# TimmyOVO/deepseek-ocr.rs

Measured on AMD Instinct MI355X. Metric: pages/sec + decode tok/s, DeepSeek-OCR fp16 1024px/512tok, higher is better.
Workload: dtype f32 (fp16-rounded decoder weights, bf16 vision/lm_head weights); 1 GPU; configs[1]: deepseek-ocr, 1024x1024 page, crop (2,2), 706-token prefill, 512 greedy tokens; pages_per_gpu=1, global_batch=1, parallelism=dp1

## Files before the change

deepseek-ocr.rs_amd/csrc/engine/capi.cpp:

```cpp
#include "../../../include/dsocr.h"

#include <fcntl.h>
#include <signal.h>
#include <unistd.h>

#include <cmath>
#include <cstdio>
#include <cstdlib>
#include <cstring>
#include <fstream>
#include <memory>
#include <sstream>
#include <string>
#include <utility>

#include "../common/host_util.hpp"
#include "dots.hpp"
#include "engine.hpp"
#include "host_ops.hpp"

struct dsocr_engine {
    std::unique_ptr<dsocr::Engine> impl;
    dsocr::Controls staged;
};
// ... 998 lines not shown
        out->o_proj = cp(p.o_proj);
        out->router = cp(p.router);
        out->layers_step = cp(p.layers_step);
        out->lm_head_screened = cp(p.lm_head_screened);
        out->moe_gateup_kernel = p.gateup_kernel;
        out->moe_down_kernel = p.down_kernel;
    });
}

dsocr_status dsocr_engine_set_spans(dsocr_engine* e, int enable) {
    return guarded([&] {
        if (!e) throw std::runtime_error("EINVAL: NULL engine");
        e->impl->set_spans(enable);
    });
}

dsocr_status dsocr_engine_spans(const dsocr_engine* e, uint64_t* out, size_t cap, size_t* kinds, size_t* layers,
                                size_t* steps) {
    return guarded([&] {
        if (!e) throw std::runtime_error("EINVAL: NULL engine");
        const auto& v = e->impl->spans();
        const size_t nl = e->impl->cfg().lang.layers;
        const size_t ns = v.empty() ? 0 : (size_t)e->impl->span_steps();
        if (kinds) *kinds = (size_t)e->impl->span_kinds();
        if (layers) *layers = nl;
        if (steps) *steps = ns;
        if (!out) return;
        if (v.size() > cap)
            throw std::runtime_error("EINVAL: span buffer holds " + std::to_string(cap) + " values, " +
                                     std::to_string(v.size()) + " needed");
        if (!v.empty()) std::memcpy(out, v.data(), v.size() * 8);
    });
}
static_assert(dsocr::Engine::SPAN_FIELDS == 5, "dsocr.h documents 5 fields per span record");

dsocr_status dsocr_engine_set_persist_stamps(dsocr_engine* e, int mode) {
    return guarded([&] {
        if (!e) throw std::runtime_error("EINVAL: NULL engine");
        e->impl->set_persist_stamps(mode);
    });
}

dsocr_status dsocr_engine_persist_info(const dsocr_engine* e, int* used, double* durations, size_t cap_d,
                                       size_t* n_launches, uint64_t* stamps, size_t cap_s, size_t* n_stamps) {
    return guarded([&] {
        if (!e) throw std::runtime_error("EINVAL: NULL engine");
        const auto& d = e->impl->persist_launch_us();
        const auto& st = e->impl->persist_stamps();
        if (used) *used = e->impl->persist_used() ? 1 : 0;
        if (n_launches) *n_launches = d.size();
        if (n_stamps) *n_stamps = st.size();
        if (durations) {
            if (d.size() > cap_d) throw std::runtime_error("EINVAL: duration buffer too small");
            if (!d.empty()) std::memcpy(durations, d.data(), d.size() * sizeof(double));
        }
        if (stamps) {
            if (st.size() > cap_s) throw std::runtime_error("EINVAL: stamp buffer too small");
            if (!st.empty()) std::memcpy(stamps, st.data(), st.size() * 8);
        }
    });
}

dsocr_status dsocr_device_count(int* n) {
    return guarded([&] { check_hip(hipGetDeviceCount(n), "hipGetDeviceCount"); });
}
dsocr_status dsocr_dev_alloc(size_t bytes, void** ptr) {
    return guarded([&] {
        if (hipMalloc(ptr, bytes ? bytes : 16) != hipSuccess) throw std::runtime_error("ENOMEM: hipMalloc failed");
    });
}
dsocr_status dsocr_dev_free(void* ptr) {
    return guarded([&] { check_hip(hipFree(ptr), "hipFree"); });
}
dsocr_status dsocr_memcpy_h2d(void* dst, const void* src, size_t bytes) {
    return guarded([&] { check_hip(hipMemcpy(dst, src, bytes, hipMemcpyHostToDevice), "hipMemcpy H2D"); });
}
dsocr_status dsocr_memcpy_d2h(void* dst, const void* src, size_t bytes) {
    return guarded([&] { check_hip(hipMemcpy(dst, src, bytes, hipMemcpyDeviceToHost), "hipMemcpy D2H"); });
}
dsocr_status dsocr_dev_sync(void) {
    return guarded([&] { check_hip(hipDeviceSynchronize(), "hipDeviceSynchronize"); });
}
dsocr_status dsocr_synth_bf16(const char* name, uint64_t seed, uint64_t n, uint16_t* out) {
    return guarded([&] {
        if (!name || (!out && n)) throw std::runtime_error("EINVAL: NULL argument");
        dsocr::synth_bf16(name, seed, n, out);
    });
}
dsocr_status dsocr_resize_bicubic(const uint8_t* src, uint32_t sw, uint32_t sh, uint8_t* dst, uint32_t dw, uint32_t dh) {
    return guarded([&] {
        if (!src || !dst) throw std::runtime_error("EINVAL: NULL argument");
        dsocr::resize_bicubic(src, (int)sw, (int)sh, dst, (int)dw, (int)dh);
    });
}

dsocr_status dsocr_resize_catmull_rom(const uint8_t* src, uint32_t sw, uint32_t sh, uint8_t* dst, uint32_t dw,
                                      uint32_t dh) {
    return guarded([&] {
        if (!src || !dst || !sw || !sh || !dw || !dh) throw std::runtime_error("EINVAL: NULL argument or empty image");
        dsocr::resize_catmull_rom_fir(src, (int)sw, (int)sh, dst, (int)dw, (int)dh);
    });
}

dsocr_status dsocr_k_gemm(int M, int N, int K, const float* A, const void* W, int wdtype, const float* bias, float* C,
                          int act, int accumulate) {
    return guarded([&] {
        if (K % 8) throw std::runtime_error("EINVAL: K must be a multiple of 8");
        dsocr::GemmArgs g;
        g.M = M; g.N = N; g.K = K; g.A = A; g.lda = K; g.W = W; g.ldw = K; g.wdtype = wdtype; g.bias = bias;
        g.C = C; g.ldc = N; g.act = act; g.accumulate = accumulate;
        dsocr::launch_gemm(g, nullptr);
        check_hip(hipGetLastError(), "gemm launch");
        check_hip(hipDeviceSynchronize(), "gemm");
    });
}
dsocr_status dsocr_k_gemm_grouped(int M, int N, int K, const float* A, int lda, const int* a_rows, const void* W,
                                  int wdtype, long long w_group_stride, const float* bias, long long bias_group_stride,
                                  float* C, int ldc, const int* c_rows, int act, int accumulate, const int* group_off,
                                  int groups, int max_group_rows, int kernel) {
    return guarded([&] {
        if (!A || !W || !C || !group_off || groups < 1 || M < 0 || N < 1 || K < 1)
            throw std::runtime_error("EINVAL: grouped gemm arguments");
        dsocr::GemmArgs g;
        g.M = M; g.N = N; g.K = K; g.A = A; g.lda = lda; g.a_rows = a_rows; g.W = W; g.ldw = K; g.wdtype = wdtype;
        g.w_group_stride = (long)w_group_stride; g.bias = bias; g.bias_group_stride = (long)bias_group_stride;
        g.C = C; g.ldc = ldc; g.c_rows = c_rows; g.act = act; g.accumulate = accumulate;
        g.group_off = group_off; g.groups = groups; g.max_group_rows = max_group_rows;
        if (kernel == 1 || kernel == 2) dsocr::launch_gemm_f32a_grouped(g, nullptr, kernel == 2 ? 128 : 32);
        else dsocr::launch_gemm(g, nullptr);
        check_hip(hipGetLastError(), "grouped gemm launch");
        check_hip(hipDeviceSynchronize(), "grouped gemm");
    });
}
dsocr_status dsocr_k_gemm_f32a(int M, int N, int K, const float* A, const void* W, int wdtype, const float* bias,
                               float* C, int act, int accumulate, int splits) {
    return guarded([&] {
        if (wdtype != dsocr::WDT_BF16 && wdtype != dsocr::WDT_F16) throw std::runtime_error("EINVAL: weights must be bf16 or f16");
        dsocr::GemmBf16Args g;
        g.M = M; g.N = N; g.K = K; g.A = A; g.lda = K; g.W = W; g.ldw = K; g.bias = bias;
        g.w_f16 = wdtype == dsocr::WDT_F16;
        g.C = C; g.ldc = N; g.act = act; g.accumulate = accumulate;
        if (!dsocr::gemm_f32a_ok(g)) throw std::runtime_error("EINVAL: gemm_f32a needs K % 32 == 0 and 16-byte aligned rows");
        g.splits = splits > 0 ? splits : dsocr::gemm_f32a_splits(M, N, K);
        float* part = nullptr;
        if (g.splits > 1) {
            check_hip(hipMalloc(&part, sizeof(float) * (size_t)g.splits * M * N), "hipMalloc");
            g.part = part;
        }
        dsocr::launch_gemm_f32a(g, nullptr);
        hipError_t e = hipGetLastError();
        if (e == hipSuccess) e = hipDeviceSynchronize();
        if (part) (void)hipFree(part);
        check_hip(e, "gemm_f32a");
    });
}
dsocr_status dsocr_k_gemv(int M, int N, int K, const float* x, const float* norm_w, float eps, const void* W,
                          int wdtype, const float* bias, float* y, int act, int accumulate) {
    return dsocr_k_gemv_ex(M, N, K, x, K, norm_w, eps, W, K, wdtype, bias, y, N, act, accumulate, 0, nullptr);
}
static bool gemv_kind_is_mm(const char* kind) { return std::strncmp(kind, "dec_mm_", 7) == 0; }
dsocr_status dsocr_k_gemv_ex(int M, int N, int K, const float* x, int ldx, const float* norm_w, float eps,
                             const void* W, int ldw, int wdtype, const float* bias, float* y, int ldy, int act,
                             int accumulate, int swizzle, const char** kind) {
    return guarded([&] {
        if (K < 8 || K % 8) throw std::runtime_error("EINVAL: K must be a positive multiple of 8");
        if (M < 0 || N < 0 || ldx < K || ldw < K || ldy < N || ldx % 4 || ldw % 8)
            throw std::runtime_error("EINVAL: gemv strides (ldx >= K, ldx % 4 == 0, ldw >= K, ldw % 8 == 0, ldy >= N)");
        if (wdtype != dsocr::WDT_BF16 && wdtype != dsocr::WDT_F16) throw std::runtime_error("EINVAL: weights must be bf16 or f16");
        dsocr::DecGemvArgs a;
        a.M = M; a.N = N; a.K = K; a.x = x; a.ldx = ldx; a.W = W; a.ldw = ldw; a.wdtype = wdtype; a.bias = bias;
        a.y = y; a.ldy = ldy; a.act = act; a.accumulate = accumulate; a.norm_w = norm_w; a.eps = eps;
        void* swz = nullptr;
        if (swizzle) {
            if (ldw != K) throw std::runtime_error("EINVAL: swizzle needs row-major W with ldw == K");
            if (!dsocr::dec_mm_ok(a) || !gemv_kind_is_mm(dsocr::dec_gemv_kernel_kind(a)))
                throw std::runtime_error("EINVAL: swizzle outside dec_mm's range (M 3..8, K 1280, N >= 16)");
            check_hip(hipMalloc(&swz, sizeof(uint16_t) * dsocr::mm_swizzle_elems(N, K)), "hipMalloc");
            a.w_swz = swz;
        }
        if (kind) *kind = dsocr::dec_gemv_kernel_kind(a);
        hipError_t e = hipSuccess;
        try {
            if (swz) dsocr::launch_mm_swizzle(W, N, K, swz, nullptr);
            dsocr::launch_dec_gemv(a, nullptr);
            e = hipGetLastError();
        } catch (...) {
            (void)hipDeviceSynchronize();
            if (swz) (void)hipFree(swz);
            throw;
        }
        if (e == hipSuccess) e = hipDeviceSynchronize();
        if (swz) (void)hipFree(swz);
        check_hip(e, "gemv");
    });
}
dsocr_status dsocr_k_gemv_kind(int M, int N, int K, int ldw, int wdtype, int has_norm, int has_xn_out, int swizzle,
                               const char** kind, int* rows_per_launch) {
    return guarded([&] {
        if (!kind) throw std::runtime_error("EINVAL: NULL argument");
        static float fd = 0.f;
        static uint16_t wd = 0;
        dsocr::DecGemvArgs a;
        a.M = M; a.N = N; a.K = K; a.x = &fd; a.ldx = K; a.W = &wd; a.ldw = ldw; a.wdtype = wdtype;
        a.y = &fd; a.ldy = N; a.norm_w = has_norm ? &fd : nullptr; a.xn_out = has_xn_out ? &fd : nullptr;
        a.w_swz = swizzle ? &wd : nullptr;
        *kind = dsocr::dec_gemv_kernel_kind(a, rows_per_launch);
    });
}
dsocr_status dsocr_k_mm_swizzle(int N, int K, const void* w, void* out) {
    return guarded([&] {
        if (N < 1 || K < 32 || K % 32 || !w || !out) throw std::runtime_error("EINVAL: mm_swizzle needs N >= 1, K % 32 == 0, w, out");
        dsocr::launch_mm_swizzle(w, N, K, out, nullptr);
        check_hip(hipGetLastError(), "mm_swizzle launch");
        check_hip(hipDeviceSynchronize(), "mm_swizzle");
    });
}
dsocr_status dsocr_k_silu_mul(int rows, int I, const float* g, int ldg, float* h, int ldh) {
    return guarded([&] {
        if (rows < 0 || I < 1 || ldg < 2 * I || ldh < I || !g || !h) throw std::runtime_error("EINVAL: silu_mul needs ldg >= 2 I, ldh >= I");
        dsocr::launch_silu_mul(g, ldg, I, rows, h, ldh, nullptr);
        check_hip(hipGetLastError(), "silu_mul launch");
        check_hip(hipDeviceSynchronize(), "silu_mul");
    });
}
dsocr_status dsocr_k_gemv_splitk(int M, int N, int K, const float* x, const void* W, int wdtype, const float* bias,
                                 float* y, int accumulate) {
    return guarded([&] {
        dsocr::DecGemvArgs a;
        a.M = M; a.N = N; a.K = K; a.x = x; a.ldx = K; a.W = W; a.ldw = K; a.wdtype = wdtype; a.bias = bias;
        a.y = y; a.ldy = N; a.accumulate = accumulate;
        if (!dsocr::dec_mm_splitk_ok(a)) throw std::runtime_error("EINVAL: gemv_splitk needs M <= 8, K % 64 == 0");
        float* part = nullptr;
        int* tick = nullptr;
        check_hip(hipMalloc(&part, sizeof(float) * dsocr::dec_mm_splitk_part_floats(N, K)), "hipMalloc");
        check_hip(hipMalloc(&tick, sizeof(int) * dsocr::dec_mm_splitk_ticks(N)), "hipMalloc");
        check_hip(hipMemset(tick, 0, sizeof(int) * dsocr::dec_mm_splitk_ticks(N)), "hipMemset");
        dsocr::launch_dec_mm_splitk(a, part, tick, nullptr);
        hipError_t e = hipDeviceSynchronize();
        (void)hipFree(part);
        (void)hipFree(tick);
        check_hip(e, "gemv_splitk");
    });
}
dsocr_status dsocr_k_layernorm(int rows, int cols, const float* x, const float* w, const float* b, float eps, float* y) {
    return guarded([&] {
        if (cols % 4) throw std::runtime_error("EINVAL: cols must be a multiple of 4");
        dsocr::launch_layernorm(x, cols, y, cols, nullptr, rows, cols, w, b, eps, nullptr);
        check_hip(hipDeviceSynchronize(), "layernorm");
    });
}
dsocr_status dsocr_k_dsq_dequant(int qtype, const void* src, size_t src_bytes, size_t out_dim, size_t in_dim,
                                 void* out_f16) {
    return guarded([&] {
        const size_t need = dsocr::dsq_payload_bytes(qtype, (long)out_dim, (long)in_dim);
        if (need == 0) throw std::runtime_error("EINVAL: unsupported snapshot tensor dtype code " + std::to_string(qtype));
        if (src_bytes != need)
            throw std::runtime_error("EINVAL: payload is " + std::to_string(src_bytes) + " bytes, expected " + std::to_string(need));
        dsocr::launch_dsq_dequant(qtype, src, (long)out_dim, (long)in_dim, out_f16, nullptr);
        check_hip(hipGetLastError(), "dsq_dequant launch");
        check_hip(hipDeviceSynchronize(), "dsq_dequant");
    });
}
dsocr_status dsocr_k_rmsnorm(int rows, int cols, const float* x, const float* w, float eps, float* y) {
    return guarded([&] {
        if (cols % 4) throw std::runtime_error("EINVAL: cols must be a multiple of 4");
        dsocr::launch_rmsnorm(x, cols, y, cols, rows, cols, w, eps, nullptr);
        check_hip(hipDeviceSynchronize(), "rmsnorm");
    });
}
dsocr_status dsocr_k_attention(int n_seq, int L, int heads, int hd, float scale, int causal, const float* q,
                               const float* k, const float* v, float* o, const float* relh, const float* relw, int gh,
                               int gw) {
    return guarded([&] {
        if (hd != 32 && hd != 64 && hd != 128) throw std::runtime_error("EINVAL: head_dim must be 32, 64 or 128");
        const long C = (long)heads * hd;
        dsocr::AttnArgs a;
        a.q = {q, C, hd, nullptr};
        a.k = {k, C, hd, nullptr};
        a.v = {v, C, hd, nullptr};
        a.o = o; a.o_row_stride = C; a.o_head_stride = hd; a.n_seq = n_seq; a.L = L; a.heads = heads;
        a.kv_heads = heads; a.hd = hd; a.scale = scale; a.causal = causal;
        float* rb = nullptr;
        float* part = nullptr;
        if (causal) {
            a.part_floats = dsocr::attention_causal_part_floats(n_seq, heads, L, hd);
            check_hip(hipMalloc(&part, sizeof(float) * a.part_floats), "hipMalloc attention pieces");
            a.part = part;
        }
        if (relh && relw) {
            if (gh * gw != L) throw std::runtime_error("EINVAL: rel-pos grid does not match L");
            check_hip(hipMalloc(&rb, sizeof(float) * (size_t)n_seq * heads * L * (gh + gw)), "hipMalloc relbias");
            dsocr::launch_sam_relbias(q, C, n_seq, gh, gw, heads, hd, relh, relw, rb, nullptr);
            a.relbias = rb; a.rel_h = gh; a.rel_w = gw;
        }
        dsocr::launch_attention(a, nullptr);
        hipError_t e = hipDeviceSynchronize();
        if (rb) (void)hipFree(rb);
        if (part) (void)hipFree(part);
        check_hip(e, "attention");
    });
}
dsocr_status dsocr_k_attention_prefix(int n_seq, int L, int prefix, int heads, int kv_heads, int hd, float scale,
                                      const float* q, const float* k, const float* v, float* o) {
    return guarded([&] {
        dsocr::AttnPrefixArgs a;
        a.q = q; a.k = k; a.v = v; a.o = o;
// ... 1436 lines not shown
```

deepseek-ocr.rs_amd/csrc/engine/engine.cpp:

```cpp
#include "engine.hpp"

#include <algorithm>
#include <chrono>
#include <random>
#include <cstdlib>
#include <cmath>
#include <cstring>
#include <fstream>
#include <functional>
#include <sstream>

#include "../common/host_util.hpp"
#include "dsq.hpp"
#include "host_ops.hpp"

namespace dsocr {

namespace {

struct HostMat {
    std::vector<uint16_t> data;
    int dt = WDT_BF16;
};

// ... 566 lines not shown
            g.data.insert(g.data.end(), u.data.begin(), u.data.end());
            e.gu.W = up16(g);
            e.gu.wdt = g.dt;
            e.gu.N = 2 * Q.inter;
            e.gu.K = D;
            e.down = lin_nobias(lp + "mlp.down_proj", D, Q.inter);
            enc_.layers.push_back(e);
        }
        enc_.norm = vecf(qp + "model.model.norm.weight", D);
        enc_.query_768 = vecf(qp + "query_768.weight", (size_t)Q.query_768 * D);
        enc_.query_1024 = vecf(qp + "query_1024.weight", (size_t)Q.query_1024 * D);
        {
            const int Lmax = 2 * Q.query_1024, half = hd / 2;
            std::vector<float> inv(half), c((size_t)Lmax * hd), s((size_t)Lmax * hd);
            for (int i = 0; i < half; ++i) inv[i] = 1.0f / powf(Q.rope_theta, (float)i / (float)half);
            for (int p = 0; p < Lmax; ++p)
                for (int i = 0; i < half; ++i) {
                    const float a = (float)p * inv[i];
                    c[(size_t)p * hd + i] = c[(size_t)p * hd + half + i] = cosf(a);
                    s[(size_t)p * hd + i] = s[(size_t)p * hd + half + i] = sinf(a);
                }
            enc_.cos = upf(c);
            enc_.sin = upf(s);
        }
        if (S.out_ch[1] != D) throw std::runtime_error("EINVAL: SAM output channels must equal the qwen2-0-5b encoder width");
    } else {
    const ClipConfig& C = cfg_.clip;
    const std::string cp = "model.vision_model.";
    clip_.cls = vecf(cp + "embeddings.class_embedding", C.hidden);
    clip_.pos_host = src.f32(cp + "embeddings.position_embedding.weight", (size_t)(C.seq + 1) * C.hidden);
    clip_.pre = {vecf(cp + "pre_layrnorm.weight", C.hidden), vecf(cp + "pre_layrnorm.bias", C.hidden)};
    for (int l = 0; l < C.layers; ++l) {
        ClipLayer cl;
        const std::string lp = cp + "transformer.layers." + std::to_string(l) + ".";
        cl.ln1 = {vecf(lp + "layer_norm1.weight", C.hidden), vecf(lp + "layer_norm1.bias", C.hidden)};
        cl.ln2 = {vecf(lp + "layer_norm2.weight", C.hidden), vecf(lp + "layer_norm2.bias", C.hidden)};
        cl.qkv = lin(lp + "self_attn.qkv_proj", 3 * C.hidden, C.hidden, true);
        cl.out = lin(lp + "self_attn.out_proj", C.hidden, C.hidden, true);
        cl.fc1 = lin(lp + "mlp.fc1", C.ffn, C.hidden, true);
        cl.fc2 = lin(lp + "mlp.fc2", C.hidden, C.ffn, true);
        clip_.layers.push_back(cl);
    }
    if (C.hidden != S.out_ch[1]) throw std::runtime_error("EINVAL: CLIP width must equal SAM output channels");
    if (C.hidden + S.out_ch[1] != cfg_.proj_in) throw std::runtime_error("EINVAL: combined hidden dims do not match projector input");
    }

    proj_ = lin("model.projector.layers", cfg_.proj_out, cfg_.proj_in, true);
    newline_ = cfg_.variant != VARIANT_OCR2 && src.has("model.image_newline")
                   ? vecf("model.image_newline", cfg_.proj_out)
                   : upf(std::vector<float>(cfg_.proj_out, 0.f));
    separator_ = vecf("model.view_seperator", cfg_.proj_out);

    const LangConfig& L = cfg_.lang;
    {
        HostMat m = src.h16("model.embed_tokens.weight", (size_t)L.vocab * L.hidden);
        embed_ = up16(m);
        embed_dt_ = m.dt;
    }
    const int H = L.hidden, KVH = L.kv_heads * L.head_dim;
    for (int l = 0; l < L.layers; ++l) {
        DecLayer d;
        const std::string lp = "model.layers." + std::to_string(l) + ".";
        d.in_norm = {vecf(lp + "input_layernorm.weight", H), nullptr};
        d.post_norm = {vecf(lp + "post_attention_layernorm.weight", H), nullptr};
        d.qkv = lin_cat({lp + "self_attn.q_proj", lp + "self_attn.k_proj", lp + "self_attn.v_proj"},
                        {L.heads * L.head_dim, KVH, L.kv_heads * L.v_head_dim}, H);
        d.o = lin(lp + "self_attn.o_proj", H, L.heads * L.v_head_dim, true);
        d.moe = L.moe_layer(l);
        if (!d.moe) {
            d.gu = lin_cat({lp + "mlp.gate_proj", lp + "mlp.up_proj"}, {L.inter, L.inter}, H);
            d.down = lin(lp + "mlp.down_proj", H, L.inter, true);
            if (d.gu.b || d.down.b) throw std::runtime_error("EINVAL: biased dense MLP not supported");
        } else {
            const int E = L.n_routed, I = L.moe_inter;
            HostMat r = src.h16(lp + "mlp.gate.weight", (size_t)E * H);
            d.router.W = up16(r);
            d.router.wdt = r.dt;
            d.router.N = E;
            d.router.K = H;
            d.router.b = optvec(lp + "mlp.gate.e_score_correction_bias", E);
            HostMat gu, dn;
            gu.data.resize((size_t)E * 2 * I * H);
            dn.data.resize((size_t)E * H * I);
            for (int e = 0; e < E; ++e) {
                const std::string ep = lp + "mlp.experts." + std::to_string(e) + ".";
                HostMat g = src.h16(ep + "gate_proj.weight", (size_t)I * H, I, H);
                HostMat u = src.h16(ep + "up_proj.weight", (size_t)I * H, I, H);
                HostMat w = src.h16(ep + "down_proj.weight", (size_t)H * I, H, I);
                if (src.has(ep + "gate_proj.bias") || src.has(ep + "down_proj.bias"))
                    throw std::runtime_error("EINVAL: biased experts not supported");
                std::copy(g.data.begin(), g.data.end(), gu.data.begin() + (size_t)e * 2 * I * H);
                std::copy(u.data.begin(), u.data.end(), gu.data.begin() + (size_t)e * 2 * I * H + (size_t)I * H);
                std::copy(w.data.begin(), w.data.end(), dn.data.begin() + (size_t)e * H * I);
                gu.dt = dn.dt = g.dt;
            }
            d.e_gu = up16(gu);
            d.e_d = up16(dn);
            d.e_wdt = gu.dt;
            if (L.n_shared > 0) {
                const int Is = I * L.n_shared;
                d.has_shared = true;
                d.s_gu = lin_cat({lp + "mlp.shared_experts.gate_proj", lp + "mlp.shared_experts.up_proj"}, {Is, Is}, H);
                d.s_d = lin(lp + "mlp.shared_experts.down_proj", H, Is, true);
            }
            if (packed_experts && d.e_wdt == WDT_F16 && dec_route_grp_ok(8, E, H, L.topk)) {
                std::vector<std::string> gu_n, dn_n;
                for (int e = 0; e < E; ++e) {
                    const std::string ep = lp + "mlp.experts." + std::to_string(e) + ".";
                    gu_n.push_back(ep + "gate_proj.weight");
                    gu_n.push_back(ep + "up_proj.weight");
                    dn_n.push_back(ep + "down_proj.weight");
                }
                const long Is = (long)I * L.n_shared;
                const std::vector<std::string> sgu_n = {lp + "mlp.shared_experts.gate_proj.weight",
                                                        lp + "mlp.shared_experts.up_proj.weight"};
                const std::vector<std::string> sdn_n = {lp + "mlp.shared_experts.down_proj.weight"};
                bool ok = records_qtype(gu_n, I, H) >= 0 && records_qtype(dn_n, H, I) >= 0;
                if (ok && d.has_shared)
                    ok = !d.s_gu.b && !d.s_d.b && records_qtype(sgu_n, Is, H) >= 0 && records_qtype(sdn_n, H, Is) >= 0;
                if (ok) {
                    pack_records(gu_n, I, H, d.q_gu, d.packed_bytes);
                    pack_records(dn_n, H, I, d.q_d, d.packed_bytes);
                    if (d.has_shared) {
                        pack_records(sgu_n, Is, H, d.q_sgu, d.packed_bytes);
                        pack_records(sdn_n, H, Is, d.q_sd, d.packed_bytes);
                    }
                    d.packed = true;
                }
            }
        }
        layers_.push_back(d);
    }
    HIP_CHECK(hipDeviceSynchronize());
    final_norm_ = vecf("model.norm.weight", H);
    lm_head_ = lin("lm_head", L.vocab, H, false);
    if ((lm_head_.wdt == WDT_BF16 || lm_head_.wdt == WDT_F16) && H % 16 == 0 && H <= 1536) {
        const size_t vp = (size_t)(L.vocab + 15) / 16 * 16;
        lmq_ = dev_alloc((size_t)L.vocab * H);
        lmq_scale_ = (float*)dev_alloc(vp * 4);
        lmq_bound_ = (float*)dev_alloc(vp * 4);
        HIP_CHECK(hipMemset(lmq_scale_, 0, vp * 4));
        HIP_CHECK(hipMemset(lmq_bound_, 0, vp * 4));
        if (lmhead_q8mm_ok(8, L.vocab, H)) {
            lmq_qnorm_ = (float*)dev_alloc(vp * 4);
            HIP_CHECK(hipMemset(lmq_qnorm_, 0, vp * 4));
            lmq_frag_ = dev_alloc(lmhead_qfrag_bytes(L.vocab, H));
        }
        launch_lmhead_quantize(lm_head_.W, L.vocab, H, lmq_, lmq_scale_, lmq_bound_, nullptr, lmq_qnorm_, lmq_frag_,
                               lm_head_.wdt);
        HIP_CHECK(hipDeviceSynchronize());
    }
}

void Engine::linear(const float* x, int M, int ldx, const Lin& l, float* y, int ldy, int act, int accumulate,
                    const int* c_rows) {
    flops_acc_ += 2.0 * M * (double)l.N * l.K;
    if (M <= 16 && !c_rows) {
        DecGemvArgs a;
        a.M = M; a.N = l.N; a.K = l.K; a.x = x; a.ldx = ldx; a.W = l.W; a.ldw = l.K; a.wdtype = l.wdt;
        a.bias = l.b; a.y = y; a.ldy = ldy; a.act = act; a.accumulate = accumulate;
        launch_dec_gemv(a, stream_);
    } else if ((l.wdt == WDT_F16 || l.wdt == WDT_BF16) && l.K % 32 == 0 && ldx % 4 == 0 &&
               (reinterpret_cast<uintptr_t>(x) & 15) == 0) {
        GemmBf16Args g;
        g.M = M; g.N = l.N; g.K = l.K; g.A = x; g.lda = ldx; g.W = l.W; g.ldw = l.K; g.w_f16 = l.wdt == WDT_F16;
        g.bias = l.b; g.C = y; g.ldc = ldy; g.c_rows = c_rows; g.act = act; g.accumulate = accumulate;
        g.splits = gemm_f32a_splits(M, l.N, l.K);
        if (g.splits > 1) g.part = wsf("g_splitk", (size_t)g.splits * M * l.N);
        launch_gemm_f32a(g, stream_);
    } else {
        GemmArgs g;
        g.M = M; g.N = l.N; g.K = l.K; g.A = x; g.lda = ldx; g.W = l.W; g.ldw = l.K; g.wdtype = l.wdt;
        g.bias = l.b; g.C = y; g.ldc = ldy; g.c_rows = c_rows; g.act = act; g.accumulate = accumulate;
        launch_gemm(g, stream_);
    }
}

float* Engine::sam_pos(int g) {
    auto it = sam_.pos_dev.find(g);
    if (it != sam_.pos_dev.end()) return it->second;
    const int C = cfg_.sam.dim, src = sam_.pos_grid;
    std::vector<float> r = bicubic_resize_aa(sam_.pos_host, C, src, src, g, g);
    std::vector<float> nhwc((size_t)g * g * C);
    for (int c = 0; c < C; ++c)
        for (int p = 0; p < g * g; ++p) nhwc[(size_t)p * C + c] = r[(size_t)c * g * g + p];
    float* d = (float*)dev_alloc(nhwc.size() * 4);
    HIP_CHECK(hipMemcpy(d, nhwc.data(), nhwc.size() * 4, hipMemcpyHostToDevice));
    sam_.pos_dev[g] = d;
    return d;
}

std::pair<float*, float*> Engine::sam_rel(SamBlock& b, int g) {
    auto it = b.rel_dev.find(g);
    if (it != b.rel_dev.end()) return it->second;
    const int hd = cfg_.sam.dim / cfg_.sam.heads;
    std::vector<float> rh = rel_pos_resize(b.relh, b.rel_len, hd, g);
    std::vector<float> rw = rel_pos_resize(b.relw, b.rel_len, hd, g);
    float* dh = (float*)dev_alloc(rh.size() * 4);
    float* dw = (float*)dev_alloc(rw.size() * 4);
    HIP_CHECK(hipMemcpy(dh, rh.data(), rh.size() * 4, hipMemcpyHostToDevice));
    HIP_CHECK(hipMemcpy(dw, rw.data(), rw.size() * 4, hipMemcpyHostToDevice));
    b.rel_dev[g] = {dh, dw};
    return {dh, dw};
}

float* Engine::clip_pos(int tokens) {
    auto it = clip_.pos_dev.find(tokens);
    if (it != clip_.pos_dev.end()) return it->second;
    const ClipConfig& C = cfg_.clip;
    std::vector<float> out;
    if (tokens == C.seq + 1) {
        out = clip_.pos_host;
    } else {
        const int s = (int)std::lround(std::sqrt((double)C.seq)), t = (int)std::lround(std::sqrt((double)(tokens - 1)));
        if (t * t != tokens - 1) throw std::runtime_error("EINVAL: clip positional table tgt tokens not square");
        std::vector<float> grid((size_t)C.hidden * s * s);
        for (int p = 0; p < s * s; ++p)
            for (int c = 0; c < C.hidden; ++c) grid[(size_t)c * s * s + p] = clip_.pos_host[(size_t)(1 + p) * C.hidden + c];
        std::vector<float> r = bicubic_resize_aa(grid, C.hidden, s, s, t, t);
        out.resize((size_t)tokens * C.hidden);
        std::copy(clip_.pos_host.begin(), clip_.pos_host.begin() + C.hidden, out.begin());
        for (int p = 0; p < t * t; ++p)
            for (int c = 0; c < C.hidden; ++c) out[(size_t)(1 + p) * C.hidden + c] = r[(size_t)c * t * t + p];
    }
    float* d = (float*)dev_alloc(out.size() * 4);
    HIP_CHECK(hipMemcpy(d, out.data(), out.size() * 4, hipMemcpyHostToDevice));
    clip_.pos_dev[tokens] = d;
    return d;
}

static bool vis_streams_on() {
    static const bool v = !(getenv("DSOCR_VIS_STREAMS") && atoi(getenv("DSOCR_VIS_STREAMS")) == 0);
    return v;
}

float* Engine::vision_pass(const float* imgs, int n, int Spx, const std::string& out) {
    const SamConfig& S = cfg_.sam;
    const ClipConfig& CC = cfg_.clip;
    const int C = S.dim, heads = S.heads, hd = C / heads;
    if (Spx % S.patch) throw std::runtime_error("EINVAL: image dimensions must be divisible by patch size");
    const int g = Spx / S.patch;
    if (g % 2 || (g / 2) % 2) throw std::runtime_error("EINVAL: spatial dims cannot be evenly downsampled by stride 2");
    const long rows = (long)n * g * g;
    hipStream_t st = stream_;
    const bool s1 = vis_stage_ == 0 || vis_stage_ == 1, s2 = vis_stage_ == 0 || vis_stage_ == 2;
    const bool s3 = vis_stage_ == 0 || vis_stage_ == 3;
    const int g2 = g / 2, g4 = g / 4, c0 = S.out_ch[0], c1 = S.out_ch[1];
    const int Sq = g4 * g4;
    float* sam_out = wsf("v_samout", (size_t)n * Sq * c1);
    if (s1) {
    float* cols = wsf("v_cols", (size_t)rows * 3 * S.patch * S.patch);
    launch_patch_im2col(imgs, n, Spx, Spx, S.patch, cols, st);
    float* x = wsf("v_x", (size_t)rows * C);
    linear(cols, (int)rows, 3 * S.patch * S.patch, sam_.patch, x, C);
    if (sam_.has_pos) launch_add_broadcast(x, sam_pos(g), (long)g * g, C, n, st);

    const int W = S.window;
    const int gp = g + (W - g % W) % W, nw = gp / W;
    const long wrows = (long)n * nw * nw * W * W;
    auto wm = winmaps_.find({n, g});
    if (wm == winmaps_.end()) {
        std::vector<int> tok2win(rows), win2tok(wrows, -1);
        for (int b = 0; b < n; ++b)
            for (int y = 0; y < g; ++y)
                for (int xx = 0; xx < g; ++xx) {
                    long t = ((long)b * g + y) * g + xx;
                    long w = (((long)b * nw + y / W) * nw + xx / W) * W * W + (y % W) * W + (xx % W);
                    tok2win[t] = (int)w;
                    win2tok[w] = (int)t;
                }
        int *a = nullptr, *b2 = nullptr;
        HIP_CHECK(hipMalloc(&a, tok2win.size() * 4));
        HIP_CHECK(hipMalloc(&b2, win2tok.size() * 4));
        HIP_CHECK(hipMemcpy(a, tok2win.data(), tok2win.size() * 4, hipMemcpyHostToDevice));
        HIP_CHECK(hipMemcpy(b2, win2tok.data(), win2tok.size() * 4, hipMemcpyHostToDevice));
        wm = winmaps_.emplace(std::make_pair(n, g), std::make_pair(a, b2)).first;
    }
    int* d_tok2win = wm->second.first;
    int* d_win2tok = wm->second.second;
    const long maxrows = std::max(rows, wrows);
    float* xn = wsf("v_xn", (size_t)maxrows * C);
    float* qkv = wsf("v_qkv", (size_t)maxrows * 3 * C);
    float* ctx = wsf("v_ctx", (size_t)maxrows * C);
    const int hid = (int)(C * S.mlp_ratio);
    float* hbuf = wsf("v_h", (size_t)rows * hid);

    for (int bi = 0; bi < S.depth; ++bi) {
        SamBlock& blk = sam_.blocks[bi];
        const bool win = !blk.global;
        const int L = win ? W * W : g * g;
        const int nseq = win ? n * nw * nw : n;
        const long arows = (long)nseq * L;
        if (win) {
            HIP_CHECK(hipMemsetAsync(xn, 0, (size_t)wrows * C * 4, st));
            launch_layernorm(x, C, xn, C, d_tok2win, (int)rows, C, blk.n1.w, blk.n1.b, 1e-6f, st);
        } else {
            launch_layernorm(x, C, xn, C, nullptr, (int)rows, C, blk.n1.w, blk.n1.b, 1e-6f, st);
        }
        linear(xn, (int)arows, C, blk.qkv, qkv, 3 * C);
        AttnArgs a;
        a.q = {qkv, 3L * C, hd, nullptr};
        a.k = {qkv + C, 3L * C, hd, nullptr};
        a.v = {qkv + 2 * C, 3L * C, hd, nullptr};
        a.o = ctx;
        a.o_row_stride = C;
        a.o_head_stride = hd;
        a.n_seq = nseq;
        a.L = L;
        a.heads = heads;
        a.kv_heads = heads;
        a.hd = hd;
        a.scale = (float)(1.0 / std::sqrt((double)hd));
        if (blk.use_rel) {
            const int gg = win ? W : g;
            auto rel = win ? std::make_pair<float*, float*>(nullptr, nullptr) : sam_rel(blk, g);
            if (win) rel = sam_rel(blk, W);
            float* rb = wsf("v_relbias", (size_t)nseq * heads * L * (2 * gg));
            launch_sam_relbias(qkv, 3L * C, nseq, gg, gg, heads, hd, rel.first, rel.second, rb, st);
            a.relbias = rb;
            a.rel_h = gg;
            a.rel_w = gg;
        }
        flops_acc_ += 4.0 * nseq * (double)L * L * hd * heads;
        launch_attention(a, st);
        linear(ctx, (int)arows, C, blk.proj, x, C, 0, 1, win ? d_win2tok : nullptr);
        launch_layernorm(x, C, xn, C, nullptr, (int)rows, C, blk.n2.w, blk.n2.b, 1e-6f, st);
        linear(xn, (int)rows, C, blk.fc1, hbuf, hid, ACT_GELU_ERF);
        linear(hbuf, (int)rows, hid, blk.fc2, x, C, 0, 1);
    }
    const int NC = S.neck;
    float* y = wsf("v_neck", (size_t)rows * NC);
    linear(x, (int)rows, C, sam_.neck0, y, NC);
    launch_layernorm(y, NC, y, NC, nullptr, (int)rows, NC, sam_.neck1.w, sam_.neck1.b, 1e-6f, st);
    float* ncols = wsf("v_ncols", (size_t)rows * 9 * NC);
    launch_conv_im2col_nhwc(y, n, g, g, NC, 3, 3, 1, 1, ncols, st);
    linear(ncols, (int)rows, 9 * NC, sam_.neck2, y, NC);
    launch_layernorm(y, NC, y, NC, nullptr, (int)rows, NC, sam_.neck3.w, sam_.neck3.b, 1e-6f, st);
    launch_conv_im2col_nhwc(y, n, g, g, NC, 3, 3, 2, 1, ncols, st);
    float* z = wsf("v_net2", (size_t)n * g2 * g2 * c0);
    linear(ncols, n * g2 * g2, 9 * NC, sam_.net2, z, c0);
    float* ncols2 = wsf("v_ncols2", (size_t)n * g4 * g4 * 9 * c0);
    launch_conv_im2col_nhwc(z, n, g2, g2, c0, 3, 3, 2, 1, ncols2, st);
    linear(ncols2, n * Sq, 9 * c0, sam_.net3, sam_out, c1);
    }
    if (cfg_.variant == VARIANT_OCR2) return encoder_pass(sam_out, n, Sq, out);

    const int T = Sq + 1, CH = CC.hidden, chd = CH / CC.heads;
    const long crow = (long)n * T;
    float* cx = wsf("c_x", (size_t)crow * CH);
    if (s2) {
    launch_clip_embed(sam_out, clip_.cls, clip_pos(T), n, Sq, CH, cx, st);
    launch_layernorm(cx, CH, cx, CH, nullptr, (int)crow, CH, clip_.pre.w, clip_.pre.b, 1e-5f, st);
    }
    float* cxn = wsf("c_xn", (size_t)crow * CH);
    float* cqkv = wsf("c_qkv", (size_t)crow * 3 * CH);
    float* cctx = wsf("c_ctx", (size_t)crow * CH);
    float* ch = wsf("c_h", (size_t)crow * CC.ffn);
    for (int l = 0; s2 && l < CC.layers; ++l) {
        ClipLayer& cl = clip_.layers[l];
        launch_layernorm(cx, CH, cxn, CH, nullptr, (int)crow, CH, cl.ln1.w, cl.ln1.b, 1e-5f, st);
        linear(cxn, (int)crow, CH, cl.qkv, cqkv, 3 * CH);
        AttnArgs a;
        a.q = {cqkv, 3L * CH, chd, nullptr};
        a.k = {cqkv + CH, 3L * CH, chd, nullptr};
        a.v = {cqkv + 2 * CH, 3L * CH, chd, nullptr};
        a.o = cctx;
        a.o_row_stride = CH;
        a.o_head_stride = chd;
        a.n_seq = n;
        a.L = T;
        a.heads = CC.heads;
        a.kv_heads = CC.heads;
        a.hd = chd;
        a.scale = (float)(1.0 / std::sqrt((double)chd));
        flops_acc_ += 4.0 * n * (double)T * T * chd * CC.heads;
        launch_attention(a, st);
        linear(cctx, (int)crow, CH, cl.out, cx, CH, 0, 1);
        launch_layernorm(cx, CH, cxn, CH, nullptr, (int)crow, CH, cl.ln2.w, cl.ln2.b, 1e-5f, st);
        linear(cxn, (int)crow, CH, cl.fc1, ch, CC.ffn, ACT_QUICK_GELU);
        linear(ch, (int)crow, CC.ffn, cl.fc2, cx, CH, 0, 1);
    }
    float* pre = wsf("p_pre", (size_t)n * Sq * (CH + c1));
    float* post = wsf(out, (size_t)n * Sq * cfg_.proj_out);
    if (s3) {
        launch_concat_clip_sam(cx, sam_out, n, Sq, CH, c1, pre, st);
        linear(pre, n * Sq, CH + c1, proj_, post, cfg_.proj_out);
    }
    return post;
}

float* Engine::encoder_pass(const float* sam_out, int n, int P, const std::string& out) {
    const Qwen2EncConfig& Q = cfg_.enc;
    const float* query = P == Q.query_768 ? enc_.query_768 : P == Q.query_1024 ? enc_.query_1024 : nullptr;
    if (!query)
        throw std::runtime_error("EINVAL: unsupported Qwen2 query length " + std::to_string(P) + " (expected " +
                                 std::to_string(Q.query_768) + " or " + std::to_string(Q.query_1024) + ")");
    hipStream_t st = stream_;
    const int D = Q.dim, hd = Q.head_dim, L = 2 * P, QW = Q.heads * hd, KW = Q.kv_heads * hd, W3 = QW + 2 * KW;
    const long rows = (long)n * L;
    float* x = wsf("q2_x", (size_t)rows * D);
    float* xn = wsf("q2_xn", (size_t)rows * D);
    float* qkv = wsf("q2_qkv", (size_t)rows * W3);
    float* ctx = wsf("q2_ctx", (size_t)rows * QW);
    float* gu = wsf("q2_gu", (size_t)rows * 2 * Q.inter);
    float* hbuf = wsf("q2_h", (size_t)rows * Q.inter);
    const bool s2 = vis_stage_ == 0 || vis_stage_ == 2, s3 = vis_stage_ == 0 || vis_stage_ == 3;
    if (s2) launch_ocr2_build_seq(sam_out, query, n, P, D, x, st);
    for (const EncLayer& e : enc_.layers) {
        if (!s2) break;
        launch_rmsnorm(x, D, xn, D, (int)rows, D, e.in_norm.w, Q.rms_eps, st);
        linear(xn, (int)rows, D, e.qkv, qkv, W3);
        launch_ocr2_rope(qkv, W3, rows, L, Q.heads + Q.kv_heads, hd, enc_.cos, enc_.sin, st);
        AttnPrefixArgs a;
        a.q = qkv; a.k = qkv + QW; a.v = qkv + QW + KW; a.o = ctx;
        a.ldq = a.ldk = a.ldv = W3; a.ldo = QW;
        a.n_seq = n; a.L = L; a.prefix = P; a.heads = Q.heads; a.kv_heads = Q.kv_heads; a.hd = hd;
        a.scale = (float)(1.0 / std::sqrt((double)hd));
        flops_acc_ += 4.0 * n * Q.heads * hd * (2.0 * P * P + 0.5 * P * (P + 1.0));
        launch_attention_prefix(a, st);
        linear(ctx, (int)rows, QW, e.o, x, D, 0, 1);
        launch_rmsnorm(x, D, xn, D, (int)rows, D, e.post_norm.w, Q.rms_eps, st);
        linear(xn, (int)rows, D, e.gu, gu, 2 * Q.inter);
        launch_silu_mul(gu, 2 * Q.inter, Q.inter, (int)rows, hbuf, Q.inter, st);
        linear(hbuf, (int)rows, Q.inter, e.down, x, D, 0, 1);
    }
    float* qx = wsf("q2_q", (size_t)n * P * D);
    float* post = wsf(out, (size_t)n * P * cfg_.proj_out);
    if (s3) {
        launch_ocr2_take_queries(x, n, P, D, qx, st);
        launch_rmsnorm(qx, D, qx, D, n * P, D, enc_.norm, Q.rms_eps, st);
        linear(qx, n * P, D, proj_, post, cfg_.proj_out);
    }
    return post;
}

void Engine::check_page_variant(const PagePixels& pg) const {
    if (pg.variant != cfg_.variant)
        throw std::runtime_error(std::string("EINVAL: page was prepared for ") +
                                 (pg.variant == VARIANT_OCR2 ? "DeepSeek-OCR-2" : "DeepSeek-OCR") + " but the engine runs " +
                                 (cfg_.variant == VARIANT_OCR2 ? "DeepSeek-OCR-2" : "DeepSeek-OCR") +
                                 " (image slot layout mismatch)");
}

enum RowKind : int { ROW_TOKEN = 0, ROW_HOST = 1, ROW_VISION = 2, ROW_NEWLINE = 3, ROW_SEPARATOR = 4 };

static std::vector<std::pair<int, long>> image_row_order(const PagePixels& pg) {
    std::vector<std::pair<int, long>> seq;
    const int ls = pg.tile / 64, gs = pg.gsize / 64;
    const long n_local = pg.n_tiles > 0 ? (long)pg.n_tiles * ls * ls : 0;
    if (pg.variant == VARIANT_OCR2) {
        for (long i = 0; i < n_local + (long)gs * gs; ++i) seq.push_back({ROW_VISION, i});
        seq.push_back({ROW_SEPARATOR, 0});
        return seq;
    }
    for (int R = 0; n_local && R < pg.crop_h * ls; ++R) {
        for (int Cc = 0; Cc < pg.crop_w * ls; ++Cc) {
            const int crop = (R / ls) * pg.crop_w + (Cc / ls);
            seq.push_back({ROW_VISION, ((long)crop * ls + R % ls) * ls + Cc % ls});
        }
        seq.push_back({ROW_NEWLINE, 0});
    }
    for (int R = 0; R < gs; ++R) {
        for (int Cc = 0; Cc < gs; ++Cc) seq.push_back({ROW_VISION, n_local + (long)R * gs + Cc});
        seq.push_back({ROW_NEWLINE, 0});
    }
    seq.push_back({ROW_SEPARATOR, 0});
    return seq;
}

std::vector<std::vector<float>> Engine::image_embeddings(const std::vector<const PagePixels*>& pages) {
    std::vector<std::vector<float>> result;
    const int H = cfg_.proj_out;
    for (const PagePixels* p : pages) {
        check_page_variant(*p);
        float* gimg = p->global_dev && p->dev_ordinal == device_ ? p->global_dev : upload("e_gimg", p->global_chw);
        float* gpost = vision_pass(gimg, 1, p->gsize, "e_gpost");
        const int gs = p->gsize / 64;
        std::vector<float> gh((size_t)gs * gs * H);
        HIP_CHECK(hipMemcpyAsync(gh.data(), gpost, gh.size() * 4, hipMemcpyDeviceToHost, stream_));
        std::vector<float> lh;
        int ls = 0;
        if (p->n_tiles > 0) {
            float* timg = p->tiles_dev && p->dev_ordinal == device_ ? p->tiles_dev : upload("e_timg", p->tiles_chw);
            float* lpost = vision_pass(timg, p->n_tiles, p->tile, "e_lpost");
            ls = p->tile / 64;
            lh.resize((size_t)p->n_tiles * ls * ls * H);
            HIP_CHECK(hipMemcpyAsync(lh.data(), lpost, lh.size() * 4, hipMemcpyDeviceToHost, stream_));
        }
        HIP_CHECK(hipStreamSynchronize(stream_));
        std::vector<float> nl(H), sp(H);
        HIP_CHECK(hipMemcpy(nl.data(), newline_, H * 4, hipMemcpyDeviceToHost));
        HIP_CHECK(hipMemcpy(sp.data(), separator_, H * 4, hipMemcpyDeviceToHost));
        std::vector<float> rows;
        const size_t n_local = lh.size() / H;
        for (const auto& [kind, i] : image_row_order(*p)) {
            const float* r = kind == ROW_NEWLINE ? nl.data() : kind == ROW_SEPARATOR ? sp.data()
                             : (size_t)i < n_local ? &lh[i * H] : &gh[(i - n_local) * H];
            rows.insert(rows.end(), r, r + H);
        }
        result.push_back(std::move(rows));
    }
    return result;
}

void Engine::layer_forward_prefill(int l, int T, int B, const int* row_page, const int* row_pos, const long* q_off,
                                   const long* kv_off, const long* o_off, const int* seq_len, int max_len, int Lmax,
                                   const int* past, int max_total, bool chunk_attn) {
    const LangConfig& L = cfg_.lang;
    DecLayer& d = layers_[l];
    hipStream_t st = stream_;
    const int H = L.hidden, hd = L.head_dim, KVH = L.kv_heads * hd, QKVN = d.qkv.N;
    float* X = wsf("d_x", (size_t)T * H);
    float* XN = wsf("d_xn", (size_t)T * H);
    float* QKV = wsf("d_qkv", (size_t)T * QKVN);
    float* CTX = wsf("d_ctx", (size_t)T * H);
    float* kc = kc_ + (long)l * layer_kv(B) + (long)kv_page0_ * page_stride_;
    float* vc = vc_ + (long)l * layer_kv(B) + (long)kv_page0_ * page_stride_;

    launch_rmsnorm(X, H, XN, H, T, H, d.in_norm.w, L.rms_eps, st);
    linear(XN, T, H, d.qkv, QKV, QKVN);
    RopeKvArgs r;
    r.qkv = QKV; r.ld = QKVN; r.rows = T; r.row_page = row_page; r.row_pos = row_pos;
    r.heads = L.heads; r.kv_heads = L.kv_heads; r.hd = hd; r.rope_dim = L.rope_dim; r.use_mla = L.use_mla;
    r.cos = rope_cos_; r.sin = rope_sin_; r.kc = kc; r.vc = vc; r.page_stride = page_stride_; r.head_stride = head_stride_;
    launch_rope_kv(r, st);
    if (past) {
        AttnPastArgs a;
        a.q = {QKV, QKVN, hd, q_off};
        a.k = {kc, hd, head_stride_, kv_off};
        a.v = {vc, hd, head_stride_, kv_off};
        a.o = CTX; a.o_row_stride = H; a.o_head_stride = hd; a.o_seq_off = o_off;
        a.n_seq = B; a.past = past; a.n_q = seq_len; a.max_q = max_len; a.max_total = max_total;
        a.heads = L.heads; a.kv_heads = L.kv_heads; a.hd = hd;
        a.scale = (float)(1.0 / std::sqrt((double)hd));
        flops_acc_ += 4.0 * (double)T * max_total * hd * L.heads;
        if (chunk_attn) {
            launch_attention_chunk(a, st);
            ++chunk_attn_launches_;
        } else {
            a.part_floats = attention_past_part_floats(B, L.heads, max_len, max_total, hd);
            a.part = wsf("d_attn_past", a.part_floats);
            launch_attention_past(a, st);
        }
    } else {
        AttnArgs a;
        a.q = {QKV, QKVN, hd, q_off};
        a.k = {kc, hd, head_stride_, kv_off};
        a.v = {vc, hd, head_stride_, kv_off};
        a.o = CTX; a.o_row_stride = H; a.o_head_stride = hd; a.o_seq_off = o_off;
        a.n_seq = B; a.L = max_len; a.seq_len = seq_len;
        a.heads = L.heads; a.kv_heads = L.kv_heads; a.hd = hd;
        a.scale = (float)(1.0 / std::sqrt((double)hd));
        a.causal = 1;
        constexpr size_t kPartCapFloats = (size_t)128 << 20;
        const size_t part_floats = attention_causal_part_floats(B, L.heads, max_len, hd);
        if (part_floats <= kPartCapFloats) {
            a.part_floats = part_floats;
            a.part = wsf("d_attn_part", a.part_floats);
        }
        for (int q = 0; q < B && q < (int)prefill_lens_.size(); ++q)
            flops_acc_ += 2.0 * (double)prefill_lens_[q] * (prefill_lens_[q] + 1) * hd * L.heads;
        launch_attention(a, st);
    }
    (void)Lmax;
    (void)KVH;
    linear(CTX, T, H, d.o, X, H, 0, 1);
    launch_rmsnorm(X, H, XN, H, T, H, d.post_norm.w, L.rms_eps, st);
    if (!d.moe) {
        const int I = L.inter;
        float* G = wsf("d_g", (size_t)T * 2 * I);
        float* HH = wsf("d_hh", (size_t)T * I);
        linear(XN, T, H, d.gu, G, 2 * I);
        launch_silu_mul(G, 2 * I, I, T, HH, I, st);
        linear(HH, T, I, d.down, X, H, 0, 1);
        return;
    }
    const int E = L.n_routed, K = L.topk, I = L.moe_inter, TK = T * K;
    float* LOG = wsf("d_log", (size_t)T * E);
    int* IDS = wsi("d_ids", TK);
    float* WTS = wsf("d_wts", TK);
    int* EOFF = wsi("d_eoff", E + 1);
    int* AROW = wsi("d_arow", TK);
    int* APOS = wsi("d_apos", TK);
    linear(XN, T, H, d.router, LOG, E);
    launch_router_topk(LOG, T, E, K, L.scoring == "softmax", L.norm_topk, L.routed_scaling, IDS, WTS, st);
    launch_moe_group(IDS, T, K, E, EOFF, AROW, APOS, nullptr, st);
    float* G = wsf("d_eg", (size_t)TK * 2 * I);
    float* HH = wsf("d_ehh", (size_t)TK * I);
    float* Y = wsf("d_ey", (size_t)TK * H);
    GemmArgs g1;
    g1.M = TK; g1.N = 2 * I; g1.K = H; g1.A = XN; g1.lda = H; g1.a_rows = AROW; g1.W = d.e_gu; g1.ldw = H;
    g1.wdtype = d.e_wdt; g1.w_group_stride = (long)2 * I * H; g1.C = G; g1.ldc = 2 * I;
    g1.group_off = EOFF; g1.groups = E; g1.max_group_rows = T;
    launch_gemm(g1, st);
    flops_acc_ += 2.0 * TK * (2.0 * I) * H + 2.0 * TK * (double)H * I;
    launch_silu_mul(G, 2 * I, I, TK, HH, I, st);
    GemmArgs g2;
    g2.M = TK; g2.N = H; g2.K = I; g2.A = HH; g2.lda = I; g2.W = d.e_d; g2.ldw = I; g2.wdtype = d.e_wdt;
    g2.w_group_stride = (long)H * I; g2.C = Y; g2.ldc = H; g2.group_off = EOFF; g2.groups = E; g2.max_group_rows = T;
    launch_gemm(g2, st);
    float* YS = nullptr;
    if (d.has_shared) {
        const int Is = d.s_d.K;
        float* GS = wsf("d_sg", (size_t)T * 2 * Is);
        float* HS = wsf("d_shh", (size_t)T * Is);
        YS = wsf("d_sy", (size_t)T * H);
        linear(XN, T, H, d.s_gu, GS, 2 * Is);
        launch_silu_mul(GS, 2 * Is, Is, T, HS, Is, st);
        linear(HS, T, Is, d.s_d, YS, H);
    }
    launch_moe_combine(Y, APOS, WTS, YS, T, K, H, X, 1, st);
}

static bool router_swz_off() {
    const char* e = getenv("DSOCR_ROUTER_SWZ");
    return e && atoi(e) == 0;
}
static bool mm_swz_off() {
    const char* e = getenv("DSOCR_MM_SWZ");
    return e && atoi(e) == 0;
}

MoeDecodeArgs Engine::moe_args(int l, int B, float* X) {
    const LangConfig& L = cfg_.lang;
    DecLayer& d = layers_[l];
    const int H = L.hidden, E = L.n_routed, K = L.topk, I = L.moe_inter, TK = B * K;
    MoeDecodeArgs a;
    a.T = B; a.H = H; a.E = E; a.topk = K; a.I = I;
    a.x = X; a.norm_w = d.post_norm.w; a.eps = L.rms_eps; a.out = X;
    a.router = d.router.W; a.router_wdt = d.router.wdt; a.router_bias = d.router.b;
    a.Wgu = d.e_gu; a.Wd = d.e_d; a.wdtype = d.e_wdt;
    if (d.has_shared) {
        if (d.s_gu.wdt != d.e_wdt) throw std::runtime_error("EINTERNAL: shared/routed expert dtype mismatch");
        a.Is = d.s_d.K; a.sWgu = d.s_gu.W; a.sWd = d.s_d.W; a.hs = wsf("s_shh", (size_t)B * a.Is);
    }
    a.softmax_scoring = L.scoring == "softmax"; a.norm_topk = L.norm_topk; a.scaling = L.routed_scaling;
    a.xn = wsf("s_xn", (size_t)B * H);
    a.xn_router = wsf("s_xn_router", (size_t)B * H);
    a.logits = wsf("s_log", (size_t)B * E);
    a.ids = wsi("s_ids", TK); a.wts = wsf("s_wts", TK);
    a.h = wsf("s_ehh", (size_t)TK * I);
    a.grp = wsi("s_grp", moe_grp_ints(E, B, K));
    a.route_cnt = rows_.route_cnt;
    if (B >= 3 && B <= 8) {
        a.dn_part = wsf("s_dnpart", moe_down_mm_part_floats(E, B, K, I, a.Is, H));
        a.dn_tick = rows_.dn_tick;
    }
    if (B <= 8 && d.packed) {
        a.qWgu = d.q_gu; a.qWd = d.q_d; a.qsWgu = d.q_sgu; a.qsWd = d.q_sd;
    }
    if (B <= 8 && d.e_gu_swz && (!d.has_shared || d.s_gu_swz)) {
        a.Wgu_swz = d.e_gu_swz; a.Wd_swz = d.e_d_swz; a.sWgu_swz = d.s_gu_swz; a.sWd_swz = d.s_d_swz;
        if (!router_swz_off()) a.router_swz = d.router_swz;
    }
    if (B > 8) {
        a.eoff = wsi("s_eoff", E + 1); a.arow = wsi("s_arow", TK); a.apos = wsi("s_apos", TK);
        a.aw = wsf("s_aw", TK); a.active = wsi("s_active", E); a.n_active = wsi("s_nact", 1);
    }
    return a;
}

DecAttn2Args Engine::attn_args(int l, int B, int Lmax, int copy) {
    const LangConfig& L = cfg_.lang;
    const int hd = L.head_dim, QKVN = layers_[l].qkv.N;
    const long layer_kv = this->layer_kv(B);
    DecAttn2Args da;
    da.qkv = rows_.qkv[copy]; da.ld = QKVN; da.kv_pos = rows_.kv_pos; da.B = B;
    da.heads = L.heads; da.kv_heads = L.kv_heads; da.hd = hd; da.rope_dim = L.rope_dim; da.use_mla = L.use_mla;
    da.max_len = Lmax; da.cos = rope_cos_; da.sin = rope_sin_;
    da.kc = kc_ + (long)l * layer_kv; da.vc = vc_ + (long)l * layer_kv;
    da.page_stride = page_stride_; da.head_stride = head_stride_;
    da.scale = (float)(1.0 / std::sqrt((double)hd));
    da.part = rows_.part[copy];
    da.o = wsf("s_ctx", (size_t)B * L.hidden); da.o_ld = L.hidden;
    da.counters = rows_.attn_cnt;
    da.err = rows_.err;
    return da;
}

static bool graphs_on() {
    const char* e = getenv("DSOCR_NO_GRAPH");
    return !(e && atoi(e) != 0);
}

bool Engine::persist_ok(int B, int Lmax) {
    const char* e = getenv("DSOCR_PERSIST");
    if (!e || atoi(e) == 0) return false;
    const LangConfig& L = cfg_.lang;
    for (const DecLayer& d : layers_)
        if (d.packed) return false;
    if (B != 1 || L.use_mla || L.rope_dim != L.head_dim || L.v_head_dim != L.head_dim || L.n_shared <= 0 ||
        L.topk_method != "greedy" || L.hidden_act != "silu")
        return false;
    if (!dec_persist_shape_ok(L.hidden, L.heads, L.kv_heads, L.head_dim, L.n_routed, L.topk, L.moe_inter,
                              L.n_shared * L.moe_inter, L.inter, Lmax))
        return false;
    for (const DecLayer& d : layers_) {
        if (d.qkv.wdt != WDT_F16 || d.qkv.b || d.o.wdt != WDT_F16 || d.o.b) return false;
        if (d.moe) {
            if (!d.router.W || d.router.wdt != WDT_F16 || d.e_wdt != WDT_F16 || !d.has_shared || d.s_gu.wdt != WDT_F16 ||
                d.s_d.wdt != WDT_F16 || d.s_gu.b || d.s_d.b)
                return false;
        } else if (!d.gu.W || d.gu.wdt != WDT_F16 || d.down.wdt != WDT_F16) {
            return false;
        }
    }
    return dec_persist_resident() != 0;
}

void Engine::ensure_persist() {
    if (persist_lw_ || capturing_) return;
    const LangConfig& L = cfg_.lang;
    const int H = L.hidden, E = L.n_routed, I = L.moe_inter;
    std::vector<PersistLayerW> tab(layers_.size());
    for (size_t l = 0; l < layers_.size(); ++l) {
        DecLayer& d = layers_[l];
        PersistLayerW& w = tab[l];
        w.qkv = (const uint16_t*)d.qkv.W;
        w.o = (const uint16_t*)d.o.W;
        w.in_w = d.in_norm.w;
// ... 2295 lines not shown
```

deepseek-ocr.rs_amd/csrc/engine/engine.hpp:

```cpp
#pragma once
#include <hip/hip_runtime.h>

#include <cstring>
#include <functional>
#include <map>
#include <memory>
#include <set>
#include <stdexcept>
#include <string>
#include <vector>

#include "../kernels/kernels.hpp"
#include "config.hpp"
#include "hip_raii.hpp"

namespace dsocr {

struct Lin {
    void* W = nullptr;
    int wdt = WDT_BF16;
    int N = 0, K = 0;
    float* b = nullptr;
};
struct Ln {
// ... 199 lines not shown
        *g_status = nullptr, *g_on = nullptr, *g_stage = nullptr;
    size_t g_stage_cap = 0;
    GuidedTables guided_tables() const {
        GuidedTables t;
        t.mask = g_mask; t.mask_ld = g_mask_ld; t.cap_states = g_states; t.cap_edges = g_edges;
        t.rowptr = g_rowptr; t.tok = g_tok; t.next = g_next;
        t.state = g_state; t.seen = g_seen; t.status = g_status; t.on = g_on;
        return t;
    }
};
struct DecodeRowsSpec {
    int rows = 0, Lcap = 0;
    long ctx_cap = 0, out_cap = 0;
    bool sampler = false, ban = false, rowpar = false;
    bool handoff_max = false;
    bool zero_fill = false;
    int lp_k = -1;
    bool lp_side = false;
    bool bias = false;
    size_t bias_stage = 0;
    bool stops = false;
    int stop_stage_rows = 1;
    bool penalties = false;
    bool ngram_window = false;
    bool guided = false;
    int guided_states = GUIDED_MAX_STATES;
    long guided_edges = GUIDED_MAX_EDGES;
    size_t guided_stage = 0;
};
typedef void (*TokenCb)(size_t, const int64_t*, void*);
std::vector<uint32_t> rng_state_from_u64(uint64_t seed);

class Engine {
  public:
    Engine(const std::string& config_path, const std::string& weights_path, int device, int dtype, uint64_t seed,
           const std::string& snapshot_path = "", uint32_t load_flags = 0);
    ~Engine();
    void packed_info(size_t* packed_layers, size_t* moe_layers, size_t* packed_bytes) const;

    const ModelConfig& cfg() const { return cfg_; }
    int variant() const { return cfg_.variant; }
    std::vector<std::vector<float>> image_embeddings(const std::vector<const PagePixels*>& pages);
    std::vector<std::vector<int64_t>> generate(const std::vector<GenRequest>& reqs, const GenParams& p, TokenCb cb,
                                               void* user);
    Timings last_timings() const { return timings_; }
    struct LogprobRows {
        int K = 0;
        size_t cap = 0;
        std::vector<int> n;
        std::vector<float> lp, top_lp;
        std::vector<int> top_id;
    };
    const LogprobRows& last_logprobs() const { return last_lp_; }
    const std::vector<int>& last_stop_hits() const { return last_stop_hits_; }
    const std::vector<int>& last_guided() const { return last_guided_; }
    size_t stop_launches() const { return stop_launches_; }
    struct KernelProfile {
        double avg_us = 0, bytes = 0, flops = 0;
        int launches = 0;
        double replay_us = 0;
        double ctx_us = 0;
    };
    struct DecodeProfile {
        KernelProfile moe_gateup, moe_down, attention, lm_head, qkv, o_proj, router, layers_step, lm_head_screened;
        int experts_touched = 0, tokens = 0, kv_len = 0;
        const char* gateup_kernel = "";
        const char* down_kernel = "";
    };
    DecodeProfile profile_decode(int iters);
    enum SpanKind : int { SPAN_GATEUP = 0, SPAN_DOWN = 1, SPAN_ATTN = 2, SPAN_KINDS = 3, SPAN_OPROJ = 3, SPAN_ROUTER = 4,
                          SPAN_KINDS_CHAIN = 5 };
    static constexpr int SPAN_FIELDS = 5;
    enum SpanMode : int { SPAN_WAVES = 1, SPAN_EVENTS = 2, SPAN_CHAIN = 4 };
    void set_spans(int mode) { span_mode_ = (mode & SPAN_CHAIN) ? SPAN_CHAIN : mode & (SPAN_WAVES | SPAN_EVENTS); }
    int span_kinds() const { return spans_kinds_; }
    const std::vector<unsigned long long>& spans() const { return spans_host_; }
    int span_steps() const { return spans_steps_; }
    hipStream_t stream() const { return stream_; }
    void set_persist_stamps(int mode) { persist_stamp_mode_ = mode; }
    bool persist_used() const { return persist_active_; }
    const std::vector<unsigned long long>& persist_stamps() const { return persist_stamps_host_; }
    const std::vector<double>& persist_launch_us() const { return persist_ev_us_; }
    void upload_page(PagePixels& pg);
    void prepare_page_device(const uint8_t* rgb, int w, int h, PagePixels& px);

    struct SessionFeatures {
        bool per_request = false;
        bool logprobs = false;
        bool logit_bias = false;
        bool stops = false;
        bool penalties = false;
        bool ngram_window = false;
        bool guided = false;
    };
    struct SessionInfo {
        int slots = 0, active = 0, max_context = 0, out_cap = 0, kv_cap = 0, burst_cap = 0;
        size_t steps = 0;
        size_t steps_screened = 0, steps_exact = 0;
        SessionFeatures feat;
        bool pending = false;
        int pending_rows_done = 0, pending_rows_total = 0, pending_slices = 0;
        int pending_stage = 0;
        size_t chunk_attn_launches = 0;
    };
    struct SlotStatus {
        int slot = 0, done = 0, out_len = 0;
        std::vector<int64_t> fresh;
    };
    void session_open(int slots, int max_context, const GenParams& p, const SessionFeatures& feat);
    void session_stop_hit(int slot, int* seq, int* match_len);
    void session_guided_state(int slot, int* state, int* status);
    void session_logprobs(int slot, size_t first, size_t count, int top_k, float* token_lp, int64_t* top_id, float* top_lp);
    int session_admit(const GenRequest& rq, size_t max_new, bool seed_set, uint64_t seed);
    int session_admit(const GenRequest& rq, const GenParams& p);
    std::vector<SlotStatus> session_step(int k);
    std::vector<SlotStatus> session_poll();
    std::vector<int64_t> session_retire(int slot, int* moved_from);
    void session_close();
    bool session_info(SessionInfo* out) const;
    static constexpr int kMaxPrefixEntries = 64;
    struct PrefixStats {
        size_t entries = 0, bytes = 0, admissions = 0, rows_reused = 0;
    };
    int session_prefix_keep(int slot, int rows);
    int session_admit_prefix(int handle, const GenRequest& rq, const GenParams& p);
    void session_prefix_drop(int handle);
    PrefixStats session_prefix_stats() const;
    int session_admit_begin(const GenRequest& rq, const GenParams& p, int chunk_rows);
    bool session_admit_advance(int* slot);
    void session_admit_cancel();

  private:
    void load_weights(const std::string& path, uint64_t seed, const std::string& snapshot_path, bool packed_experts);
    void* ws(const std::string& name, size_t bytes);
    float* wsf(const std::string& name, size_t n) { return (float*)ws(name, n * sizeof(float)); }
    int* wsi(const std::string& name, size_t n) { return (int*)ws(name, n * sizeof(int)); }
    long* wsl(const std::string& name, size_t n) { return (long*)ws(name, n * sizeof(long)); }
    template <typename T>
    T* upload(const std::string& name, const std::vector<T>& v) {
        T* p = (T*)ws(name, v.size() * sizeof(T) + 16);
        upload_to(p, name, v);
        return p;
    }
    template <typename T>
    void upload_to(T* dst, const std::string& name, const std::vector<T>& v) {
        const size_t bytes = v.size() * sizeof(T);
        if (v.empty()) return;
        void* h = pinned(name, bytes);
        std::memcpy(h, v.data(), bytes);
        HIP_CHECK(hipMemcpyAsync(dst, h, bytes, hipMemcpyHostToDevice, stream_));
    }
    void* pinned(const std::string& name, size_t bytes);
    void linear(const float* x, int M, int ldx, const Lin& l, float* y, int ldy, int act = 0, int accumulate = 0,
                const int* c_rows = nullptr);
    float* sam_pos(int g);
    std::pair<float*, float*> sam_rel(SamBlock& b, int g);
    float* clip_pos(int tokens);
    float* vision_pass(const float* imgs, int n, int S, const std::string& out);
    float* encoder_pass(const float* sam_out, int n, int P, const std::string& out);
    void check_page_variant(const PagePixels& pg) const;
    void decode_step(int B, int Lmax);
    bool persist_ok(int B, int Lmax);
    void ensure_persist();
    MoeDecodeArgs moe_args(int l, int B, float* X);
    DecAttn2Args attn_args(int l, int B, int Lmax, int copy = 0);
    DecodeRows rows_;
    void reserve_decode_rows(const DecodeRowsSpec& spec);
    void refill_handoffs();
    void sample_args(int B, int slot0, const GenParams& p, bool per_request, DecSampleArgs& sa, SampleArgs& pen);
    DecLpArgs lp_args(const DecSampleArgs& sa, int row0);
    DecBiasArgs bias_args(const DecSampleArgs& sa, int row0);
    void build_logit_bias(const LogitBias& lb, int row, size_t stage_off);
    DecPenaltyArgs penalty_args(const DecSampleArgs& sa, int row0);
    void write_penalties(const GenRequest* reqs, int row0, int n);
    DecNgramWindowArgs ngram_window_args(const DecSampleArgs& sa, int row0, int plain);
    void write_ngram_windows(const GenRequest* reqs, int row0, int n);
    void build_guided(const Guided& g, int row, size_t stage_off, long eos);
    DecGuidedMaskArgs guided_mask_args(const DecSampleArgs& sa, int row0);
    DecGuidedAdvanceArgs guided_advance_args(const DecSampleArgs& sa, int row0);
    DecStopArgs stop_args(const DecSampleArgs& sa, int row0);
    void stop_match(const DecSampleArgs& sa, int row0);
    void build_stop_table(const StopSet& st, int row, int stage_row);
    void decode_head(int B, DecSampleArgs& sa, const SampleArgs& pen, bool screened, const DecLpArgs* lp = nullptr,
                     bool stops = false, int window = -1);
    struct TailPlan {
        bool bias = false, guided = false, penalties = false, stops = false;
        int window = -1;
        const DecLpArgs* lp = nullptr;
    };
    void selection_tail(const DecSampleArgs& sa, const SampleArgs& pen, int row0, const TailPlan& t);
    void write_controls(const GenRequest* reqs, int row0, int n, long eos);
    void reserve_head_ws(int B);
    LmHeadQ8Args head_q8_args(int B);
    bool screen_applies(int B, float rep_penalty) const;
    struct GenState;
    void embed_pages(GenState& g);
    void plan_image_rows(GenState& g);
    void reset_decode_state(GenState& g);
    void forward_rows(GenState& g, const std::vector<int>& lens, const std::vector<int>& past = {}, int row0 = 0,
                      bool head = true, bool chunk_attn = false);
    void init_sampling(GenState& g);
    bool poll(GenState& g);
    void stream_tokens(GenState& g, int n);
    void decode_uncached(GenState& g);
    void decode_cached(GenState& g);
    void step_body(GenState& g);
    void begin_spans(GenState& g);
    void read_span_events(size_t step);
    void collect_spans();
    std::vector<std::vector<int64_t>> collect_outputs(GenState& g);
    struct Session;
    std::unique_ptr<Session> sess_;
    Session& open_session();
    void session_step_body(Session& s, bool screened, bool stops, bool windowed);
    bool session_head_screened(const Session& s, unsigned carried) const;
    double replay_us(int n, const std::function<void()>& body);
    void time_launches(KernelProfile& kp, int n, const std::function<void(int)>& body);
    void profile_gemvs(DecodeProfile& prof, int iters, const std::vector<int>& moe_layers);
    void profile_step_context(DecodeProfile& prof, int iters, int n_moe);
    void layer_forward_prefill(int l, int T, int B, const int* row_page, const int* row_pos, const long* q_off,
                               const long* kv_off, const long* o_off, const int* seq_len, int max_len, int Lmax,
                               const int* past = nullptr, int max_total = 0, bool chunk_attn = false);
    void session_admit_checks(const Session& s, const GenRequest& rq, const GenParams& rp, bool behind_prefix) const;
    int session_admit_tail(Session& s, const GenRequest& rq, const GenParams& rp, const RowParams& row, int slot = -1,
                           bool finish = true);
    struct PendingAdmit;
    void session_slot_move(Session& s, int src, int dst, int rows_bound);

    ModelConfig cfg_;
    int device_ = 0;
    int dtype_ = 1;
    hipStream_t stream_ = nullptr;
    hipStream_t vstream_ = nullptr;
    hipEvent_t vis_ev_[2] = {nullptr, nullptr};
    std::string ws_prefix_;
    std::vector<void*> allocations_;
    std::map<std::string, std::pair<void*, size_t>> ws_;
    bool capturing_ = false;

    SamW sam_;
    ClipW clip_;
    Qwen2EncW enc_;
    Lin proj_;
    float* newline_ = nullptr;
    float* separator_ = nullptr;
    void* embed_ = nullptr;
    int embed_dt_ = WDT_F16;
    std::vector<DecLayer> layers_;
    float* final_norm_ = nullptr;
    Lin lm_head_;
    void* lm_swz_ = nullptr;
    void ensure_mm_weights(int B);
    bool dense_mm_ok(const DecLayer& d, int B) const;
    void* lmq_ = nullptr;
    float* lmq_scale_ = nullptr;
    float* lmq_bound_ = nullptr;
    float* lmq_qnorm_ = nullptr;
    void* lmq_frag_ = nullptr;
    float* rope_cos_ = nullptr;
    float* rope_sin_ = nullptr;
    int rope_cap_ = 0;
    float* ones_ = nullptr;
    int* iota_ = nullptr;
    int small_cap_ = 0;
    float* kc_ = nullptr;
    float* vc_ = nullptr;
    long page_stride_ = 0, head_stride_ = 0;
    int kv_pages_ = 0, kv_page0_ = 0;
    long layer_kv(int B) const { return (long)(kv_pages_ ? kv_pages_ : B) * page_stride_; }
    std::set<std::string> ws_frozen_;
    Timings timings_;
    int vis_stage_ = 0;
    size_t chunk_attn_launches_ = 0;
    size_t stop_launches_ = 0;
    std::vector<int> last_stop_hits_;
    std::vector<int> last_guided_;
    double flops_acc_ = 0;
    std::vector<int> prefill_lens_;
    int last_B_ = 0;
    std::map<std::string, std::pair<void*, size_t>> pinned_;
    std::map<std::pair<int, int>, std::pair<int*, int*>> winmaps_;
    int last_Lmax_ = 0;
    float* trace_ = nullptr;
    LogprobRows last_lp_;
    int span_mode_ = 0;
    enum StepSkip : int { SKIP_GATEUP = 1, SKIP_DOWN = 2, SKIP_ATTN = 4 };
    int step_skip_ = 0;
    static bool qkv_attn_fused();
    static bool att_refill_defer();
    static int att_kv_delay();
    unsigned long long* span_slots_ = nullptr;
    unsigned long long* span_rec_ = nullptr;
    const int* span_step_ = nullptr;
    int span_cap_ = 0;
    std::vector<unsigned long long> spans_host_;
    int spans_steps_ = 0;
    std::vector<HipEvent> span_ev_;
    std::vector<double> span_ev_ns_;
    int spans_kinds_ = SPAN_KINDS;
    bool chain_active_ = false;
    unsigned long long* span_chain_ = nullptr;
    unsigned long long* span_chain_rec_ = nullptr;
    unsigned long long* span_tmark_ = nullptr;
    unsigned long long* chain_slots(int layer, int kind) const {
        return chain_active_ ? span_chain_ + ((size_t)layer * SPAN_KINDS_CHAIN + kind) * SPAN_SLOTS * 2 : nullptr;
    }
    unsigned long long* span_rec(int kind, int layer) const {
// ... 20 lines not shown
```

deepseek-ocr.rs_amd/csrc/kernels/gemm_bf16.hip:

```cpp
#include <algorithm>
#include <cstdint>
#include <cstdlib>
#include <stdexcept>

#include "dev_common.hpp"
#include "kernels.hpp"

namespace dsocr {

typedef __bf16 bf16x8_v __attribute__((ext_vector_type(8)));
typedef __attribute__((address_space(3))) void lds_void;

constexpr int TB_M = 128, TB_N = 128, TB_K = 64;
constexpr int TB_STAGE = (TB_M + TB_N) * TB_K;

__device__ __forceinline__ void stage_tile(const uint16_t* g, long ld, int r0, int rmax, int k0, uint16_t* lds,
                                           int wave, int lane) {
#pragma unroll
    for (int i = 0; i < 4; ++i) {
        const int R = (wave * 4 + i) * 8;
        const int r = R + (lane >> 3);
        const int j = (lane & 7) ^ ((r >> 1) & 7);
        const long row = min(r0 + r, rmax);
        __builtin_amdgcn_global_load_lds(reinterpret_cast<const void*>(g + row * ld + k0 + j * 8),
                                         (lds_void*)(lds + R * TB_K), 16, 0, 0);
    }
}

__device__ __forceinline__ bf16x8_v frag(const uint16_t* lds, int r, int kc) {
    const int c = kc ^ ((r >> 1) & 7);
    return *reinterpret_cast<const bf16x8_v*>(lds + r * TB_K + c * 8);
}

__device__ __forceinline__ float rnd_bf16(float v) { return (float)(__bf16)v; }

__device__ __forceinline__ void tile_coords(int tile, int ntm, int ntn, int gm, int& bm, int& bn) {
    if (gm <= 1) {
        bm = tile / ntn;
        bn = tile % ntn;
        return;
    }
    const int per_group = gm * ntn;
    const int first = (tile / per_group) * gm;
    const int gsz = min(ntm - first, gm);
    const int t = tile % per_group;
    bm = first + t % gsz;
    bn = t / gsz;
}

static int gemm_group_m(int requested) {
    if (requested >= 0) return requested;
    static const int v = getenv("DSOCR_GEMM_GROUP_M") ? atoi(getenv("DSOCR_GEMM_GROUP_M")) : 8;
    return v;
}

__device__ __forceinline__ void bf16_store_epilogue(const GemmBf16Args& g, long orow, int col, float acc, float bv) {
    float v = rnd_bf16(acc);
    if (g.bias) v = rnd_bf16(v + bv);
    if (g.act) v = rnd_bf16(apply_act(v, g.act));
    __bf16* cp = reinterpret_cast<__bf16*>(g.C) + orow * (long)g.ldc + col;
    if (g.accumulate) v = rnd_bf16((float)*cp + v);
    *cp = (__bf16)v;
}

template <int NST>
__global__ __launch_bounds__(256, 2) void gemm_bf16_nt_kernel(GemmBf16Args g) {
    __shared__ __attribute__((aligned(16))) uint16_t smem[NST * TB_STAGE];
    const int tid = threadIdx.x, lane = tid & 63, wave = tid >> 6;
    const int wm = wave >> 1, wn = wave & 1;
    const int ntn = (g.N + TB_N - 1) / TB_N;
    const int nwg = gridDim.x;
    const int orig = blockIdx.x, xcd = orig & 7, q = nwg >> 3, rr = nwg & 7;
    const int wgid = (xcd < rr ? xcd * (q + 1) : rr * (q + 1) + (xcd - rr) * q) + (orig >> 3);
    const int split = wgid % g.splits, tile = wgid / g.splits;
    int bm, bn;
    tile_coords(tile, (g.M + TB_M - 1) / TB_M, ntn, g.group_m, bm, bn);
    const int m0 = bm * TB_M, n0 = bn * TB_N;
    const uint16_t* A = reinterpret_cast<const uint16_t*>(g.A);
    const uint16_t* W = reinterpret_cast<const uint16_t*>(g.W);
    f32x16 acc[2][2];
#pragma unroll
    for (int i = 0; i < 2; ++i)
#pragma unroll
        for (int j = 0; j < 2; ++j)
#pragma unroll
            for (int r = 0; r < 16; ++r) acc[i][j][r] = 0.f;
    const int nk_all = g.K / TB_K;
    const int kbeg = (int)((long)nk_all * split / g.splits), kend = (int)((long)nk_all * (split + 1) / g.splits);
    const int nk = kend - kbeg;
    auto issue = [&](int kt) {
        uint16_t* st = smem + (NST == 1 ? 0 : (kt & 1) * TB_STAGE);
        stage_tile(A, g.lda, m0, g.M - 1, (kbeg + kt) * TB_K, st, wave, lane);
        stage_tile(W, g.ldw, n0, g.N - 1, (kbeg + kt) * TB_K, st + TB_M * TB_K, wave, lane);
    };
    if (NST == 2 && nk > 0) issue(0);
    for (int kt = 0; kt < nk; ++kt) {
        if (NST == 1) {
            issue(kt);
            asm volatile("s_waitcnt vmcnt(0)" ::: "memory");
        } else if (kt + 1 < nk) {
            issue(kt + 1);
            asm volatile("s_waitcnt vmcnt(8)" ::: "memory");
        } else {
            asm volatile("s_waitcnt vmcnt(0)" ::: "memory");
        }
        __builtin_amdgcn_s_barrier();
        asm volatile("" ::: "memory");
        const uint16_t* As = smem + (NST == 1 ? 0 : (kt & 1) * TB_STAGE);
        const uint16_t* Bs = As + TB_M * TB_K;
#pragma unroll
        for (int ks = 0; ks < TB_K / 16; ++ks) {
            const int kc = ks * 2 + (lane >> 5);
            bf16x8_v af[2], bfv[2];
#pragma unroll
            for (int i = 0; i < 2; ++i) af[i] = frag(As, wm * 64 + i * 32 + (lane & 31), kc);
#pragma unroll
            for (int j = 0; j < 2; ++j) bfv[j] = frag(Bs, wn * 64 + j * 32 + (lane & 31), kc);
#pragma unroll
            for (int i = 0; i < 2; ++i)
#pragma unroll
                for (int j = 0; j < 2; ++j) acc[i][j] = __builtin_amdgcn_mfma_f32_32x32x16_bf16(af[i], bfv[j], acc[i][j], 0, 0, 0);
        }
        asm volatile("s_waitcnt lgkmcnt(0)" ::: "memory");
        __builtin_amdgcn_s_barrier();
        asm volatile("" ::: "memory");
    }
    const int half = lane >> 5, l32 = lane & 31;
    if (g.splits > 1) {
        float* P = g.part + (long)split * g.M * g.N;
#pragma unroll
        for (int i = 0; i < 2; ++i)
#pragma unroll
            for (int j = 0; j < 2; ++j) {
                const int col = n0 + wn * 64 + j * 32 + l32;
#pragma unroll
                for (int r = 0; r < 16; ++r) {
                    const int row = m0 + wm * 64 + i * 32 + (r & 3) + 8 * (r >> 2) + 4 * half;
                    if (row < g.M && col < g.N) P[(long)row * g.N + col] = acc[i][j][r];
                }
            }
        return;
    }
#pragma unroll
    for (int i = 0; i < 2; ++i) {
#pragma unroll
        for (int j = 0; j < 2; ++j) {
            const int col = n0 + wn * 64 + j * 32 + l32;
            if (col >= g.N) continue;
            const float bv = g.bias ? g.bias[col] : 0.f;
#pragma unroll
            for (int r = 0; r < 16; ++r) {
                const int row = m0 + wm * 64 + i * 32 + (r & 3) + 8 * (r >> 2) + 4 * half;
                if (row >= g.M) continue;
                const long orow = g.c_rows ? (long)g.c_rows[row] : (long)row;
                if (orow < 0) continue;
                if (g.out_bf16) {
                    bf16_store_epilogue(g, orow, col, acc[i][j][r], bv);
                    continue;
                }
                float v = apply_act(acc[i][j][r] + bv, g.act);
                float* cp = g.C + orow * (long)g.ldc + col;
                if (g.accumulate) v += *cp;
                *cp = v;
            }
        }
    }
}

__global__ __launch_bounds__(256) void splitk_reduce_kernel(GemmBf16Args g) {
    const long i = (long)blockIdx.x * 256 + threadIdx.x;
    if (i >= (long)g.M * g.N) return;
    const int row = (int)(i / g.N), col = (int)(i % g.N);
    float v = 0.f;
    for (int sp = 0; sp < g.splits; ++sp) v += g.part[(long)sp * g.M * g.N + i];
    const long orow = g.c_rows ? (long)g.c_rows[row] : (long)row;
    if (orow < 0) return;
    if (g.out_bf16) {
        bf16_store_epilogue(g, orow, col, v, g.bias ? g.bias[col] : 0.f);
        return;
    }
    v = apply_act(v + (g.bias ? g.bias[col] : 0.f), g.act);
    float* cp = g.C + orow * g.ldc + col;
    if (g.accumulate) v += *cp;
    *cp = v;
}

__global__ __launch_bounds__(256) void splitk_reduce4_kernel(GemmBf16Args g) {
    const int col = (blockIdx.x * 256 + threadIdx.x) * 4;
    const int row = blockIdx.y;
    if (col >= g.N) return;
    const long i = (long)row * g.N + col;
    const long mn = (long)g.M * g.N;
    const long orow = g.c_rows ? (long)g.c_rows[row] : (long)row;
    float bv[4] = {0.f, 0.f, 0.f, 0.f};
    if (g.bias)
#pragma unroll
        for (int e = 0; e < 4; ++e) bv[e] = g.bias[col + e];
    float4 v = make_float4(0.f, 0.f, 0.f, 0.f);
    for (int sp0 = 0; sp0 < g.splits; sp0 += 8) {
        float4 p[8];
#pragma unroll
        for (int j = 0; j < 8; ++j)
            if (sp0 + j < g.splits) p[j] = *reinterpret_cast<const float4*>(g.part + (sp0 + j) * mn + i);
#pragma unroll
        for (int j = 0; j < 8; ++j)
            if (sp0 + j < g.splits) { v.x += p[j].x; v.y += p[j].y; v.z += p[j].z; v.w += p[j].w; }
    }
    if (orow < 0) return;
    const float r[4] = {v.x, v.y, v.z, v.w};
#pragma unroll
    for (int e = 0; e < 4; ++e) {
        if (g.out_bf16) {
            bf16_store_epilogue(g, orow, col + e, r[e], bv[e]);
            continue;
        }
        float x = apply_act(r[e] + bv[e], g.act);
        float* cp = g.C + orow * g.ldc + col + e;
        if (g.accumulate) x += *cp;
        *cp = x;
    }
}

static void launch_splitk_reduce(const GemmBf16Args& g, hipStream_t s) {
    if (g.N % 4 == 0 && g.M <= 65535 && (reinterpret_cast<uintptr_t>(g.part) & 15) == 0) {
        hipLaunchKernelGGL(splitk_reduce4_kernel, dim3((unsigned)((g.N / 4 + 255) / 256), (unsigned)g.M), dim3(256), 0, s, g);
        return;
    }
    const long n = (long)g.M * g.N;
    hipLaunchKernelGGL(splitk_reduce_kernel, dim3((unsigned)((n + 255) / 256)), dim3(256), 0, s, g);
}

constexpr int PP_M = 256, PP_N = 256, PP_K = 32, PP_NST = 4;
constexpr int PP_STAGE = (PP_M + PP_N) * PP_K;
constexpr int PP_LDS = PP_NST * PP_STAGE * 2;

__device__ __forceinline__ bf16x8_v pp_frag(const uint16_t* lds, int r, int kc) {
    return *reinterpret_cast<const bf16x8_v*>(lds + r * PP_K + ((kc ^ ((r >> 2) & 3)) * 8));
}

__device__ __forceinline__ void pp_issue(int p, const uint16_t* A, long lda, int m0, int mmax, const uint16_t* W,
                                         long ldw, int n0, int nmax, int k0, uint16_t* st, int grp, int wg, int lane) {
    const int R = grp * 128 + (wg * 2 + (p >> 1)) * 16;
    const int r = R + (lane >> 2);
    const int j = (lane & 3) ^ ((r >> 2) & 3);
    if ((p & 1) == 0) {
        const long ra = min(m0 + r, mmax);
        __builtin_amdgcn_global_load_lds(reinterpret_cast<const void*>(A + ra * lda + k0 + j * 8),
                                         (lds_void*)(st + R * PP_K), 16, 0, 0);
    } else {
        const long rw = min(n0 + r, nmax);
        __builtin_amdgcn_global_load_lds(reinterpret_cast<const void*>(W + rw * ldw + k0 + j * 8),
                                         (lds_void*)(st + PP_M * PP_K + R * PP_K), 16, 0, 0);
    }
}

__device__ __forceinline__ void pp_wait_n(int n) {
    if (n >= 8) asm volatile("s_waitcnt vmcnt(8)" ::: "memory");
    else if (n >= 6) asm volatile("s_waitcnt vmcnt(6)" ::: "memory");
    else if (n >= 4) asm volatile("s_waitcnt vmcnt(4)" ::: "memory");
    else if (n >= 2) asm volatile("s_waitcnt vmcnt(2)" ::: "memory");
    else asm volatile("s_waitcnt vmcnt(0)" ::: "memory");
}

__device__ __forceinline__ void pp_barrier() {
    __builtin_amdgcn_sched_barrier(0);
    __builtin_amdgcn_s_barrier();
    asm volatile("" ::: "memory");
    __builtin_amdgcn_sched_barrier(0);
}

#define PP_STAMP(var)                                                                           \
    if (STAMPS) {                                                                               \
        __builtin_amdgcn_sched_barrier(0);                                                      \
        asm volatile("s_memtime %0\n\ts_waitcnt lgkmcnt(0)" : "=s"(var)::"memory");          \
        __builtin_amdgcn_sched_barrier(0);                                                      \
    }

__device__ __forceinline__ float pp_rope(float x, float pt, float cs, float sn, bool lo) {
#pragma clang fp contract(off)
    const float rot = lo ? -pt : pt;
    const float a = x * cs;
    const float b = rot * sn;
    return a + b;
}

template <bool STAMPS>
__global__ __launch_bounds__(512, 1) void gemm_bf16_pp_kernel(GemmBf16Args g) {
    extern __shared__ __attribute__((aligned(16))) uint16_t pp_smem[];
    const int lane = threadIdx.x & 63;
    const int wave = __builtin_amdgcn_readfirstlane(threadIdx.x >> 6);
    const int wr = wave >> 2, wc = wave & 3;
    const int ntn = (g.N + PP_N - 1) / PP_N;
    const int nwg = gridDim.x;
    const int orig = blockIdx.x, xcd = orig & 7, q = nwg >> 3, rr = nwg & 7;
    const int tile = (xcd < rr ? xcd * (q + 1) : rr * (q + 1) + (xcd - rr) * q) + (orig >> 3);
    int bm, bn;
    tile_coords(tile, (g.M + PP_M - 1) / PP_M, ntn, g.group_m, bm, bn);
    const int m0 = bm * PP_M, n0 = bn * PP_N;
    const uint16_t* A = reinterpret_cast<const uint16_t*>(g.A);
    const uint16_t* W = reinterpret_cast<const uint16_t*>(g.W);
    f32x16 acc[4][2];
#pragma unroll
    for (int i = 0; i < 4; ++i)
#pragma unroll
        for (int j = 0; j < 2; ++j)
#pragma unroll
            for (int r = 0; r < 16; ++r) acc[i][j][r] = 0.f;
    const int nk = g.K / PP_K;
    auto issue = [&](int p, int kt) {
        pp_issue(p, A, g.lda, m0, g.M - 1, W, g.ldw, n0, g.N - 1, kt * PP_K, pp_smem + (kt & 3) * PP_STAGE, wr, wc, lane);
    };
    unsigned long long p0 = 0, rt0 = 0;
    if (STAMPS) {
        asm volatile("s_memtime %0\n\ts_waitcnt lgkmcnt(0)" : "=s"(p0)::"memory");
        asm volatile("s_memrealtime %0\n\ts_waitcnt lgkmcnt(0)" : "=s"(rt0)::"memory");
    }
    for (int kt = 0; kt < 3 && kt < nk; ++kt)
#pragma unroll
        for (int p = 0; p < 4; ++p) issue(p, kt);
    pp_wait_n(4 * min(2, nk - 1));
    pp_barrier();
    if (wr == 1) pp_barrier();
    unsigned long long seg[8] = {0, 0, 0, 0, 0, 0, 0, 0}, sa = 0, sb = 0, sc = 0, sd = 0, se = 0, sf = 0, sh = 0, si = 0, s0 = 0;
    PP_STAMP(s0);
    for (int t = 0; t < nk; ++t) {
        const bool more = t + 3 < nk;
        PP_STAMP(sa);
        PP_STAMP(sb);
        const uint16_t* As = pp_smem + (t & 3) * PP_STAGE;
        const uint16_t* Bs = As + PP_M * PP_K;
        bf16x8_v af[2][4], bfv[2][2];
#pragma unroll
        for (int ks = 0; ks < 2; ++ks) {
            const int kc = ks * 2 + (lane >> 5);
#pragma unroll
            for (int j = 0; j < 2; ++j) bfv[ks][j] = pp_frag(Bs, wc * 64 + j * 32 + (lane & 31), kc);
#pragma unroll
            for (int i = 0; i < 4; ++i) af[ks][i] = pp_frag(As, wr * 128 + i * 32 + (lane & 31), kc);
        }
        asm volatile("s_waitcnt lgkmcnt(0)" ::: "memory");
        PP_STAMP(sc);
        if (wr == 1 && t + 1 < nk) pp_wait_n(t + 2 < nk ? 4 : 0);
        PP_STAMP(sd);
        pp_barrier();
        PP_STAMP(se);
        __builtin_amdgcn_s_setprio(1);
#pragma unroll
        for (int ks = 0; ks < 2; ++ks)
#pragma unroll
            for (int i = 0; i < 4; ++i) {
#pragma unroll
                for (int j = 0; j < 2; ++j)
                    acc[i][j] = __builtin_amdgcn_mfma_f32_32x32x16_bf16(af[ks][i], bfv[ks][j], acc[i][j], 0, 0, 0);
                const int m = ks * 4 + i;
                if (m % 2 == 1) {
                    if (more) issue(m / 2, t + 3);
                    __builtin_amdgcn_sched_barrier(0);
                }
            }
        __builtin_amdgcn_s_setprio(0);
        PP_STAMP(sf);
        if (wr == 0 && t + 1 < nk) pp_wait_n((t + 2 < nk ? 4 : 0) + (more ? 4 : 0));
        PP_STAMP(sh);
        pp_barrier();
        PP_STAMP(si);
        if (STAMPS) {
            seg[0] += sb - sa; seg[1] += sc - sb; seg[2] += sd - sc; seg[3] += se - sd;
            seg[4] += sf - se; seg[5] += sh - sf; seg[6] += si - sh;
        }
    }
    if (wr == 0) pp_barrier();
    const int half = lane >> 5, l32 = lane & 31;
    uint16_t* ep = pp_smem + wave * (128 * 64);
    if (g.swiglu) {
        if (n0 + wc * 64 >= g.N) return;
        const int gc = n0 + wc * 64 + l32, uc = gc + 32;
        const float bg = g.bias ? g.bias[gc] : 0.f, bu = g.bias ? g.bias[uc] : 0.f;
#pragma unroll
        for (int i = 0; i < 4; ++i) {
#pragma unroll
            for (int r = 0; r < 16; ++r) {
                const int row = i * 32 + (r & 3) + 8 * (r >> 2) + 4 * half;
                float gv = rnd_bf16(acc[i][0][r]), uv = rnd_bf16(acc[i][1][r]);
                if (g.bias) {
                    gv = rnd_bf16(gv + bg);
                    uv = rnd_bf16(uv + bu);
                }
                const float ex = rnd_bf16(expf(-gv));
                const float sv = rnd_bf16(gv / rnd_bf16(1.0f + ex));
                const __bf16 hv = (__bf16)(sv * uv);
                ep[row * 32 + l32] = *reinterpret_cast<const uint16_t*>(&hv);
            }
        }
        asm volatile("s_waitcnt lgkmcnt(0)" ::: "memory");
        __builtin_amdgcn_wave_barrier();
        __bf16* H = reinterpret_cast<__bf16*>(g.C);
        const int hc = (n0 + wc * 64) / 2;
#pragma unroll 4
        for (int it = 0; it < 8; ++it) {
            const int row = it * 16 + (lane >> 2), ch = lane & 3;
            const int grow = m0 + wr * 128 + row;
            const u32x4 q = *reinterpret_cast<const u32x4*>(ep + row * 32 + ch * 8);
            if (grow < g.M) *reinterpret_cast<u32x4*>(H + (long)grow * g.ldc + hc + ch * 8) = q;
        }
        return;
    }
#pragma unroll
    for (int j = 0; j < 2; ++j) {
        const int col = n0 + wc * 64 + j * 32 + l32;
        const float bv = (g.bias && col < g.N) ? g.bias[col] : 0.f;
#pragma unroll
        for (int i = 0; i < 4; ++i) {
#pragma unroll
            for (int r = 0; r < 16; ++r) {
                const int row = i * 32 + (r & 3) + 8 * (r >> 2) + 4 * half;
                float v = rnd_bf16(acc[i][j][r]);
                if (g.bias) v = rnd_bf16(v + bv);
                const int c = j * 32 + l32;
                const int cs = (((c >> 3) ^ (((row >> 2) & 1) << 2)) << 3) | (c & 7);
                const __bf16 hv = (__bf16)v;
                ep[row * 64 + cs] = *reinterpret_cast<const uint16_t*>(&hv);
            }
        }
    }
    asm volatile("s_waitcnt lgkmcnt(0)" ::: "memory");
    __builtin_amdgcn_wave_barrier();
    __bf16* C = reinterpret_cast<__bf16*>(g.C);
    if (g.rope_cos && n0 < g.rope_cols) {
        __builtin_amdgcn_s_barrier();
        asm volatile("" ::: "memory");
        const uint16_t* pe = pp_smem + (wr * 4 + (wc ^ 1)) * (128 * 64);
        const int d0 = (wc & 1) * 64;
#pragma unroll 2
        for (int it = 0; it < 16; ++it) {
            const int row = it * 8 + (lane >> 3), ch = lane & 7;
            const int off = row * 64 + ((ch ^ (((row >> 2) & 1) << 2)) << 3);
            const u32x4 q = *reinterpret_cast<const u32x4*>(ep + off);
            const u32x4 pq = *reinterpret_cast<const u32x4*>(pe + off);
            const int grow = m0 + wr * 128 + row;
            if (grow >= g.M) continue;
            const float* ct = g.rope_cos + (long)grow * 128 + d0 + ch * 8;
            const float* st = g.rope_sin + (long)grow * 128 + d0 + ch * 8;
            const float4 c0 = *reinterpret_cast<const float4*>(ct), c1 = *reinterpret_cast<const float4*>(ct + 4);
            const float4 s0 = *reinterpret_cast<const float4*>(st), s1 = *reinterpret_cast<const float4*>(st + 4);
            const float cs[8] = {c0.x, c0.y, c0.z, c0.w, c1.x, c1.y, c1.z, c1.w};
            const float sn[8] = {s0.x, s0.y, s0.z, s0.w, s1.x, s1.y, s1.z, s1.w};
            const uint16_t* xv = reinterpret_cast<const uint16_t*>(&q);
            const uint16_t* pv = reinterpret_cast<const uint16_t*>(&pq);
            u32x4 o;
#pragma unroll
            for (int e = 0; e < 4; ++e) {
                const float a0 = pp_rope(__uint_as_float((uint32_t)xv[2 * e] << 16), __uint_as_float((uint32_t)pv[2 * e] << 16),
                                         cs[2 * e], sn[2 * e], d0 == 0);
                const float a1 = pp_rope(__uint_as_float((uint32_t)xv[2 * e + 1] << 16),
                                         __uint_as_float((uint32_t)pv[2 * e + 1] << 16), cs[2 * e + 1], sn[2 * e + 1], d0 == 0);
                const __bf16 h0 = (__bf16)a0, h1 = (__bf16)a1;
                o[e] = (uint32_t)*reinterpret_cast<const uint16_t*>(&h0) | ((uint32_t)*reinterpret_cast<const uint16_t*>(&h1) << 16);
            }
            *reinterpret_cast<u32x4*>(C + (long)grow * g.ldc + n0 + wc * 64 + ch * 8) = o;
        }
        return;
    }
#pragma unroll 4
    for (int it = 0; it < 16; ++it) {
        const int row = it * 8 + (lane >> 3), ch = lane & 7;
        const u32x4 q = *reinterpret_cast<const u32x4*>(ep + row * 64 + ((ch ^ (((row >> 2) & 1) << 2)) << 3));
        const int grow = m0 + wr * 128 + row, gcol = n0 + wc * 64 + ch * 8;
        if (grow >= g.M || gcol >= g.N) continue;
        __bf16* cp = C + (long)grow * g.ldc + gcol;
        const uint16_t* qv = reinterpret_cast<const uint16_t*>(&q);
        if (gcol + 8 <= g.N && !g.accumulate) {
            *reinterpret_cast<u32x4*>(cp) = q;
            continue;
        }
        u32x4 cv = gcol + 8 <= g.N ? *reinterpret_cast<const u32x4*>(cp) : u32x4{0, 0, 0, 0};
        uint16_t* cw = reinterpret_cast<uint16_t*>(&cv);
#pragma unroll
        for (int e = 0; e < 8; ++e) {
            if (gcol + e >= g.N) break;
            float v = __uint_as_float((uint32_t)qv[e] << 16);
            if (g.accumulate) {
                const float cold = gcol + 8 <= g.N ? __uint_as_float((uint32_t)cw[e] << 16) : (float)cp[e];
                v = rnd_bf16(cold + v);
            }
            const __bf16 hv = (__bf16)v;
            cw[e] = *reinterpret_cast<const uint16_t*>(&hv);
        }
        if (gcol + 8 <= g.N) *reinterpret_cast<u32x4*>(cp) = cv;
        else
            for (int e = 0; e < 8 && gcol + e < g.N; ++e) reinterpret_cast<uint16_t*>(cp)[e] = cw[e];
    }
    if (STAMPS) {
        unsigned long long e1 = 0, rt1 = 0;
        asm volatile("s_waitcnt vmcnt(0)" ::: "memory");
        asm volatile("s_memtime %0\n\ts_waitcnt lgkmcnt(0)" : "=s"(e1)::"memory");
        asm volatile("s_memrealtime %0\n\ts_waitcnt lgkmcnt(0)" : "=s"(rt1)::"memory");
        if (lane == 0 && blockIdx.x < 64) {
            seg[7] = si - s0;
            unsigned long long* o = g.stamps + ((long)blockIdx.x * 8 + wave) * 12;
            for (int k = 0; k < 8; ++k) o[k] = seg[k];
            o[8] = s0 - p0; o[9] = e1 - si; o[10] = e1 - p0; o[11] = rt1 - rt0;
        }
    }
}

static bool gemm_pp_on() {
    static const int v = getenv("DSOCR_GEMM_PP") ? atoi(getenv("DSOCR_GEMM_PP")) : 1;
    return v != 0;
}

int gemm_bf16_splits(int M, int N, int K) {
    const int tiles = ((M + TB_M - 1) / TB_M) * ((N + TB_N - 1) / TB_N);
    const int nk = K / TB_K;
    int sp = 1;
    while (tiles * sp < 256 && nk / (sp * 2) >= 8) sp *= 2;
    return sp;
}

void launch_gemm_bf16(const GemmBf16Args& g0, hipStream_t s) {
    GemmBf16Args g = g0;
    if (g.M <= 0 || g.N <= 0) return;
    if (g.K % TB_K || g.lda % 8 || g.ldw % 8 || (reinterpret_cast<uintptr_t>(g.A) & 15) ||
        (reinterpret_cast<uintptr_t>(g.W) & 15))
        throw std::runtime_error("EINVAL: gemm_bf16 needs K % 64 == 0 and 16-byte aligned rows");
    if (g.splits < 1 || !g.part) g.splits = 1;
    g.group_m = gemm_group_m(g.group_m);
    const long pp_tiles = (long)((g.M + PP_M - 1) / PP_M) * ((g.N + PP_N - 1) / PP_N);
    if (g.swiglu && (g.splits != 1 || g.K % PP_K || !g.out_bf16 || g.act || g.c_rows || g.accumulate || g.N % 64 ||
                     g.ldc % 8 || (reinterpret_cast<uintptr_t>(g.C) & 15)))
        throw std::runtime_error("EINVAL: the SwiGLU-pair GEMM needs one K slice, K % 32, N % 64, bf16 out, 16-byte rows");
    if (g.rope_cos && (g.swiglu || g.splits != 1 || g.K % PP_K || !g.out_bf16 || g.act || g.c_rows || g.accumulate ||
                       g.rope_cols % PP_N || g.rope_cols > g.N || g.ldc % 8 || (reinterpret_cast<uintptr_t>(g.C) & 15) ||
                       !g.rope_sin))
        throw std::runtime_error("EINVAL: the rotary GEMM epilogue needs one K slice, K % 32, bf16 out, q|k columns "
                                 "in whole 256-column tiles, 16-byte rows");
    if (g.swiglu || g.rope_cos || (g.splits == 1 && g.K % PP_K == 0 && g.out_bf16 && !g.act && !g.c_rows && g.ldc % 8 == 0 &&
                     (reinterpret_cast<uintptr_t>(g.C) & 15) == 0 &&
                     (g.variant == 3 || (g.variant == 0 && gemm_pp_on() && pp_tiles >= 256)))) {
        static bool attr = false;
        if (!attr) {
            const void* fns[2] = {reinterpret_cast<const void*>(gemm_bf16_pp_kernel<false>),
                                  reinterpret_cast<const void*>(gemm_bf16_pp_kernel<true>)};
            for (const void* f : fns)
                if (hipFuncSetAttribute(f, hipFuncAttributeMaxDynamicSharedMemorySize, PP_LDS) != hipSuccess)
                    throw std::runtime_error("gemm_bf16_pp: cannot reserve 128 KiB of LDS");
            attr = true;
        }
        const dim3 grid((unsigned)pp_tiles), blk(512);
        if (g.stamps) hipLaunchKernelGGL((gemm_bf16_pp_kernel<true>), grid, blk, PP_LDS, s, g);
        else hipLaunchKernelGGL((gemm_bf16_pp_kernel<false>), grid, blk, PP_LDS, s, g);
        return;
    }
    const int tiles = ((g.M + TB_M - 1) / TB_M) * ((g.N + TB_N - 1) / TB_N);
    if (g.variant == 2) hipLaunchKernelGGL(gemm_bf16_nt_kernel<2>, dim3(tiles * g.splits), dim3(256), 0, s, g);
    else hipLaunchKernelGGL(gemm_bf16_nt_kernel<1>, dim3(tiles * g.splits), dim3(256), 0, s, g);
    if (g.splits > 1) launch_splitk_reduce(g, s);
}

constexpr int FX_M = 128, FX_N = 128, FX_K = 32;
constexpr int FX_AS = FX_M * FX_K;
constexpr int FX_WS = FX_N * FX_K;

__device__ __forceinline__ bf16x8_v fx_pack(const float* v) {
    bf16x8_v r;
#pragma unroll
    for (int j = 0; j < 8; ++j) r[j] = (__bf16)v[j];
    return r;
}

template <bool F16W, bool W22 = F16W, int NST = 2, int BN = FX_N>
__global__ __launch_bounds__(256, 2) void gemm_f32a_nt_kernel(GemmBf16Args g) {
    constexpr int WN = W22 ? 2 : 1, WM = 4 / WN;
    constexpr int TI = FX_M / WM / 32, TJ = BN / WN / 32;
    constexpr int WS = BN * FX_K;
    __shared__ __attribute__((aligned(16))) float a_lds[NST * FX_AS];
    __shared__ __attribute__((aligned(16))) uint16_t w_lds[NST * WS];
    const int tid = threadIdx.x, lane = tid & 63, wave = tid >> 6;
    const int wm = wave / WN, wn = wave % WN;
    const int ntn = (g.N + BN - 1) / BN;
    const int nwg = gridDim.x;
    const int orig = blockIdx.x, xcd = orig & 7, q = nwg >> 3, rr = nwg & 7;
    const int wgid = (xcd < rr ? xcd * (q + 1) : rr * (q + 1) + (xcd - rr) * q) + (orig >> 3);
    const int split = wgid % g.splits, tile = wgid / g.splits;
    int bm, bn;
    tile_coords(tile, (g.M + FX_M - 1) / FX_M, ntn, g.group_m, bm, bn);
    const int m0 = bm * FX_M, n0 = bn * BN;
    const float* A = reinterpret_cast<const float*>(g.A);
    const uint16_t* W = reinterpret_cast<const uint16_t*>(g.W);
    f32x16 acc[TI][TJ];
#pragma unroll
    for (int i = 0; i < TI; ++i)
#pragma unroll
        for (int j = 0; j < TJ; ++j)
#pragma unroll
            for (int r = 0; r < 16; ++r) acc[i][j][r] = 0.f;
    const int nk_all = g.K / FX_K;
    const int kbeg = (int)((long)nk_all * split / g.splits), kend = (int)((long)nk_all * (split + 1) / g.splits);
    const int nk = kend - kbeg;
    auto issue = [&](int kt) {
        const int k0 = (kbeg + kt) * FX_K;
        float* as = a_lds + (NST == 1 ? 0 : (kt & 1) * FX_AS);
        uint16_t* ws_ = w_lds + (NST == 1 ? 0 : (kt & 1) * WS);
#pragma unroll
        for (int i = 0; i < 4; ++i) {
            const int R = (wave * 4 + i) * 8;
            const int r = R + (lane >> 3);
            const int j = (lane & 7) ^ ((r >> 1) & 7);
            const long row = min(m0 + r, g.M - 1);
            __builtin_amdgcn_global_load_lds(reinterpret_cast<const void*>(A + row * g.lda + k0 + j * 4),
                                             (lds_void*)(as + R * FX_K), 16, 0, 0);
        }
#pragma unroll
        for (int i = 0; i < BN / 64; ++i) {
            const int R = (wave * (BN / 64) + i) * 16;
            const int r = R + (lane >> 2);
            const int j = (lane & 3) ^ ((r >> 2) & 3);
            const long row = min(n0 + r, g.N - 1);
            __builtin_amdgcn_global_load_lds(reinterpret_cast<const void*>(W + row * g.ldw + k0 + j * 8),
                                             (lds_void*)(ws_ + R * FX_K), 16, 0, 0);
        }
    };
    if (NST == 2 && nk > 0) issue(0);
    for (int kt = 0; kt < nk; ++kt) {
        if (NST == 1) issue(kt);
        asm volatile("s_waitcnt vmcnt(0)" ::: "memory");
        __builtin_amdgcn_s_barrier();
        asm volatile("" ::: "memory");
        if (NST == 2 && kt + 1 < nk) issue(kt + 1);
        const float* As = a_lds + (NST == 1 ? 0 : (kt & 1) * FX_AS);
        const uint16_t* Ws = w_lds + (NST == 1 ? 0 : (kt & 1) * WS);
#pragma unroll
        for (int ks = 0; ks < FX_K / 16; ++ks) {
            const int kc = ks * 2 + (lane >> 5);
            bf16x8_v bfv[TJ], blo[TJ];
#pragma unroll
            for (int j = 0; j < TJ; ++j) {
                const int r = wn * (BN / WN) + j * 32 + (lane & 31);
                if constexpr (F16W) {
                    const uint4 raw = *reinterpret_cast<const uint4*>(Ws + r * FX_K + ((kc ^ ((r >> 2) & 3)) * 8));
                    float wv[8], wh[8], wl[8];
                    unpack8<f16_t>(raw, wv);
#pragma unroll
                    for (int e = 0; e < 8; ++e) {
                        wh[e] = (float)(__bf16)wv[e];
                        wl[e] = wv[e] - wh[e];
                    }
                    bfv[j] = fx_pack(wh);
                    blo[j] = fx_pack(wl);
                } else {
                    bfv[j] = *reinterpret_cast<const bf16x8_v*>(Ws + r * FX_K + ((kc ^ ((r >> 2) & 3)) * 8));
                }
            }
#pragma unroll
            for (int i = 0; i < TI; ++i) {
                const int r = wm * (FX_M / WM) + i * 32 + (lane & 31);
                const int sw = (r >> 1) & 7;
                const float4 lo4 = *reinterpret_cast<const float4*>(As + r * FX_K + (((2 * kc) ^ sw) * 4));
                const float4 hi4 = *reinterpret_cast<const float4*>(As + r * FX_K + (((2 * kc + 1) ^ sw) * 4));
                const float av[8] = {lo4.x, lo4.y, lo4.z, lo4.w, hi4.x, hi4.y, hi4.z, hi4.w};
                float h[8], m[8], l[8];
#pragma unroll
                for (int e = 0; e < 8; ++e) {
                    h[e] = (float)(__bf16)av[e];
                    const float r1 = av[e] - h[e];
                    m[e] = (float)(__bf16)r1;
                    l[e] = r1 - m[e];
                }
                const bf16x8_v ph = fx_pack(h), pm = fx_pack(m), pl = fx_pack(l);
#pragma unroll
                for (int j = 0; j < TJ; ++j) {
                    if constexpr (F16W) {
                        acc[i][j] = __builtin_amdgcn_mfma_f32_32x32x16_bf16(pl, bfv[j], acc[i][j], 0, 0, 0);
                        acc[i][j] = __builtin_amdgcn_mfma_f32_32x32x16_bf16(pm, blo[j], acc[i][j], 0, 0, 0);
                        acc[i][j] = __builtin_amdgcn_mfma_f32_32x32x16_bf16(pm, bfv[j], acc[i][j], 0, 0, 0);
                        acc[i][j] = __builtin_amdgcn_mfma_f32_32x32x16_bf16(ph, blo[j], acc[i][j], 0, 0, 0);
                        acc[i][j] = __builtin_amdgcn_mfma_f32_32x32x16_bf16(ph, bfv[j], acc[i][j], 0, 0, 0);
                    } else {
                        acc[i][j] = __builtin_amdgcn_mfma_f32_32x32x16_bf16(pl, bfv[j], acc[i][j], 0, 0, 0);
                        acc[i][j] = __builtin_amdgcn_mfma_f32_32x32x16_bf16(pm, bfv[j], acc[i][j], 0, 0, 0);
                        acc[i][j] = __builtin_amdgcn_mfma_f32_32x32x16_bf16(ph, bfv[j], acc[i][j], 0, 0, 0);
                    }
                }
            }
        }
        asm volatile("s_waitcnt lgkmcnt(0)" ::: "memory");
        if (NST == 1) {
            __builtin_amdgcn_s_barrier();
            asm volatile("" ::: "memory");
        }
    }
    const int half = lane >> 5, l32 = lane & 31;
    if (g.splits > 1) {
        float* P = g.part + (long)split * g.M * g.N;
#pragma unroll
        for (int i = 0; i < TI; ++i)
#pragma unroll
            for (int j = 0; j < TJ; ++j) {
                const int col = n0 + wn * (BN / WN) + j * 32 + l32;
#pragma unroll
                for (int r = 0; r < 16; ++r) {
                    const int row = m0 + wm * (FX_M / WM) + i * 32 + (r & 3) + 8 * (r >> 2) + 4 * half;
                    if (row < g.M && col < g.N) P[(long)row * g.N + col] = acc[i][j][r];
                }
            }
        return;
    }
#pragma unroll
    for (int i = 0; i < TI; ++i) {
#pragma unroll
        for (int j = 0; j < TJ; ++j) {
            const int col = n0 + wn * (BN / WN) + j * 32 + l32;
            if (col >= g.N) continue;
            const float bv = g.bias ? g.bias[col] : 0.f;
#pragma unroll
            for (int r = 0; r < 16; ++r) {
                const int row = m0 + wm * (FX_M / WM) + i * 32 + (r & 3) + 8 * (r >> 2) + 4 * half;
                if (row >= g.M) continue;
                const long orow = g.c_rows ? (long)g.c_rows[row] : (long)row;
                if (orow < 0) continue;
                float v = apply_act(acc[i][j][r] + bv, g.act);
                float* cp = g.C + orow * (long)g.ldc + col;
                if (g.accumulate) v += *cp;
                *cp = v;
            }
        }
    }
}

int gemm_f32a_splits(int M, int N, int K) {
    const int tiles = ((M + FX_M - 1) / FX_M) * ((N + FX_N - 1) / FX_N);
    const int nk = K / FX_K;
    int sp = 1;
    while (tiles * sp < 512 && nk / (sp * 2) >= 2) sp *= 2;
    return sp;
}

bool gemm_f32a_ok(const GemmBf16Args& g) {
    return g.K % FX_K == 0 && g.lda % 4 == 0 && g.ldw % 8 == 0 && (reinterpret_cast<uintptr_t>(g.A) & 15) == 0 &&
           (reinterpret_cast<uintptr_t>(g.W) & 15) == 0 && !g.out_bf16;
}

static int gemm_nst_env() {
    static const int v = getenv("DSOCR_GEMM_NST") ? atoi(getenv("DSOCR_GEMM_NST")) : 1;
    return v;
}

void launch_gemm_f32a(const GemmBf16Args& g0, hipStream_t s) {
    GemmBf16Args g = g0;
    if (!g.variant) g.variant = gemm_nst_env();
    if (g.M <= 0 || g.N <= 0) return;
    if (!gemm_f32a_ok(g)) throw std::runtime_error("EINVAL: gemm_f32a needs K % 32 == 0 and 16-byte aligned rows");
    if (g.splits < 1 || !g.part) g.splits = 1;
    g.group_m = gemm_group_m(g.group_m);
    const int tiles = ((g.M + FX_M - 1) / FX_M) * ((g.N + FX_N - 1) / FX_N);
    if (g.w_f16) hipLaunchKernelGGL((gemm_f32a_nt_kernel<true>), dim3(tiles * g.splits), dim3(256), 0, s, g);
    else if (g.variant == 2) hipLaunchKernelGGL((gemm_f32a_nt_kernel<false, false, 2>), dim3(tiles * g.splits), dim3(256), 0, s, g);
    else hipLaunchKernelGGL((gemm_f32a_nt_kernel<false, false, 1>), dim3(tiles * g.splits), dim3(256), 0, s, g);
    if (g.splits > 1) launch_splitk_reduce(g, s);
}

constexpr int GX_N = 128, GX_K = 32;

template <bool F16W, int GM>
__global__ __launch_bounds__(256) void gemm_f32a_grp_kernel(GemmArgs g) {
    constexpr int GX_M = GM, WM = GM == 32 ? 1 : 2, WN = 4 / WM, TI = GM / WM / 32, TJ = GX_N / WN / 32;
    constexpr int AI = GM / 32;
    __shared__ __attribute__((aligned(16))) float a_lds[2 * GX_M * GX_K];
    __shared__ __attribute__((aligned(16))) uint16_t w_lds[2 * GX_N * GX_K];
    const int tid = threadIdx.x, lane = tid & 63, wave = tid >> 6;
    const int t = blockIdx.y;
    int cnt = 0;
    if (lane < g.groups) cnt = g.group_off[lane + 1] - g.group_off[lane];
    const int nt = (cnt + GX_M - 1) / GX_M;
    int pre = nt;
#pragma unroll
    for (int d = 1; d < 64; d <<= 1) {
        const int o = __shfl_up(pre, d);
        if (lane >= d) pre += o;
    }
    const unsigned long long hit = __ballot(lane < g.groups && pre > t);
    if (!hit) return;
    const int grp = __builtin_ctzll(hit);
    const int m_begin = __shfl(g.group_off[min(lane, g.groups - 1)], grp);
    const int rows = __shfl(cnt, grp);
    const int mt = t - (__shfl(pre, grp) - __shfl(nt, grp));
    const int m0 = mt * GX_M, n0 = blockIdx.x * GX_N;
    const uint16_t* W = reinterpret_cast<const uint16_t*>(g.W) + (long)grp * g.w_group_stride;
    const float* bias = g.bias ? g.bias + (long)grp * g.bias_group_stride : nullptr;
    const float* a_src[AI];
#pragma unroll
    for (int i = 0; i < AI; ++i) {
        const int ar = (wave * AI + i) * 8 + (lane >> 3);
        const int aj = (lane & 7) ^ ((ar >> 1) & 7);
        const int arr = m_begin + min(m0 + ar, rows - 1);
        a_src[i] = g.A + (long)(g.a_rows ? g.a_rows[arr] : arr) * g.lda + aj * 4;
    }
    const uint16_t* w_src[2];
#pragma unroll
    for (int i = 0; i < 2; ++i) {
        const int r = (wave * 2 + i) * 16 + (lane >> 2);
        const int j = (lane & 3) ^ ((r >> 2) & 3);
        w_src[i] = W + (long)min(n0 + r, g.N - 1) * g.ldw + j * 8;
    }
    auto issue = [&](int kt) {
        const int k0 = kt * GX_K;
        float* as = a_lds + (kt & 1) * GX_M * GX_K;
        uint16_t* ws_ = w_lds + (kt & 1) * GX_N * GX_K;
#pragma unroll
        for (int i = 0; i < AI; ++i)
            __builtin_amdgcn_global_load_lds(reinterpret_cast<const void*>(a_src[i] + k0),
                                             (lds_void*)(as + (wave * AI + i) * 8 * GX_K), 16, 0, 0);
#pragma unroll
        for (int i = 0; i < 2; ++i)
            __builtin_amdgcn_global_load_lds(reinterpret_cast<const void*>(w_src[i] + k0),
                                             (lds_void*)(ws_ + (wave * 2 + i) * 16 * GX_K), 16, 0, 0);
    };
    const int wm = wave / WN, wn = wave % WN;
    f32x16 acc[TI][TJ];
#pragma unroll
    for (int i = 0; i < TI; ++i)
#pragma unroll
        for (int j = 0; j < TJ; ++j)
#pragma unroll
            for (int r = 0; r < 16; ++r) acc[i][j][r] = 0.f;
    const int nk = g.K / GX_K;
    issue(0);
    for (int kt = 0; kt < nk; ++kt) {
        asm volatile("s_waitcnt vmcnt(0)" ::: "memory");
        __builtin_amdgcn_s_barrier();
        asm volatile("" ::: "memory");
        if (kt + 1 < nk) issue(kt + 1);
        const float* As = a_lds + (kt & 1) * GX_M * GX_K;
        const uint16_t* Ws = w_lds + (kt & 1) * GX_N * GX_K;
#pragma unroll
        for (int ks = 0; ks < GX_K / 16; ++ks) {
            const int kc = ks * 2 + (lane >> 5);
            bf16x8_v bfv[TJ], blo[TJ];
#pragma unroll
            for (int j = 0; j < TJ; ++j) {
                const int r = wn * (GX_N / WN) + j * 32 + (lane & 31);
                if constexpr (F16W) {
                    const uint4 raw = *reinterpret_cast<const uint4*>(Ws + r * GX_K + ((kc ^ ((r >> 2) & 3)) * 8));
                    float wv[8], wh[8], wl[8];
                    unpack8<f16_t>(raw, wv);
#pragma unroll
                    for (int e = 0; e < 8; ++e) {
                        wh[e] = (float)(__bf16)wv[e];
                        wl[e] = wv[e] - wh[e];
                    }
                    bfv[j] = fx_pack(wh);
                    blo[j] = fx_pack(wl);
                } else {
                    bfv[j] = *reinterpret_cast<const bf16x8_v*>(Ws + r * GX_K + ((kc ^ ((r >> 2) & 3)) * 8));
                }
            }
#pragma unroll
            for (int i = 0; i < TI; ++i) {
            const int r = wm * (GX_M / WM) + i * 32 + (lane & 31);
            const int sw = (r >> 1) & 7;
            const float4 lo4 = *reinterpret_cast<const float4*>(As + r * GX_K + (((2 * kc) ^ sw) * 4));
            const float4 hi4 = *reinterpret_cast<const float4*>(As + r * GX_K + (((2 * kc + 1) ^ sw) * 4));
            const float av[8] = {lo4.x, lo4.y, lo4.z, lo4.w, hi4.x, hi4.y, hi4.z, hi4.w};
            float h[8], m[8], l[8];
#pragma unroll
            for (int e = 0; e < 8; ++e) {
                h[e] = (float)(__bf16)av[e];
                const float r1 = av[e] - h[e];
                m[e] = (float)(__bf16)r1;
                l[e] = r1 - m[e];
            }
            const bf16x8_v ph = fx_pack(h), pm = fx_pack(m), pl = fx_pack(l);
#pragma unroll
            for (int j = 0; j < TJ; ++j) {
                if constexpr (F16W) {
                    acc[i][j] = __builtin_amdgcn_mfma_f32_32x32x16_bf16(pl, bfv[j], acc[i][j], 0, 0, 0);
                    acc[i][j] = __builtin_amdgcn_mfma_f32_32x32x16_bf16(pm, blo[j], acc[i][j], 0, 0, 0);
                    acc[i][j] = __builtin_amdgcn_mfma_f32_32x32x16_bf16(pm, bfv[j], acc[i][j], 0, 0, 0);
                    acc[i][j] = __builtin_amdgcn_mfma_f32_32x32x16_bf16(ph, blo[j], acc[i][j], 0, 0, 0);
                    acc[i][j] = __builtin_amdgcn_mfma_f32_32x32x16_bf16(ph, bfv[j], acc[i][j], 0, 0, 0);
                } else {
                    acc[i][j] = __builtin_amdgcn_mfma_f32_32x32x16_bf16(pl, bfv[j], acc[i][j], 0, 0, 0);
                    acc[i][j] = __builtin_amdgcn_mfma_f32_32x32x16_bf16(pm, bfv[j], acc[i][j], 0, 0, 0);
                    acc[i][j] = __builtin_amdgcn_mfma_f32_32x32x16_bf16(ph, bfv[j], acc[i][j], 0, 0, 0);
                }
            }
            }
        }
        asm volatile("s_waitcnt lgkmcnt(0)" ::: "memory");
    }
    const int half = lane >> 5, l32 = lane & 31;
#pragma unroll
    for (int j = 0; j < TJ; ++j) {
        const int col = n0 + wn * (GX_N / WN) + j * 32 + l32;
        if (col >= g.N) continue;
        const float bv = bias ? bias[col] : 0.f;
#pragma unroll
        for (int i = 0; i < TI; ++i) {
#pragma unroll
            for (int r = 0; r < 16; ++r) {
                const int row = m0 + wm * (GX_M / WM) + i * 32 + (r & 3) + 8 * (r >> 2) + 4 * half;
                if (row >= rows) continue;
                const long orow = g.c_rows ? (long)g.c_rows[m_begin + row] : (long)(m_begin + row);
                if (orow < 0) continue;
                float v = apply_act(acc[i][j][r] + bv, g.act);
                float* cp = g.C + orow * (long)g.ldc + col;
// ... 31 lines not shown
```

deepseek-ocr.rs_amd/csrc/kernels/kernels.hpp:

```cpp
#pragma once
#include <hip/hip_runtime.h>
#include <math.h>
#include <stdint.h>

namespace dsocr {

enum WDType : int { WDT_BF16 = 0, WDT_F16 = 1 };

struct QMat {
    const void* q = nullptr;
    const void* d = nullptr;
    int qtype = 0;
};

constexpr long SPAN_SLOTS = 16384;
void launch_span_chain_fold(const unsigned long long* slots, int nreg, unsigned long long* rec, const int* step, int cap,
                            unsigned long long* tmark, hipStream_t s);
void launch_span_reduce(unsigned long long* slots, unsigned long long* rec, const int* step, int cap, const int* ids,
                        int n_ids, hipStream_t s);
struct ProfEvents {
    hipEvent_t start = nullptr, stop = nullptr;
};
ProfEvents& prof_events();
enum Act : int { ACT_NONE = 0, ACT_GELU_ERF = 1, ACT_QUICK_GELU = 2, ACT_SILU = 3 };

struct GemmBf16Args {
    int M = 0, N = 0, K = 0;
    const void* A = nullptr; long lda = 0;
    const void* W = nullptr; long ldw = 0;
    const float* bias = nullptr;
    float* C = nullptr; long ldc = 0;
    const int* c_rows = nullptr;
    int act = 0, accumulate = 0;
    int splits = 1; float* part = nullptr;
    int out_bf16 = 0;
    int w_f16 = 0;
    int variant = 0;
    int group_m = -1;
    int swiglu = 0;
    const float* rope_cos = nullptr;
    const float* rope_sin = nullptr;
    int rope_cols = 0;
    unsigned long long* stamps = nullptr;
};
void launch_gemm_bf16(const GemmBf16Args& g, hipStream_t s);
int gemm_bf16_splits(int M, int N, int K);
bool gemm_f32a_ok(const GemmBf16Args& g);
int gemm_f32a_splits(int M, int N, int K);
void launch_gemm_f32a(const GemmBf16Args& g, hipStream_t s);

struct GemmArgs {
    int M = 0, N = 0, K = 0;
    const float* A = nullptr;
    int lda = 0;
    const int* a_rows = nullptr;
    const void* W = nullptr;
    int ldw = 0;
    int wdtype = WDT_BF16;
    long w_group_stride = 0;
    const float* bias = nullptr;
    long bias_group_stride = 0;
    float* C = nullptr;
    int ldc = 0;
    const int* c_rows = nullptr;
    int act = 0;
    int accumulate = 0;
    const int* group_off = nullptr;
    int groups = 1;
    int max_group_rows = 0;
};
void launch_gemm(const GemmArgs& g, hipStream_t s);
bool gemm_f32a_grouped_ok(const GemmArgs& g);
void launch_gemm_f32a_grouped(const GemmArgs& g, hipStream_t s, int tile_rows = 0);

void launch_router_topk(const float* logits, int T, int E, int topk, int softmax_scoring, int norm_topk,
                        float scaling, int* topk_ids, float* topk_w, hipStream_t s);
void launch_moe_group(const int* topk_ids, int T, int topk, int E, int* eoff, int* arow, int* apos, int* scratch,
                      hipStream_t s);
void launch_moe_combine(const float* y, const int* apos, const float* topk_w, const float* shared, int T, int topk,
                        int H, float* out, int accumulate, hipStream_t s);
void launch_silu_mul(const float* g, int ldg, int I, int rows, float* h, int ldh, hipStream_t s);

void launch_layernorm(const float* x, int ldx, float* y, int ldy, const int* out_rows, int rows, int cols,
                      const float* w, const float* b, float eps, hipStream_t s);
void launch_rmsnorm(const float* x, int ldx, float* y, int ldy, int rows, int cols, const float* w, float eps,
                    hipStream_t s);

struct AttnView {
    const float* ptr = nullptr;
    long row_stride = 0, head_stride = 0;
    const long* seq_off = nullptr;
};
struct AttnArgs {
    AttnView q, k, v;
    float* o = nullptr;
    long o_row_stride = 0, o_head_stride = 0;
    const long* o_seq_off = nullptr;
    int n_seq = 0, L = 0;
    const int* seq_len = nullptr;
    int heads = 0, kv_heads = 0, hd = 0;
    float scale = 1.f;
    int causal = 0;
    const float* relbias = nullptr;
    int rel_h = 0, rel_w = 0;
    float* part = nullptr;
    size_t part_floats = 0;
};
void launch_attention(const AttnArgs& a, hipStream_t s);
size_t attention_causal_part_floats(int n_seq, int heads, int L, int hd);
struct AttnBf16Args {
    const uint16_t* q = nullptr; const uint16_t* k = nullptr; const uint16_t* v = nullptr;
    long q_rs = 0, q_hs = 0, k_rs = 0, k_hs = 0, v_rs = 0, v_hs = 0;
    void* o = nullptr; long o_rs = 0, o_hs = 0; int o_bf16 = 0;
    int n_seq = 0, L = 0, heads = 0, kv_heads = 0, hd = 0;
    float scale = 1.f;
    int pv_planes = 3;
};
void launch_attention_bf16(const AttnBf16Args& a, hipStream_t s);
void launch_sam_relbias(const float* q, long q_row_stride, int n_seq, int gh, int gw, int heads, int hd,
                        const float* Rh, const float* Rw, float* out, hipStream_t s);
struct RopeKvArgs {
    float* qkv = nullptr; long ld = 0; int rows = 0;
    const int* row_page = nullptr; const int* row_pos = nullptr;
    int heads = 0, kv_heads = 0, hd = 0, rope_dim = 0, use_mla = 0;
    const float* cos = nullptr; const float* sin = nullptr;
    float* kc = nullptr; float* vc = nullptr; long page_stride = 0, head_stride = 0;
};
void launch_rope_kv(const RopeKvArgs& a, hipStream_t s);

struct AttnPrefixArgs {
    const float* q = nullptr; const float* k = nullptr; const float* v = nullptr;
    float* o = nullptr;
    long ldq = 0, ldk = 0, ldv = 0, ldo = 0;
    int n_seq = 0, L = 0, prefix = 0, heads = 0, kv_heads = 0, hd = 0;
    float scale = 1.f;
};
bool attention_prefix_ok(const AttnPrefixArgs& a);
void launch_attention_prefix(const AttnPrefixArgs& a, hipStream_t s);

struct AttnPastArgs {
    AttnView q, k, v;
    float* o = nullptr;
    long o_row_stride = 0, o_head_stride = 0;
    const long* o_seq_off = nullptr;
    int n_seq = 0;
    const int* past = nullptr;
    const int* n_q = nullptr;
    int max_q = 0, max_total = 0;
    int heads = 0, kv_heads = 0, hd = 0;
    float scale = 1.f;
    float* part = nullptr;
    size_t part_floats = 0;
};
size_t attention_past_part_floats(int n_seq, int heads, int max_q, int max_total, int hd);
bool attention_past_ok(const AttnPastArgs& a);
void launch_attention_past(const AttnPastArgs& a, hipStream_t s);
bool attention_chunk_ok(const AttnPastArgs& a);
void launch_attention_chunk(const AttnPastArgs& a, hipStream_t s);

void launch_ocr2_build_seq(const float* feat, const float* query, int n, int P, int D, float* out, hipStream_t s);
void launch_ocr2_rope(float* x, long ld, long rows, int L, int n_heads, int hd, const float* cos_t, const float* sin_t,
                      hipStream_t s);
void launch_ocr2_take_queries(const float* src, int n, int P, int D, float* dst, hipStream_t s);

void launch_dots_rmsnorm(const void* x, int in_f32, long rows, int D, const float* w, float eps, void* y, hipStream_t s);
void launch_dots_layernorm(const void* x, long rows, int D, const float* w, const float* b, float eps, void* y,
                           hipStream_t s);
void launch_dots_swiglu(const void* gu, long N, int I, void* h, hipStream_t s);
void launch_dots_rope_qk(const void* qkv, long N, int heads, int hd, const float* cos_t, const float* sin_t, void* out,
                         hipStream_t s);
void launch_dots_gelu(void* x, long n, hipStream_t s);
void launch_dots_to_bf16(const float* x, long N, int D, long ldi, void* y, int ldo, hipStream_t s);
void launch_dots_bf16_to_f32(const void* x, long n, float* y, hipStream_t s);

void launch_patch_im2col(const float* img, int n, int H, int W, int ps, float* cols, hipStream_t s);
void launch_conv_im2col_nhwc(const float* x, int n, int H, int W, int C, int kh, int kw, int stride, int pad,
                             float* cols, hipStream_t s);
void launch_add_broadcast(float* x, const float* t, long rows_per_rep, int cols, int reps, hipStream_t s);
void launch_clip_embed(const float* sam, const float* cls, const float* pos, int n, int S, int C, float* out,
                       hipStream_t s);
void launch_concat_clip_sam(const float* clip, const float* sam, int n, int S, int C1, int C2, float* out,
                            hipStream_t s);
void launch_assemble_rows(const int* kind, const int* index, int rows, int H, const void* table, int table_dt,
                          const float* srcA, const float* srcB, const float* vecA, const float* vecB, float* dst,
                          long ld_dst, hipStream_t s);
void launch_trace_logits(const float* logits, int B, int V, long ld, const int* out_len, const int* done, float* trace,
                         long steps, hipStream_t s);
void launch_embed_tokens(const void* table, int table_dt, const int* ids, int n, int H, float* out, long ld,
                         hipStream_t s);
struct RowParams {
    double temperature = 0.0, top_p = -1.0;
    long top_k = 0;
    float rep_penalty = 1.f;
    int do_sample = 0, ngram = 0, eos = -1;
};
constexpr int ROWPAR_INTS = (int)(sizeof(RowParams) / sizeof(int));
static_assert(sizeof(RowParams) == 40 && sizeof(RowParams) % sizeof(int) == 0, "RowParams is staged as ints");
inline bool rep_penalty_active(float p) { return p > 0.f && fabsf(p - 1.0f) > 1.1920929e-07f; }
struct PenaltyRec {
    float frequency = 0.f, presence = 0.f;
    double ln_min_p = -INFINITY;
// ... 451 lines not shown
```

deepseek-ocr.rs_amd/csrc/kernels/norm.hip:

```cpp
#include "dev_common.hpp"
#include "kernels.hpp"

namespace dsocr {

__global__ __launch_bounds__(256) void layernorm_kernel(const float* x, int ldx, float* y, int ldy, const int* out_rows,
                                                        int rows, int cols, const float* w, const float* b, float eps) {
    const int lane = threadIdx.x & 63;
    const int r = blockIdx.x * 4 + (threadIdx.x >> 6);
    if (r >= rows) return;
    const float* xr = x + (long)r * ldx;
    const long orow = out_rows ? (long)out_rows[r] : (long)r;
    if (orow < 0) return;
    float* yr = y + orow * ldy;
    float s = 0.f;
    for (int c = lane * 4; c < cols; c += 256) {
        float4 v = *reinterpret_cast<const float4*>(xr + c);
        s += (v.x + v.y) + (v.z + v.w);
    }
    const float mean = wave_sum(s) / (float)cols;
    float q = 0.f;
    for (int c = lane * 4; c < cols; c += 256) {
        float4 v = *reinterpret_cast<const float4*>(xr + c);
        float a0 = v.x - mean, a1 = v.y - mean, a2 = v.z - mean, a3 = v.w - mean;
        q += (a0 * a0 + a1 * a1) + (a2 * a2 + a3 * a3);
    }
    const float var = wave_sum(q) / (float)cols;
    const float denom = sqrtf(var + eps);
    for (int c = lane * 4; c < cols; c += 256) {
        float4 v = *reinterpret_cast<const float4*>(xr + c);
        float4 wv = *reinterpret_cast<const float4*>(w + c);
        float4 bv = *reinterpret_cast<const float4*>(b + c);
        float4 o;
        o.x = (v.x - mean) / denom * wv.x + bv.x;
        o.y = (v.y - mean) / denom * wv.y + bv.y;
        o.z = (v.z - mean) / denom * wv.z + bv.z;
        o.w = (v.w - mean) / denom * wv.w + bv.w;
        *reinterpret_cast<float4*>(yr + c) = o;
    }
}

void launch_layernorm(const float* x, int ldx, float* y, int ldy, const int* out_rows, int rows, int cols,
                      const float* w, const float* b, float eps, hipStream_t s) {
    if (rows == 0) return;
    hipLaunchKernelGGL(layernorm_kernel, dim3((rows + 3) / 4), dim3(256), 0, s, x, ldx, y, ldy, out_rows, rows, cols,
                       w, b, eps);
}

__global__ __launch_bounds__(256) void rmsnorm_kernel(const float* x, int ldx, float* y, int ldy, int rows, int cols,
                                                      const float* w, float eps) {
    const int lane = threadIdx.x & 63;
    const int r = blockIdx.x * 4 + (threadIdx.x >> 6);
    if (r >= rows) return;
    const float* xr = x + (long)r * ldx;
    float* yr = y + (long)r * ldy;
    float q = 0.f;
    for (int c = lane * 4; c < cols; c += 256) {
        float4 v = *reinterpret_cast<const float4*>(xr + c);
        q += (v.x * v.x + v.y * v.y) + (v.z * v.z + v.w * v.w);
    }
    const float denom = sqrtf(wave_sum(q) / (float)cols + eps);
    for (int c = lane * 4; c < cols; c += 256) {
        float4 v = *reinterpret_cast<const float4*>(xr + c);
        float4 wv = *reinterpret_cast<const float4*>(w + c);
        float4 o;
        o.x = (v.x / denom) * wv.x;
        o.y = (v.y / denom) * wv.y;
        o.z = (v.z / denom) * wv.z;
        o.w = (v.w / denom) * wv.w;
        *reinterpret_cast<float4*>(yr + c) = o;
    }
}

void launch_rmsnorm(const float* x, int ldx, float* y, int ldy, int rows, int cols, const float* w, float eps,
                    hipStream_t s) {
    if (rows == 0) return;
    hipLaunchKernelGGL(rmsnorm_kernel, dim3((rows + 3) / 4), dim3(256), 0, s, x, ldx, y, ldy, rows, cols, w, eps);
}

}
```

deepseek-ocr.rs_amd/dsocr/_lib.py:

```python
from __future__ import annotations

import ctypes as C
import os

_HERE = os.path.dirname(os.path.abspath(__file__))
LIB_PATH = os.path.join(os.path.dirname(_HERE), "lib", "libdsocr.so")

OK, EINVAL, ENOENT, EDEVICE, ENOMEM, EINTERNAL = range(6)
STATUS_NAMES = {0: "OK", 1: "EINVAL", 2: "ENOENT", 3: "EDEVICE", 4: "ENOMEM", 5: "EINTERNAL"}
DTYPES = {"f32": 0, "f16": 1, "bf16": 2}


class DsocrError(RuntimeError):
    def __init__(self, status: int, message: str):
        super().__init__(f"{STATUS_NAMES.get(status, status)}: {message}")
        self.status = status
        self.message = message


class LoadArgs(C.Structure):
    _fields_ = [("config_path", C.c_char_p), ("weights_path", C.c_char_p), ("snapshot_path", C.c_char_p),
                ("device_ordinal", C.c_int), ("dtype", C.c_int), ("synthetic_seed", C.c_uint64)]


class VisionSettingsC(C.Structure):
    _fields_ = [("base_size", C.c_uint32), ("image_size", C.c_uint32), ("crop_mode", C.c_int)]


class DecodeParamsC(C.Structure):
    _fields_ = [("max_new_tokens", C.c_size_t), ("do_sample", C.c_int), ("temperature", C.c_double),
                ("top_p", C.c_double), ("top_k", C.c_size_t), ("repetition_penalty", C.c_float),
                ("no_repeat_ngram_size", C.c_size_t), ("seed", C.c_uint64), ("use_cache", C.c_int),
                ("eos_token_id", C.c_int64), ("ignore_eos", C.c_int), ("has_seed", C.c_int)]


class RequestC(C.Structure):
    _fields_ = [("input_ids", C.POINTER(C.c_int64)), ("image_mask", C.POINTER(C.c_uint8)),
                ("prompt_len", C.c_size_t), ("page", C.c_void_p), ("image_rows", C.POINTER(C.c_float)),
                ("n_image_rows", C.c_size_t)]


class ResultC(C.Structure):
    _fields_ = [("out_ids", C.POINTER(C.c_int64)), ("cap", C.c_size_t), ("n_out", C.c_size_t),
                ("status", C.c_int)]


class TimingsC(C.Structure):
    _fields_ = [("vision_prepare_ms", C.c_double), ("vision_compute_ms", C.c_double),
                ("decode_prefill_ms", C.c_double), ("decode_iterative_ms", C.c_double),
                ("decode_generate_ms", C.c_double), ("decode_steps", C.c_size_t), ("pages", C.c_size_t),
                ("vision_flops", C.c_double), ("prefill_flops", C.c_double)]


class KernelProfileC(C.Structure):
    _fields_ = [("avg_us", C.c_double), ("bytes", C.c_double), ("flops", C.c_double), ("launches", C.c_int),
                ("replay_us", C.c_double), ("ctx_us", C.c_double)]


class DecodeProfileC(C.Structure):
    _fields_ = [("moe_gateup", KernelProfileC), ("moe_down", KernelProfileC), ("attention", KernelProfileC),
                ("lm_head", KernelProfileC), ("experts_touched", C.c_int), ("tokens", C.c_int), ("kv_len", C.c_int),
                ("qkv", KernelProfileC), ("o_proj", KernelProfileC), ("router", KernelProfileC),
                ("layers_step", KernelProfileC), ("lm_head_screened", KernelProfileC),
                ("moe_gateup_kernel", C.c_char_p), ("moe_down_kernel", C.c_char_p)]


class SlotStatusC(C.Structure):
    _fields_ = [("slot", C.c_int32), ("done", C.c_int32), ("out_len", C.c_int32), ("n_new", C.c_int32)]


class SessionDescC(C.Structure):
    _fields_ = [("slots", C.c_size_t), ("active", C.c_size_t), ("max_context", C.c_size_t), ("out_cap", C.c_size_t),
                ("kv_cap", C.c_size_t), ("burst_cap", C.c_size_t), ("steps", C.c_size_t), ("flags", C.c_size_t)]


class LogprobsC(C.Structure):
    _fields_ = [("token_lp", C.POINTER(C.c_float)), ("top_id", C.POINTER(C.c_int64)), ("top_lp", C.POINTER(C.c_float)),
                ("cap", C.c_size_t), ("n", C.c_size_t)]


class LogitBiasC(C.Structure):
    _fields_ = [("ids", C.POINTER(C.c_int64)), ("values", C.POINTER(C.c_float)), ("n", C.c_size_t),
                ("allow_only", C.c_int)]


class StopSetC(C.Structure):
    _fields_ = [("ids", C.POINTER(C.c_int64)), ("lens", C.POINTER(C.c_size_t)), ("n", C.c_size_t)]


class StopHitC(C.Structure):
    _fields_ = [("seq", C.c_int32), ("match_len", C.c_int32)]


class PenaltiesC(C.Structure):
    _fields_ = [("frequency", C.c_float), ("presence", C.c_float), ("min_p", C.c_double)]


class NgramWindowC(C.Structure):
    _fields_ = [("ngram_size", C.c_int32), ("window", C.c_int32), ("whitelist", C.POINTER(C.c_int32)),
                ("n_whitelist", C.c_size_t)]


class GuidedC(C.Structure):
    _fields_ = [("n_states", C.c_int32), ("start", C.c_int32), ("accepting", C.POINTER(C.c_uint8)),
                ("row_ptr", C.POINTER(C.c_int32)), ("edge_tok", C.POINTER(C.c_int32)),
                ("edge_next", C.POINTER(C.c_int32))]


class GuidedResultC(C.Structure):
    _fields_ = [("state", C.c_int32), ("status", C.c_int32)]


class RowParamsC(C.Structure):
    _fields_ = [("do_sample", C.c_int), ("temperature", C.c_double), ("top_p", C.c_double), ("top_k", C.c_size_t),
                ("repetition_penalty", C.c_float), ("no_repeat_ngram_size", C.c_size_t), ("eos_token_id", C.c_int64)]


class ScreenStepsC(C.Structure):
    _fields_ = ([(n, C.c_int) for n in ("B", "V", "K", "wdtype", "steps", "probe")] +
                [("W", C.c_void_p), ("x", C.c_void_p), ("ldx", C.c_longlong), ("norm_w", C.c_void_p), ("eps", C.c_float),
                 ("ctx", C.c_void_p), ("ctx_cap", C.c_int), ("ctx_len", C.c_void_p), ("ngram", C.c_int), ("eos", C.c_int),
                 ("rows", C.POINTER(RowParamsC)), ("ban", C.c_void_p), ("ban_ld", C.c_int), ("out_cap", C.c_int),
                 ("table", C.c_void_p), ("table_dt", C.c_int), ("H", C.c_int)] +
                [(n, C.c_void_p) for n in ("out_tok", "ban_out", "ctx_out", "ctx_len_out", "out_ids", "out_len", "done",
                                           "kv_pos", "kv_len", "x_next", "blk_cnt", "blk_t", "cand", "cand_hi", "xn_out", "xn_gemv",
                                           "q", "scale", "bound", "qnorm", "qfrag")])


SESSION_PER_REQUEST = 1
SESSION_LOGPROBS = 2
SESSION_LOGIT_BIAS = 4
SESSION_STOP = 8
SESSION_PENALTIES = 16
SESSION_NGRAM_WINDOW = 32
MAX_NGRAM_WHITELIST = 32
SESSION_GUIDED = 64
MAX_STOP_SEQS = 16
MAX_STOP_LEN = 32
SESSION_ADMIT_PENDING = 0x100
MAX_TOP_LOGPROBS = 20


class DotsTimingsC(C.Structure):
    _fields_ = [("total_ms", C.c_double), ("patch_ms", C.c_double), ("blocks_ms", C.c_double),
                ("attention_ms", C.c_double), ("merger_ms", C.c_double), ("tokens", C.c_size_t), ("groups", C.c_size_t)]


LOAD_PACKED_EXPERTS = 1
STREAM_CB = C.CFUNCTYPE(None, C.c_size_t, C.POINTER(C.c_int64), C.c_void_p)

EXPORTS = [
    "dsocr_engine_load", "dsocr_engine_free", "dsocr_last_error", "dsocr_engine_info", "dsocr_prepare_page",
    "dsocr_page_free", "dsocr_page_to_device", "dsocr_page_info", "dsocr_page_pixels_view", "dsocr_image_embeddings", "dsocr_generate",
    "dsocr_generate_batch", "dsocr_last_timings", "dsocr_profile_decode", "dsocr_device_count", "dsocr_dev_alloc", "dsocr_dev_free",
    "dsocr_memcpy_h2d", "dsocr_memcpy_d2h", "dsocr_dev_sync", "dsocr_synth_bf16", "dsocr_resize_bicubic",
    "dsocr_k_gemm", "dsocr_k_gemm_f32a", "dsocr_k_gemm_grouped", "dsocr_k_gemv", "dsocr_k_layernorm", "dsocr_k_rmsnorm", "dsocr_k_attention", "dsocr_k_decode_attention", "dsocr_k_moe",
    "dsocr_k_sample_greedy", "dsocr_k_sample_stoch", "dsocr_k_dsq_dequant", "dsocr_prepare_page_device", "dsocr_page_read_device",
    "dsocr_generate_trace", "dsocr_k_moe_kernels", "dsocr_k_lmhead_screened",
    "dsocr_dots_load", "dsocr_dots_free", "dsocr_dots_info", "dsocr_dots_preprocess", "dsocr_dots_embed",
    "dsocr_dots_embed_device", "dsocr_dots_last_timings", "dsocr_k_attention_bf16", "dsocr_k_gemv_splitk",
    "dsocr_engine_set_spans", "dsocr_engine_spans", "dsocr_k_qkv_attention", "dsocr_k_poll_wait_fits",
    "dsocr_engine_set_persist_stamps", "dsocr_engine_persist_info",
    "dsocr_resize_catmull_rom",
    "dsocr_engine_load_flags", "dsocr_engine_packed_info", "dsocr_k_moe_packed", "dsocr_k_dsq_rows_dot",
    "dsocr_k_moe_ex", "dsocr_k_moe_route_kind", "dsocr_k_moe_prefill_route", "dsocr_k_moe_combine",
    "dsocr_k_gemm_bf16", "dsocr_k_dots_op",
    "dsocr_k_gemv_ex", "dsocr_k_gemv_kind", "dsocr_k_mm_swizzle", "dsocr_k_silu_mul",
    "dsocr_config_variant", "dsocr_engine_variant", "dsocr_prepare_page_variant", "dsocr_prepare_page_device_variant", "dsocr_k_attention_prefix",
    "dsocr_k_prefill_attention",
    "dsocr_session_open", "dsocr_session_admit", "dsocr_session_step", "dsocr_session_poll", "dsocr_session_retire",
    "dsocr_session_close", "dsocr_session_info", "dsocr_k_session_slot_move",
    "dsocr_session_open_ex", "dsocr_session_admit_params", "dsocr_session_head_steps", "dsocr_k_select_rows",
    "dsocr_generate_logprobs", "dsocr_session_logprobs", "dsocr_k_logprobs", "dsocr_k_logprobs_penalty",
    "dsocr_session_prefix_keep", "dsocr_session_admit_prefix", "dsocr_session_prefix_drop", "dsocr_session_prefix_stats",
    "dsocr_k_prefill_attention_past", "dsocr_k_session_prefix_copy",
    "dsocr_k_qkv_attention_layers",
    "dsocr_k_lmhead_screen_steps", "dsocr_k_lmhead_screen_grid",
    "dsocr_session_admit_begin", "dsocr_session_admit_advance", "dsocr_session_admit_cancel",
    "dsocr_session_admit_progress", "dsocr_k_attention_chunk",
    "dsocr_logit_bias_check", "dsocr_generate_logit_bias", "dsocr_session_stage_logit_bias", "dsocr_k_logit_bias",
    "dsocr_stop_set_check", "dsocr_generate_stop", "dsocr_session_stage_stop", "dsocr_session_stop_hit",
    "dsocr_stop_launches", "dsocr_k_stop_match", "dsocr_generate_stop_stream",
    "dsocr_penalties_check", "dsocr_generate_penalties", "dsocr_session_stage_penalties", "dsocr_k_out_penalty",
    "dsocr_k_sample_stoch_min_p",
    "dsocr_ngram_window_check", "dsocr_generate_ngram_window", "dsocr_session_stage_ngram_window",
    "dsocr_k_ngram_window",
    "dsocr_guided_check", "dsocr_generate_guided", "dsocr_session_stage_guided", "dsocr_session_guided_state",
    "dsocr_k_guided_mask", "dsocr_k_guided_advance",
]

VARIANT_OCR1, VARIANT_OCR2 = 0, 1

DOTS_RMSNORM, DOTS_LAYERNORM, DOTS_SWIGLU, DOTS_GELU, DOTS_ROPE_QK, DOTS_TO_BF16, DOTS_BF16_TO_F32 = range(7)

_lib = None


def lib():
    global _lib
    if _lib is not None:
        return _lib
    if not os.path.exists(LIB_PATH):
        raise DsocrError(EINTERNAL, f"libdsocr.so not built at {LIB_PATH}; run `python deepseek-ocr.rs_amd/build.py`")
    L = C.CDLL(LIB_PATH)
    vp, sz, i32, u32, f32, i64 = C.c_void_p, C.c_size_t, C.c_int, C.c_uint32, C.c_float, C.c_int64
    L.dsocr_last_error.restype = C.c_char_p
    L.dsocr_engine_load.argtypes = [C.POINTER(LoadArgs), C.POINTER(vp)]
    L.dsocr_engine_load_flags.argtypes = [C.POINTER(LoadArgs), u32, C.POINTER(vp)]
    L.dsocr_engine_packed_info.argtypes = [vp, C.POINTER(sz), C.POINTER(sz), C.POINTER(sz)]
    L.dsocr_engine_free.argtypes = [vp]
    L.dsocr_engine_free.restype = None
    L.dsocr_engine_info.argtypes = [vp, C.POINTER(sz), C.POINTER(sz), C.POINTER(i64), C.POINTER(sz)]
    L.dsocr_prepare_page.argtypes = [vp, u32, u32, C.POINTER(VisionSettingsC), C.POINTER(vp)]
    L.dsocr_page_free.argtypes = [vp]
    L.dsocr_engine_variant.argtypes = [vp, C.POINTER(i32)]
    L.dsocr_config_variant.argtypes = [C.c_char_p, C.POINTER(i32), C.POINTER(u32), C.POINTER(u32)]
    L.dsocr_prepare_page_variant.argtypes = [vp, u32, u32, C.POINTER(VisionSettingsC), i32, C.POINTER(vp)]
    L.dsocr_prepare_page_device_variant.argtypes = [vp, vp, u32, u32, C.POINTER(VisionSettingsC), C.POINTER(vp)]
    L.dsocr_k_attention_prefix.argtypes = [i32, i32, i32, i32, i32, i32, f32, vp, vp, vp, vp]
    L.dsocr_prepare_page_device.argtypes = [vp, vp, u32, u32, C.POINTER(VisionSettingsC), C.POINTER(vp)]
    L.dsocr_page_read_device.argtypes = [vp, vp, vp]
    L.dsocr_page_free.restype = None
    L.dsocr_page_to_device.argtypes = [vp, vp]
    L.dsocr_page_info.argtypes = [vp, C.POINTER(u32), C.POINTER(u32), C.POINTER(u32), C.POINTER(sz)]
    L.dsocr_page_pixels_view.argtypes = [vp, C.POINTER(vp), C.POINTER(u32), C.POINTER(vp), C.POINTER(u32)]
    L.dsocr_image_embeddings.argtypes = [vp, C.POINTER(vp), sz, vp, sz, C.POINTER(sz)]
    L.dsocr_generate.argtypes = [vp, C.POINTER(RequestC), C.POINTER(DecodeParamsC), STREAM_CB, vp, vp, sz,
                                 C.POINTER(sz)]
    L.dsocr_generate_batch.argtypes = [vp, sz, C.POINTER(RequestC), C.POINTER(DecodeParamsC), C.POINTER(ResultC)]
    L.dsocr_generate_trace.argtypes = [vp, sz, C.POINTER(RequestC), C.POINTER(DecodeParamsC), C.POINTER(ResultC), vp,
                                       sz]
    L.dsocr_k_attention_bf16.argtypes = [i32, i32, i32, i32, f32, vp, C.c_long, vp, C.c_long, i32]
    L.dsocr_k_gemm_bf16.argtypes = [i32, i32, i32, vp, C.c_long, vp, C.c_long, vp, vp, C.c_long, i32, i32, i32, i32, i32,
                                    vp, vp, i32]
    L.dsocr_k_dots_op.argtypes = [i32, C.c_long, i32, i32, C.c_long, vp, vp, vp, f32, vp]
    L.dsocr_dots_load.argtypes = [C.c_char_p, C.c_char_p, C.c_uint64, i32, C.POINTER(vp)]
    L.dsocr_dots_free.argtypes = [vp]
    L.dsocr_dots_free.restype = None
    L.dsocr_dots_info.argtypes = [vp, C.POINTER(sz), C.POINTER(sz), C.POINTER(sz), C.POINTER(sz)]
    L.dsocr_dots_preprocess.argtypes = [C.c_char_p, vp, u32, u32, vp, sz, C.POINTER(sz), C.POINTER(u32)]
    L.dsocr_dots_embed.argtypes = [vp, vp, u32, u32, vp, sz, C.POINTER(sz), C.POINTER(u32)]
    L.dsocr_dots_embed_device.argtypes = [vp, vp, u32, u32, u32, vp, i32]
    L.dsocr_dots_last_timings.argtypes = [vp, C.POINTER(DotsTimingsC)]
    L.dsocr_k_lmhead_screened.argtypes = [i32, i32, i32, vp, vp, f32, vp, vp, i32, vp]
    L.dsocr_k_lmhead_screen_steps.argtypes = [C.POINTER(ScreenStepsC)]
    L.dsocr_k_lmhead_screen_grid.argtypes = [i32, i32, i32, C.POINTER(i32), C.POINTER(C.c_longlong), C.POINTER(i32)]
    L.dsocr_k_moe_kernels.argtypes = [i32, i32, i32, i32, i32, i32, i32, C.POINTER(C.c_char_p), C.POINTER(C.c_char_p)]
    L.dsocr_last_timings.argtypes = [vp, C.POINTER(TimingsC)]
    L.dsocr_profile_decode.argtypes = [vp, i32, C.POINTER(DecodeProfileC)]
    L.dsocr_engine_set_spans.argtypes = [vp, i32]
    L.dsocr_engine_spans.argtypes = [vp, vp, sz, C.POINTER(sz), C.POINTER(sz), C.POINTER(sz)]
    L.dsocr_engine_set_persist_stamps.argtypes = [vp, i32]
    L.dsocr_engine_persist_info.argtypes = [vp, C.POINTER(i32), vp, sz, C.POINTER(sz), vp, sz, C.POINTER(sz)]
    L.dsocr_device_count.argtypes = [C.POINTER(i32)]
    L.dsocr_dev_alloc.argtypes = [sz, C.POINTER(vp)]
    L.dsocr_dev_free.argtypes = [vp]
    L.dsocr_memcpy_h2d.argtypes = [vp, vp, sz]
    L.dsocr_memcpy_d2h.argtypes = [vp, vp, sz]
    L.dsocr_synth_bf16.argtypes = [C.c_char_p, C.c_uint64, C.c_uint64, vp]
    L.dsocr_resize_bicubic.argtypes = [vp, u32, u32, vp, u32, u32]
    L.dsocr_resize_catmull_rom.argtypes = [vp, u32, u32, vp, u32, u32]
    L.dsocr_k_gemm.argtypes = [i32, i32, i32, vp, vp, i32, vp, vp, i32, i32]
    L.dsocr_k_gemm_f32a.argtypes = [i32, i32, i32, vp, vp, i32, vp, vp, i32, i32, i32]
    L.dsocr_k_gemm_grouped.argtypes = [i32, i32, i32, vp, i32, vp, vp, i32, C.c_longlong, vp, C.c_longlong, vp, i32, vp, i32,
                                       i32, vp, i32, i32, i32]
    L.dsocr_k_gemv.argtypes = [i32, i32, i32, vp, vp, f32, vp, i32, vp, vp, i32, i32]
    L.dsocr_k_gemv_splitk.argtypes = [i32, i32, i32, vp, vp, i32, vp, vp, i32]
    L.dsocr_k_gemv_ex.argtypes = [i32, i32, i32, vp, i32, vp, f32, vp, i32, i32, vp, vp, i32, i32, i32, i32,
                                  C.POINTER(C.c_char_p)]
    L.dsocr_k_gemv_kind.argtypes = [i32, i32, i32, i32, i32, i32, i32, i32, C.POINTER(C.c_char_p), C.POINTER(i32)]
    L.dsocr_k_mm_swizzle.argtypes = [i32, i32, vp, vp]
    L.dsocr_k_silu_mul.argtypes = [i32, i32, vp, i32, vp, i32]
    L.dsocr_k_layernorm.argtypes = [i32, i32, vp, vp, vp, f32, vp]
    L.dsocr_k_rmsnorm.argtypes = [i32, i32, vp, vp, f32, vp]
    L.dsocr_k_dsq_dequant.argtypes = [i32, vp, sz, sz, sz, vp]
    L.dsocr_k_attention.argtypes = [i32, i32, i32, i32, f32, i32, vp, vp, vp, vp, vp, vp, i32, i32]
    L.dsocr_k_decode_attention.argtypes = [i32, i32, i32, i32, i32, i32, f32, vp, vp, vp, vp, vp, vp, vp, i32]
    L.dsocr_k_prefill_attention.argtypes = [i32, i32, i32, i32, i32, i32, i32, f32, C.POINTER(i32), vp, vp, vp, vp, vp, vp,
                                            i32]
    L.dsocr_k_qkv_attention.argtypes = [i32, i32, i32, i32, i32, i32, f32, f32, vp, vp, vp, i32, vp, vp, vp, vp, vp, vp,
                                        vp, C.POINTER(i32)]
    L.dsocr_k_qkv_attention_layers.argtypes = [i32, i32, i32, i32, i32, i32, f32, f32, vp, vp, vp, i32, vp, vp, vp, vp,
                                               vp, vp, vp, vp, C.POINTER(i32)]
    L.dsocr_k_poll_wait_fits.argtypes = [C.c_long, i32, i32]
    L.dsocr_k_moe_packed.argtypes = [i32, i32, i32, i32, i32, i32, vp, vp, f32, vp, i32, vp, i32, vp, i32, vp, i32, vp,
                                     i32, f32, vp, vp, vp]
    L.dsocr_k_dsq_rows_dot.argtypes = [i32, sz, sz, vp, i32, vp, vp]
    L.dsocr_k_moe.argtypes = [i32, i32, i32, i32, i32, i32, vp, vp, f32, vp, vp, vp, vp, vp, i32, i32, f32, vp, vp, vp]
    L.dsocr_k_moe_ex.argtypes = L.dsocr_k_moe.argtypes + [i32, vp, vp]
    L.dsocr_k_moe_route_kind.argtypes = [i32, i32, i32, i32, i32, i32, i32, C.POINTER(C.c_char_p)]
    L.dsocr_k_moe_prefill_route.argtypes = [i32, i32, i32, vp, i32, i32, f32, vp, vp, vp, vp, vp]
    L.dsocr_k_moe_combine.argtypes = [i32, i32, i32, vp, vp, vp, vp, vp, i32]
    L.dsocr_k_sample_greedy.argtypes =[i32, i32, vp, vp, i32, vp, i32, f32, vp]
    L.dsocr_k_sample_stoch.argtypes = [i32, i32, vp, vp, i32, vp, i32, f32, C.c_double, C.c_size_t, C.c_double,
                                       C.c_uint64, i32, vp]
    L.dsocr_session_open.argtypes = [vp, sz, sz, C.POINTER(DecodeParamsC)]
    L.dsocr_session_admit.argtypes = [vp, C.POINTER(RequestC), sz, i32, C.c_uint64, C.POINTER(i32)]
    L.dsocr_session_open_ex.argtypes = [vp, sz, sz, C.POINTER(DecodeParamsC), u32]
    L.dsocr_session_admit_params.argtypes = [vp, C.POINTER(RequestC), C.POINTER(DecodeParamsC), C.POINTER(i32)]
    L.dsocr_session_head_steps.argtypes = [vp, C.POINTER(sz), C.POINTER(sz)]
    L.dsocr_k_select_rows.argtypes = [i32, i32, vp, vp, i32, vp, C.POINTER(RowParamsC), C.POINTER(C.c_uint64), i32, vp]
    L.dsocr_session_step.argtypes = [vp, sz, C.POINTER(SlotStatusC), sz, C.POINTER(sz), vp, sz, C.POINTER(sz)]
    L.dsocr_session_poll.argtypes = [vp, C.POINTER(SlotStatusC), sz, C.POINTER(sz), vp, sz, C.POINTER(sz)]
    L.dsocr_session_retire.argtypes = [vp, i32, vp, sz, C.POINTER(sz), C.POINTER(i32)]
    L.dsocr_session_close.argtypes = [vp]
    L.dsocr_session_info.argtypes = [vp, C.POINTER(SessionDescC)]
    L.dsocr_generate_logprobs.argtypes = [vp, sz, C.POINTER(RequestC), C.POINTER(DecodeParamsC), C.POINTER(ResultC), sz,
                                          C.POINTER(LogprobsC)]
    L.dsocr_session_logprobs.argtypes = [vp, i32, sz, sz, sz, vp, vp, vp]
    L.dsocr_session_prefix_keep.argtypes = [vp, i32, sz, C.POINTER(i32)]
    L.dsocr_session_admit_prefix.argtypes = [vp, i32, C.POINTER(RequestC), C.POINTER(DecodeParamsC), C.POINTER(i32)]
    L.dsocr_session_prefix_drop.argtypes = [vp, i32]
    L.dsocr_session_prefix_stats.argtypes = [vp, C.POINTER(sz), C.POINTER(sz), C.POINTER(sz), C.POINTER(sz)]
    L.dsocr_k_prefill_attention_past.argtypes = [i32, i32, i32, i32, i32, i32, i32, f32, C.POINTER(i32), C.POINTER(i32),
                                                 vp, vp, vp, vp, vp, vp]
    L.dsocr_session_admit_begin.argtypes = [vp, C.POINTER(RequestC), C.POINTER(DecodeParamsC), sz, C.POINTER(i32)]
    L.dsocr_session_admit_advance.argtypes = [vp, C.POINTER(i32), C.POINTER(i32)]
    L.dsocr_session_admit_cancel.argtypes = [vp]
    L.dsocr_session_admit_progress.argtypes = [vp, C.POINTER(i32), C.POINTER(sz), C.POINTER(sz), C.POINTER(sz),
                                               C.POINTER(i32), C.POINTER(sz)]
    L.dsocr_k_attention_chunk.argtypes = [i32, i32, i32, i32, i32, i32, i32, f32, C.POINTER(i32), C.POINTER(i32),
                                          vp, vp, vp, vp, vp, vp, i32, i32]
    L.dsocr_k_session_prefix_copy.argtypes = [i32, i32, i32, i32, i32, vp, vp, i32, i32, vp, i32]
    L.dsocr_k_logprobs.argtypes = [i32, i32, i32, vp, i32, vp, vp, vp, vp, vp]
    L.dsocr_k_logprobs_penalty.argtypes = [i32, i32, i32, vp, i32, vp, vp, vp, i32, vp, f32, vp, vp, vp]
    L.dsocr_k_session_slot_move.argtypes = [i32, i32, i32, i32, i32, vp, vp, vp, vp, vp, C.c_longlong, vp, vp,
                                            C.c_longlong, vp, vp, vp, vp, i32, vp, C.c_longlong, vp, i32, i32, i32]
    L.dsocr_logit_bias_check.argtypes = [C.POINTER(LogitBiasC), sz]
    L.dsocr_generate_logit_bias.argtypes = [vp, sz, C.POINTER(RequestC), C.POINTER(DecodeParamsC), C.POINTER(ResultC),
                                            C.POINTER(C.POINTER(LogitBiasC)), sz, C.POINTER(LogprobsC)]
    L.dsocr_session_stage_logit_bias.argtypes = [vp, C.POINTER(LogitBiasC)]
    L.dsocr_k_logit_bias.argtypes = [i32, i32, i32, i32, vp, vp, vp, vp, vp, vp, vp, vp, i32]
    L.dsocr_stop_set_check.argtypes = [C.POINTER(StopSetC), sz]
    L.dsocr_generate_stop.argtypes = [vp, sz, C.POINTER(RequestC), C.POINTER(DecodeParamsC), C.POINTER(ResultC),
                                      C.POINTER(C.POINTER(StopSetC)), C.POINTER(StopHitC),
                                      C.POINTER(C.POINTER(LogitBiasC)), sz, C.POINTER(LogprobsC)]
    L.dsocr_generate_stop_stream.argtypes = [vp, C.POINTER(RequestC), C.POINTER(DecodeParamsC), C.POINTER(StopSetC),
                                             STREAM_CB, vp, vp, sz, C.POINTER(sz), C.POINTER(StopHitC)]
    L.dsocr_session_stage_stop.argtypes = [vp, C.POINTER(StopSetC)]
    L.dsocr_session_stop_hit.argtypes = [vp, i32, C.POINTER(StopHitC)]
    L.dsocr_stop_launches.argtypes = [vp, C.POINTER(sz)]
    L.dsocr_k_stop_match.argtypes = [i32, i32, i32] + [vp] * 14
    L.dsocr_penalties_check.argtypes = [C.POINTER(PenaltiesC)]
    L.dsocr_generate_penalties.argtypes = [vp, sz, C.POINTER(RequestC), C.POINTER(DecodeParamsC), C.POINTER(ResultC),
                                           C.POINTER(C.POINTER(PenaltiesC)), C.POINTER(C.POINTER(StopSetC)),
                                           C.POINTER(StopHitC), C.POINTER(C.POINTER(LogitBiasC)), sz,
                                           C.POINTER(LogprobsC)]
    L.dsocr_session_stage_penalties.argtypes = [vp, C.POINTER(PenaltiesC)]
    L.dsocr_k_out_penalty.argtypes = [i32, i32, i32, vp, vp, i32, vp, C.POINTER(PenaltiesC)]
    L.dsocr_k_sample_stoch_min_p.argtypes = [i32, i32, vp, vp, i32, vp, i32, f32, C.c_double, C.c_size_t, C.c_double,
                                             vp, C.c_uint64, i32, vp]
    L.dsocr_ngram_window_check.argtypes = [C.POINTER(NgramWindowC), sz]
    L.dsocr_generate_ngram_window.argtypes = [vp, sz, C.POINTER(RequestC), C.POINTER(DecodeParamsC), C.POINTER(ResultC),
                                              C.POINTER(C.POINTER(NgramWindowC)), C.POINTER(C.POINTER(PenaltiesC)),
                                              C.POINTER(C.POINTER(StopSetC)), C.POINTER(StopHitC),
                                              C.POINTER(C.POINTER(LogitBiasC)), sz, C.POINTER(LogprobsC)]
    L.dsocr_session_stage_ngram_window.argtypes = [vp, C.POINTER(NgramWindowC)]
    L.dsocr_k_ngram_window.argtypes = [i32, i32, i32, vp, vp, i32, vp, C.POINTER(C.POINTER(NgramWindowC)), i32]
    L.dsocr_guided_check.argtypes = [C.POINTER(GuidedC), i32, C.c_longlong]
    L.dsocr_generate_guided.argtypes = [vp, sz, C.POINTER(RequestC), C.POINTER(DecodeParamsC), C.POINTER(ResultC),
                                        C.POINTER(C.POINTER(GuidedC)), C.POINTER(GuidedResultC),
                                        C.POINTER(C.POINTER(NgramWindowC)), C.POINTER(C.POINTER(PenaltiesC)),
                                        C.POINTER(C.POINTER(StopSetC)), C.POINTER(StopHitC),
                                        C.POINTER(C.POINTER(LogitBiasC)), sz, C.POINTER(LogprobsC)]
    L.dsocr_session_stage_guided.argtypes = [vp, C.POINTER(GuidedC)]
    L.dsocr_session_guided_state.argtypes = [vp, i32, C.POINTER(GuidedResultC)]
    L.dsocr_k_guided_mask.argtypes = [i32, i32, i32, i32, vp, C.POINTER(GuidedC), C.c_longlong, vp, vp, vp, vp]
    L.dsocr_k_guided_advance.argtypes = [i32, i32, C.POINTER(GuidedC), vp, vp, vp, vp]
    _lib = L
    return L


def check(status: int):
    if status != OK:
        msg = lib().dsocr_last_error()
        raise DsocrError(status, msg.decode() if msg else "")
```

include/dsocr.h:

```cpp
#ifndef DSOCR_H
#define DSOCR_H

#include <stddef.h>
#include <stdint.h>

#ifdef __cplusplus
extern "C" {
#endif

typedef enum {
    DSOCR_OK = 0,
    DSOCR_EINVAL = 1,
    DSOCR_ENOENT = 2,
    DSOCR_EDEVICE = 3,
    DSOCR_ENOMEM = 4,
    DSOCR_EINTERNAL = 5
} dsocr_status;

typedef enum { DSOCR_F32 = 0, DSOCR_F16 = 1, DSOCR_BF16 = 2 } dsocr_dtype;

typedef struct dsocr_engine dsocr_engine;
typedef struct dsocr_page_pixels dsocr_page_pixels;

typedef struct {
// ... 146 lines not shown

typedef struct {
    float frequency;
    float presence;
    double min_p;
} dsocr_penalties;
dsocr_status dsocr_penalties_check(const dsocr_penalties* pen);
dsocr_status dsocr_generate_penalties(dsocr_engine* e, size_t n, const dsocr_request* reqs,
                                      const dsocr_decode_params* params, dsocr_result* results,
                                      const dsocr_penalties* const* pen, const dsocr_stop_set* const* stops,
                                      dsocr_stop_hit* hits, const dsocr_logit_bias* const* bias, size_t top_k,
                                      dsocr_logprobs* lp);
dsocr_status dsocr_session_stage_penalties(dsocr_engine* e, const dsocr_penalties* pen);

#define DSOCR_MAX_NGRAM_WHITELIST 32
typedef struct {
    int32_t ngram_size;
    int32_t window;
    const int32_t* whitelist;
    size_t n_whitelist;
} dsocr_ngram_window;
dsocr_status dsocr_ngram_window_check(const dsocr_ngram_window* ngw, size_t vocab);
dsocr_status dsocr_generate_ngram_window(dsocr_engine* e, size_t n, const dsocr_request* reqs,
                                         const dsocr_decode_params* params, dsocr_result* results,
                                         const dsocr_ngram_window* const* ngw, const dsocr_penalties* const* pen,
                                         const dsocr_stop_set* const* stops, dsocr_stop_hit* hits,
                                         const dsocr_logit_bias* const* bias, size_t top_k, dsocr_logprobs* lp);
dsocr_status dsocr_session_stage_ngram_window(dsocr_engine* e, const dsocr_ngram_window* ngw);

#define DSOCR_MAX_GUIDED_STATES 1024
#define DSOCR_MAX_GUIDED_EDGES (1 << 20)
typedef struct {
    int32_t n_states, start;
    const uint8_t* accepting;
    const int32_t *row_ptr, *edge_tok, *edge_next;
} dsocr_guided;
typedef struct {
    int32_t state;
    int32_t status;
} dsocr_guided_result;
dsocr_status dsocr_guided_check(const dsocr_guided* g, int vocab, long long eos);
dsocr_status dsocr_generate_guided(dsocr_engine* e, size_t n, const dsocr_request* reqs,
                                   const dsocr_decode_params* params, dsocr_result* results,
                                   const dsocr_guided* const* guided, dsocr_guided_result* gres,
                                   const dsocr_ngram_window* const* ngw, const dsocr_penalties* const* pen,
                                   const dsocr_stop_set* const* stops, dsocr_stop_hit* hits,
                                   const dsocr_logit_bias* const* bias, size_t top_k, dsocr_logprobs* lp);
dsocr_status dsocr_session_stage_guided(dsocr_engine* e, const dsocr_guided* g);
dsocr_status dsocr_session_guided_state(dsocr_engine* e, int slot, dsocr_guided_result* out);

typedef struct {
    int32_t slot;
    int32_t done;
    int32_t out_len;
    int32_t n_new;
} dsocr_slot_status;
typedef struct {
    size_t slots, active, max_context, out_cap;
    size_t kv_cap;
    size_t burst_cap;
    size_t steps;
    size_t flags;
} dsocr_session_desc;
dsocr_status dsocr_session_open(dsocr_engine* e, size_t slots, size_t max_context, const dsocr_decode_params* params);
#define DSOCR_SESSION_PER_REQUEST 1u
#define DSOCR_SESSION_LOGPROBS 2u
#define DSOCR_SESSION_LOGIT_BIAS 4u
#define DSOCR_SESSION_STOP 8u
#define DSOCR_SESSION_PENALTIES 16u
#define DSOCR_SESSION_NGRAM_WINDOW 32u
#define DSOCR_SESSION_GUIDED 64u
dsocr_status dsocr_session_open_ex(dsocr_engine* e, size_t slots, size_t max_context, const dsocr_decode_params* params,
                                   uint32_t flags);
dsocr_status dsocr_session_admit(dsocr_engine* e, const dsocr_request* req, size_t max_new_tokens, int has_seed,
                                 uint64_t seed, int* slot);
dsocr_status dsocr_session_admit_params(dsocr_engine* e, const dsocr_request* req, const dsocr_decode_params* params,
                                        int* slot);
dsocr_status dsocr_session_head_steps(const dsocr_engine* e, size_t* screened, size_t* exact);
dsocr_status dsocr_session_step(dsocr_engine* e, size_t k, dsocr_slot_status* status, size_t cap_slots, size_t* n_slots,
                                int64_t* tokens, size_t cap_tokens, size_t* n_tokens);
dsocr_status dsocr_session_poll(dsocr_engine* e, dsocr_slot_status* status, size_t cap_slots, size_t* n_slots,
                                int64_t* tokens, size_t cap_tokens, size_t* n_tokens);
dsocr_status dsocr_session_retire(dsocr_engine* e, int slot, int64_t* out_ids, size_t cap, size_t* n_out,
                                  int* moved_from);
dsocr_status dsocr_session_logprobs(dsocr_engine* e, int slot, size_t first, size_t count, size_t top_k, float* token_lp,
                                    int64_t* top_id, float* top_lp);
#define DSOCR_MAX_PREFIX_ENTRIES 64
dsocr_status dsocr_session_prefix_keep(dsocr_engine* e, int slot, size_t rows, int* handle);
dsocr_status dsocr_session_admit_prefix(dsocr_engine* e, int handle, const dsocr_request* req,
                                        const dsocr_decode_params* params, int* slot);
dsocr_status dsocr_session_prefix_drop(dsocr_engine* e, int handle);
dsocr_status dsocr_session_prefix_stats(const dsocr_engine* e, size_t* entries, size_t* bytes, size_t* admissions,
                                        size_t* rows_reused);
#define DSOCR_SESSION_ADMIT_PENDING 0x100u
dsocr_status dsocr_session_admit_begin(dsocr_engine* e, const dsocr_request* req, const dsocr_decode_params* params,
                                       size_t chunk_rows, int* ticket);
dsocr_status dsocr_session_admit_advance(dsocr_engine* e, int* done, int* slot);
dsocr_status dsocr_session_admit_cancel(dsocr_engine* e);
dsocr_status dsocr_session_admit_progress(const dsocr_engine* e, int* pending, size_t* rows_done, size_t* rows_total,
                                          size_t* slices, int* vision_stage, size_t* chunk_attn_launches);
dsocr_status dsocr_session_close(dsocr_engine* e);
dsocr_status dsocr_session_info(const dsocr_engine* e, dsocr_session_desc* out);

typedef struct dsocr_kernel_profile {
    double avg_us;
    double bytes;
    double flops;
    int launches;
    double replay_us;
    double ctx_us;
} dsocr_kernel_profile;
typedef struct dsocr_decode_profile {
    dsocr_kernel_profile moe_gateup;
    dsocr_kernel_profile moe_down;
    dsocr_kernel_profile attention;
    dsocr_kernel_profile lm_head;
    int experts_touched;
    int tokens;
    int kv_len;
    dsocr_kernel_profile qkv;
    dsocr_kernel_profile o_proj;
    dsocr_kernel_profile router;
    dsocr_kernel_profile layers_step;
    dsocr_kernel_profile lm_head_screened;
    const char* moe_gateup_kernel;
    const char* moe_down_kernel;
} dsocr_decode_profile;
dsocr_status dsocr_profile_decode(dsocr_engine* e, int iters, dsocr_decode_profile* out);

dsocr_status dsocr_engine_set_spans(dsocr_engine* e, int mode);
dsocr_status dsocr_engine_spans(const dsocr_engine* e, uint64_t* out, size_t cap, size_t* kinds, size_t* layers,
                                size_t* steps);

dsocr_status dsocr_engine_set_persist_stamps(dsocr_engine* e, int mode);
dsocr_status dsocr_engine_persist_info(const dsocr_engine* e, int* used, double* durations, size_t cap_d,
                                       size_t* n_launches, uint64_t* stamps, size_t cap_s, size_t* n_stamps);

dsocr_status dsocr_device_count(int* n);
dsocr_status dsocr_dev_alloc(size_t bytes, void** ptr);
dsocr_status dsocr_dev_free(void* ptr);
dsocr_status dsocr_memcpy_h2d(void* dst, const void* src, size_t bytes);
dsocr_status dsocr_memcpy_d2h(void* dst, const void* src, size_t bytes);
dsocr_status dsocr_dev_sync(void);
dsocr_status dsocr_synth_bf16(const char* name, uint64_t seed, uint64_t n, uint16_t* out);
dsocr_status dsocr_resize_bicubic(const uint8_t* src, uint32_t sw, uint32_t sh, uint8_t* dst, uint32_t dw,
                                  uint32_t dh);
dsocr_status dsocr_resize_catmull_rom(const uint8_t* src, uint32_t sw, uint32_t sh, uint8_t* dst, uint32_t dw,
                                      uint32_t dh);

dsocr_status dsocr_k_gemm(int M, int N, int K, const float* A, const void* W, int wdtype, const float* bias, float* C,
                          int act, int accumulate);
dsocr_status dsocr_k_gemm_f32a(int M, int N, int K, const float* A, const void* W, int wdtype, const float* bias,
                               float* C, int act, int accumulate, int splits);
dsocr_status dsocr_k_gemm_grouped(int M, int N, int K, const float* A, int lda, const int* a_rows, const void* W,
                                  int wdtype, long long w_group_stride, const float* bias, long long bias_group_stride,
                                  float* C, int ldc, const int* c_rows, int act, int accumulate, const int* group_off,
                                  int groups, int max_group_rows, int kernel);
dsocr_status dsocr_k_gemv(int M, int N, int K, const float* x, const float* norm_w, float eps, const void* W,
                          int wdtype, const float* bias, float* y, int act, int accumulate);
dsocr_status dsocr_k_gemv_ex(int M, int N, int K, const float* x, int ldx, const float* norm_w, float eps,
                             const void* W, int ldw, int wdtype, const float* bias, float* y, int ldy, int act,
                             int accumulate, int swizzle, const char** kind);
dsocr_status dsocr_k_gemv_kind(int M, int N, int K, int ldw, int wdtype, int has_norm, int has_xn_out, int swizzle,
                               const char** kind, int* rows_per_launch);
dsocr_status dsocr_k_mm_swizzle(int N, int K, const void* w, void* out);
dsocr_status dsocr_k_silu_mul(int rows, int I, const float* g, int ldg, float* h, int ldh);
dsocr_status dsocr_k_gemv_splitk(int M, int N, int K, const float* x, const void* W, int wdtype, const float* bias,
                                 float* y, int accumulate);
dsocr_status dsocr_k_layernorm(int rows, int cols, const float* x, const float* w, const float* b, float eps,
                               float* y);
dsocr_status dsocr_k_dsq_dequant(int qtype, const void* src, size_t src_bytes, size_t out_dim, size_t in_dim,
                                 void* out_f16);
dsocr_status dsocr_k_rmsnorm(int rows, int cols, const float* x, const float* w, float eps, float* y);
dsocr_status dsocr_k_attention(int n_seq, int L, int heads, int hd, float scale, int causal, const float* q,
                               const float* k, const float* v, float* o, const float* relh, const float* relw, int gh,
                               int gw);
dsocr_status dsocr_k_attention_prefix(int n_seq, int L, int prefix, int heads, int kv_heads, int hd, float scale,
                                      const float* q, const float* k, const float* v, float* o);
dsocr_status dsocr_k_attention_bf16(int n_seq, int L, int heads, int hd, float scale, const void* qkv, long ld,
                                    void* o, long o_ld, int o_bf16);
dsocr_status dsocr_k_gemm_bf16(int M, int N, int K, const void* A, long lda, const void* W, long ldw, const float* bias,
                               void* C, long ldc, int out_bf16, int accumulate, int variant, int group_m, int swiglu,
                               const float* rope_cos, const float* rope_sin, int rope_cols);
enum {
    DSOCR_DOTS_RMSNORM = 0, DSOCR_DOTS_LAYERNORM = 1, DSOCR_DOTS_SWIGLU = 2, DSOCR_DOTS_GELU = 3,
    DSOCR_DOTS_ROPE_QK = 4, DSOCR_DOTS_TO_BF16 = 5, DSOCR_DOTS_BF16_TO_F32 = 6
};
dsocr_status dsocr_k_dots_op(int op, long rows, int cols, int aux, long ld, const void* x, const float* p0,
                             const float* p1, float eps, void* y);
dsocr_status dsocr_k_decode_attention(int B, int heads, int kv_heads, int hd, int rope_dim, int max_len, float scale,
                                      const float* qkv, const float* cos, const float* sin, float* kc, float* vc,
                                      const int* kv_pos, float* o, int prerot);
dsocr_status dsocr_k_prefill_attention(int B, int heads, int kv_heads, int hd, int rope_dim, int use_mla, int cap,
                                       float scale, const int* lens, float* qkv, const float* cos, const float* sin,
                                       float* kc, float* vc, float* o, int use_part);
dsocr_status dsocr_k_prefill_attention_past(int B, int heads, int kv_heads, int hd, int rope_dim, int use_mla, int cap,
                                            float scale, const int* past, const int* lens, float* qkv, const float* cos,
                                            const float* sin, float* kc, float* vc, float* o);
dsocr_status dsocr_k_attention_chunk(int B, int heads, int kv_heads, int hd, int rope_dim, int use_mla, int cap,
                                     float scale, const int* past, const int* lens, float* qkv, const float* cos,
                                     const float* sin, float* kc, float* vc, float* o, int page0, int pages);
#define DSOCR_HANDOFF_SENTINEL 0x7FBADBADu
dsocr_status dsocr_k_qkv_attention(int fused, int steps, int H, int heads, int hd, int max_len, float scale,
                                   float eps, const float* x, const float* norm_w, const void* Wqkv, int wdtype,
                                   const float* cos, const float* sin, float* kc, float* vc, const int* kv_pos,
                                   float* qkv_row, float* o, int* used_fused);
dsocr_status dsocr_k_qkv_attention_layers(int defer, int layers, int H, int heads, int hd, int max_len, float scale,
                                          float eps, const float* x, const float* norm_w, const void* Wqkv, int wdtype,
                                          const float* cos, const float* sin, float* kc, float* vc, const int* kv_pos,
                                          float* o, uint32_t* qkv_copies, uint32_t* part_copies, int* err_word);
int dsocr_k_poll_wait_fits(long waiting_blocks, int api_blocks_per_cu, int cus);
dsocr_status dsocr_k_moe(int T, int H, int E, int topk, int I, int Is, const float* x, const float* norm_w,
                         float eps, const void* router,
                         const void* Wgu, const void* Wd, const void* sWgu, const void* sWd, int wdtype,
                         int norm_topk, float scaling, float* out, int* topk_ids_out, float* topk_w_out);
dsocr_status dsocr_k_moe_ex(int T, int H, int E, int topk, int I, int Is, const float* x, const float* norm_w,
                            float eps, const void* router,
                            const void* Wgu, const void* Wd, const void* sWgu, const void* sWd, int wdtype,
                            int norm_topk, float scaling, float* out, int* topk_ids_out, float* topk_w_out,
                            int softmax_scoring, const float* router_bias, float* logits_out);
dsocr_status dsocr_k_moe_route_kind(int T, int H, int E, int topk, int I, int Is, int has_norm, const char** kind);
dsocr_status dsocr_k_moe_prefill_route(int T, int E, int topk, const float* logits, int softmax_scoring, int norm_topk,
                                       float scaling, int* ids, float* w, int* eoff, int* arow, int* apos);
dsocr_status dsocr_k_moe_combine(int T, int topk, int H, const float* y, const int* apos, const float* w,
                                 const float* shared, float* out, int accumulate);
dsocr_status dsocr_k_moe_packed(int T, int H, int E, int topk, int I, int Is, const float* x, const float* norm_w,
                                float eps, const void* router_f16, int gu_qtype, const void* Wgu_payload, int d_qtype,
                                const void* Wd_payload, int sgu_qtype, const void* sWgu_payload, int sd_qtype,
                                const void* sWd_payload, int norm_topk, float scaling, float* out, int* topk_ids_out,
                                float* topk_w_out);
dsocr_status dsocr_k_dsq_rows_dot(int qtype, size_t rows, size_t in_dim, const void* payload, int T, const float* x,
                                  float* y);
dsocr_status dsocr_k_moe_kernels(int T, int H, int E, int topk, int I, int Is, int has_norm, const char** gateup,
                                 const char** down);
dsocr_status dsocr_k_lmhead_screened(int B, int V, int K, const float* x, const float* norm_w, float eps,
                                     const void* W, const int* ban, int ban_ld, int* out_tok);
dsocr_status dsocr_k_sample_greedy(int B, int V, float* logits, const int* ctx, int ctx_cap, const int* ctx_len,
                                   int ngram, float rep_penalty, int* out_tok);
dsocr_status dsocr_k_sample_stoch(int B, int V, float* logits, const int* ctx, int ctx_cap, const int* ctx_len,
                                  int ngram, float rep_penalty, double temperature, size_t top_k, double top_p,
                                  uint64_t seed, int draws, int* out_tok);
typedef struct {
    int do_sample;
    double temperature;
    double top_p;
    size_t top_k;
    float repetition_penalty;
    size_t no_repeat_ngram_size;
    int64_t eos_token_id;
} dsocr_row_params;
dsocr_status dsocr_k_select_rows(int B, int V, float* logits, const int* ctx, int ctx_cap, const int* ctx_len,
                                 const dsocr_row_params* rows, const uint64_t* seeds, int draws, int* out_tok);
typedef struct {
    int B, V, K, wdtype, steps, probe;
    const void* W;
    const float* x;
    long long ldx;
    const float* norm_w;
    float eps;
    const int* ctx;
    int ctx_cap;
    const int* ctx_len;
    int ngram, eos;
    const dsocr_row_params* rows;
    const int* ban;
    int ban_ld, out_cap;
    const void* table;
    int table_dt, H;
    int* out_tok; int* ban_out; int* ctx_out; int* ctx_len_out; int* out_ids; int* out_len; int* done;
    int* kv_pos; int* kv_len; float* x_next;
    int* blk_cnt; float* blk_t; int* cand; float* cand_hi; float* xn_out; float* xn_gemv;
    int8_t* q; float* scale; float* bound; float* qnorm; int8_t* qfrag;
} dsocr_screen_steps;
dsocr_status dsocr_k_lmhead_screen_steps(const dsocr_screen_steps* s);
dsocr_status dsocr_k_lmhead_screen_grid(int B, int V, int K, int* nblk, long long* slot, int* matrix_core);

dsocr_status dsocr_k_logprobs(int B, int V, int K, const float* logits, int ld, const int* tok, const uint8_t* emit,
                              float* lp, int64_t* top_id, float* top_lp);
dsocr_status dsocr_k_logit_bias(int B, int V, int ld, int offset, float* logits, const int64_t* ids, const float* values,
                                const int* first, const int* count, const int* flags, const int* allow_only,
                                float* dense, int dense_ld);
dsocr_status dsocr_k_stop_match(int B, int steps, int out_cap, const int* n_seq, const int* lens, const int64_t* ids,
                                const int* tokens, const uint8_t* emit, int* out, int* out_len, int* done, int* seen,
                                int* hit, int* done_steps, int* seen_steps, int* hit_steps, int* out_len_steps);
dsocr_status dsocr_k_out_penalty(int B, int V, int ld, float* logits, const int* out_ids, int out_cap,
                                 const int* out_len, const dsocr_penalties* pen);
dsocr_status dsocr_k_guided_mask(int B, int V, int ld, int row_off, float* logits, const dsocr_guided* g, long long eos,
                                 const int* on, const int* state, const int* done, uint32_t* mask_out);
dsocr_status dsocr_k_guided_advance(int B, int steps, const dsocr_guided* g, const int* on, const int* tokens,
                                    const uint8_t* emit, int* steps_out);
dsocr_status dsocr_k_ngram_window(int B, int V, int ld, float* logits, const int* ctx, int ctx_cap, const int* ctx_len,
                                  const dsocr_ngram_window* const* recs, int plain);
dsocr_status dsocr_k_sample_stoch_min_p(int B, int V, float* logits, const int* ctx, int ctx_cap, const int* ctx_len,
                                        int ngram, float rep_penalty, double temperature, size_t top_k, double top_p,
                                        const double* ln_min_p, uint64_t seed, int draws, int* out_tok);
dsocr_status dsocr_k_logprobs_penalty(int B, int V, int K, const float* logits, int ld, const int* tok, const uint8_t* emit,
                                      const int* ctx, int ctx_cap, const int* ctx_len, float penalty, float* lp,
                                      int64_t* top_id, float* top_lp);
dsocr_status dsocr_k_session_slot_move(int layers, int slots, int kv_heads, int cap, int hd, float* kc, float* vc,
                                       int* kv_len, int* kv_pos, int* ctx, long long ctx_cap, int* ctx_len, int* out,
                                       long long out_cap, int* out_len, int* done, int* tok, uint32_t* rng,
                                       int rng_words, int* ban, long long ban_ld, float* x, int H, int src, int dst);
dsocr_status dsocr_k_session_prefix_copy(int layers, int slots, int kv_heads, int cap, int hd, float* kc, float* vc,
                                         int slot, int rows, float* entry, int to_slot);

typedef struct dsocr_dots dsocr_dots;
// ... 21 lines not shown
```

Baseline: 4.125 pages/s.

## Fuse LayerNorm/RMSNorm into split-K reduce of residual GEMMs

Adds a split-K reduce kernel that also computes a row LayerNorm or RMSNorm on the just-reduced residual row. SAM, CLIP and the decoder prefill now hand the following norm (n2, the next block's n1, post_norm) to linear() instead of launching a separate norm kernel. This removes one kernel launch and one full read of the residual per fused norm. The fused reduce runs one 64-thread wave per row, which may parallelise the reduce less well than the old 256-thread reduce. An env toggle and a test C API comparing fused and reference outputs are also added.

```diff
diff --git a/deepseek-ocr.rs_amd/csrc/engine/capi.cpp b/deepseek-ocr.rs_amd/csrc/engine/capi.cpp
--- a/deepseek-ocr.rs_amd/csrc/engine/capi.cpp
+++ b/deepseek-ocr.rs_amd/csrc/engine/capi.cpp
@@ -1174,6 +1174,54 @@
         if (e == hipSuccess) e = hipDeviceSynchronize();
         if (part) (void)hipFree(part);
         check_hip(e, "gemm_f32a");
+    });
+}
+dsocr_status dsocr_k_gemm_f32a_norm(const dsocr_gemm_norm_args* ap) {
+    return guarded([&] {
+        if (!ap) throw std::runtime_error("EINVAL: NULL argument");
+        const dsocr_gemm_norm_args& a = *ap;
+        if (!a.A || !a.W || !a.c_fused || !a.c_ref || a.M < 1 || a.N < 1 || a.K < 1 || a.ldc < a.N || a.c_rows_out < 1)
+            throw std::runtime_error("EINVAL: gemm_f32a_norm arguments");
+        if (a.wdtype != dsocr::WDT_BF16 && a.wdtype != dsocr::WDT_F16) throw std::runtime_error("EINVAL: weights must be bf16 or f16");
+        if (a.splits < 2 || a.K / 32 < a.splits) throw std::runtime_error("EINVAL: splits must be 2 .. K / 32");
+        if (a.part_skew < 0 || a.part_skew > 3) throw std::runtime_error("EINVAL: part_skew must be 0 .. 3");
+        if (a.norm_kind && (!a.norm_w || !a.y_fused || !a.y_ref || a.ldy < a.N || (a.norm_kind == 1 && !a.norm_b)))
+            throw std::runtime_error("EINVAL: gemm_f32a_norm norm arguments");
+        dsocr::GemmBf16Args g;
+        g.M = a.M; g.N = a.N; g.K = a.K; g.A = a.A; g.lda = a.K; g.W = a.W; g.ldw = a.K; g.bias = a.bias;
+        g.w_f16 = a.wdtype == dsocr::WDT_F16;
+        g.ldc = a.ldc; g.c_rows = a.c_rows; g.act = a.act; g.accumulate = a.accumulate; g.splits = a.splits;
+        g.variant = a.variant;
+        if (!dsocr::gemm_f32a_ok(g)) throw std::runtime_error("EINVAL: gemm_f32a needs K % 32 == 0 and 16-byte aligned rows");
+        float* part = nullptr;
+        check_hip(hipMalloc(&part, sizeof(float) * ((size_t)g.splits * a.M * a.N + 4)), "hipMalloc");
+        g.part = part + a.part_skew;
+        hipError_t e = hipSuccess;
+        try {
+            dsocr::GemmBf16Args f = g;
+            f.C = a.c_fused;
+            if (a.norm_kind) {
+                f.norm.kind = a.norm_kind; f.norm.w = a.norm_w; f.norm.b = a.norm_b; f.norm.eps = a.eps;
+                f.norm.y = a.y_fused; f.norm.ldy = a.ldy; f.norm.rows = a.norm_rows;
+            }
+            if (a.reduce_width) *a.reduce_width = dsocr::splitk_reduce_width(f);
+            dsocr::launch_gemm_f32a(f, nullptr);
+            g.C = a.c_ref;
+            dsocr::launch_gemm_f32a(g, nullptr);
+            if (a.norm_kind == dsocr::NORM_LAYER)
+                dsocr::launch_layernorm(a.c_ref, a.ldc, a.y_ref, a.ldy, a.norm_rows, a.c_rows_out, a.N, a.norm_w, a.norm_b,
+                                        a.eps, nullptr);
+            else if (a.norm_kind == dsocr::NORM_RMS)
+                dsocr::launch_rmsnorm(a.c_ref, a.ldc, a.y_ref, a.ldy, a.c_rows_out, a.N, a.norm_w, a.eps, nullptr);
+            e = hipGetLastError();
+        } catch (...) {
+            (void)hipDeviceSynchronize();
+            (void)hipFree(part);
+            throw;
+        }
+        if (e == hipSuccess) e = hipDeviceSynchronize();
+        (void)hipFree(part);
+        check_hip(e, "gemm_f32a_norm");
     });
 }
 dsocr_status dsocr_k_gemv(int M, int N, int K, const float* x, const float* norm_w, float eps, const void* W,
diff --git a/deepseek-ocr.rs_amd/csrc/engine/engine.cpp b/deepseek-ocr.rs_amd/csrc/engine/engine.cpp
--- a/deepseek-ocr.rs_amd/csrc/engine/engine.cpp
+++ b/deepseek-ocr.rs_amd/csrc/engine/engine.cpp
@@ -742,9 +742,15 @@
     }
 }
 
+static bool reduce_norm_on() {
+    const char* e = getenv("DSOCR_REDUCE_NORM");
+    return !(e && atoi(e) == 0);
+}
+
 void Engine::linear(const float* x, int M, int ldx, const Lin& l, float* y, int ldy, int act, int accumulate,
-                    const int* c_rows) {
+                    const int* c_rows, const NormAfter* norm, int norm_rows) {
     flops_acc_ += 2.0 * M * (double)l.N * l.K;
+    bool norm_done = !norm;
     if (M <= 16 && !c_rows) {
         DecGemvArgs a;
         a.M = M; a.N = l.N; a.K = l.K; a.x = x; a.ldx = ldx; a.W = l.W; a.ldw = l.K; a.wdtype = l.wdt;
@@ -757,6 +763,11 @@
         g.bias = l.b; g.C = y; g.ldc = ldy; g.c_rows = c_rows; g.act = act; g.accumulate = accumulate;
         g.splits = gemm_f32a_splits(M, l.N, l.K);
         if (g.splits > 1) g.part = wsf("g_splitk", (size_t)g.splits * M * l.N);
+        if (norm && reduce_norm_on()) {
+            g.norm = *norm;
+            if (gemm_f32a_norm_ok(g)) norm_done = true;
+            else g.norm = NormAfter();
+        }
         launch_gemm_f32a(g, stream_);
     } else {
         GemmArgs g;
@@ -764,6 +775,11 @@
         g.bias = l.b; g.C = y; g.ldc = ldy; g.c_rows = c_rows; g.act = act; g.accumulate = accumulate;
         launch_gemm(g, stream_);
     }
+    if (norm_done) return;
+    if (norm->kind == NORM_LAYER)
+        launch_layernorm(y, ldy, norm->y, (int)norm->ldy, norm->rows, norm_rows, l.N, norm->w, norm->b, norm->eps, stream_);
+    else
+        launch_rmsnorm(y, ldy, norm->y, (int)norm->ldy, norm_rows, l.N, norm->w, norm->eps, stream_);
 }
 
 float* Engine::sam_pos(int g) {
@@ -881,11 +897,9 @@
         const int L = win ? W * W : g * g;
         const int nseq = win ? n * nw * nw : n;
         const long arows = (long)nseq * L;
-        if (win) {
-            HIP_CHECK(hipMemsetAsync(xn, 0, (size_t)wrows * C * 4, st));
-            launch_layernorm(x, C, xn, C, d_tok2win, (int)rows, C, blk.n1.w, blk.n1.b, 1e-6f, st);
-        } else {
-            launch_layernorm(x, C, xn, C, nullptr, (int)rows, C, blk.n1.w, blk.n1.b, 1e-6f, st);
+        if (bi == 0) {
+            if (win) HIP_CHECK(hipMemsetAsync(xn, 0, (size_t)wrows * C * 4, st));
+            launch_layernorm(x, C, xn, C, win ? d_tok2win : nullptr, (int)rows, C, blk.n1.w, blk.n1.b, 1e-6f, st);
         }
         linear(xn, (int)arows, C, blk.qkv, qkv, 3 * C);
         AttnArgs a;
@@ -913,10 +927,22 @@
         }
         flops_acc_ += 4.0 * nseq * (double)L * L * hd * heads;
         launch_attention(a, st);
-        linear(ctx, (int)arows, C, blk.proj, x, C, 0, 1, win ? d_win2tok : nullptr);
-        launch_layernorm(x, C, xn, C, nullptr, (int)rows, C, blk.n2.w, blk.n2.b, 1e-6f, st);
+        NormAfter n2;
+        n2.kind = NORM_LAYER; n2.w = blk.n2.w; n2.b = blk.n2.b; n2.eps = 1e-6f; n2.y = xn; n2.ldy = C;
+        linear(ctx, (int)arows, C, blk.proj, x, C, 0, 1, win ? d_win2tok : nullptr, &n2, (int)rows);
         linear(xn, (int)rows, C, blk.fc1, hbuf, hid, ACT_GELU_ERF);
-        linear(hbuf, (int)rows, hid, blk.fc2, x, C, 0, 1);
+        if (bi + 1 == S.depth) {
+            linear(hbuf, (int)rows, hid, blk.fc2, x, C, 0, 1);
+            continue;
+        }
+        const SamBlock& nb = sam_.blocks[bi + 1];
+        NormAfter n1;
+        n1.kind = NORM_LAYER; n1.w = nb.n1.w; n1.b = nb.n1.b; n1.eps = 1e-6f; n1.y = xn; n1.ldy = C;
+        if (!nb.global) {
+            HIP_CHECK(hipMemsetAsync(xn, 0, (size_t)wrows * C * 4, st));
+            n1.rows = d_tok2win;
+        }
+        linear(hbuf, (int)rows, hid, blk.fc2, x, C, 0, 1, nullptr, &n1, (int)rows);
     }
     const int NC = S.neck;
     float* y = wsf("v_neck", (size_t)rows * NC);
@@ -948,7 +974,7 @@
     float* ch = wsf("c_h", (size_t)crow * CC.ffn);
     for (int l = 0; s2 && l < CC.layers; ++l) {
         ClipLayer& cl = clip_.layers[l];
-        launch_layernorm(cx, CH, cxn, CH, nullptr, (int)crow, CH, cl.ln1.w, cl.ln1.b, 1e-5f, st);
+        if (l == 0) launch_layernorm(cx, CH, cxn, CH, nullptr, (int)crow, CH, cl.ln1.w, cl.ln1.b, 1e-5f, st);
         linear(cxn, (int)crow, CH, cl.qkv, cqkv, 3 * CH);
         AttnArgs a;
         a.q = {cqkv, 3L * CH, chd, nullptr};
@@ -965,10 +991,16 @@
         a.scale = (float)(1.0 / std::sqrt((double)chd));
         flops_acc_ += 4.0 * n * (double)T * T * chd * CC.heads;
         launch_attention(a, st);
-        linear(cctx, (int)crow, CH, cl.out, cx, CH, 0, 1);
-        launch_layernorm(cx, CH, cxn, CH, nullptr, (int)crow, CH, cl.ln2.w, cl.ln2.b, 1e-5f, st);
+        NormAfter ln;
+        ln.kind = NORM_LAYER; ln.w = cl.ln2.w; ln.b = cl.ln2.b; ln.eps = 1e-5f; ln.y = cxn; ln.ldy = CH;
+        linear(cctx, (int)crow, CH, cl.out, cx, CH, 0, 1, nullptr, &ln, (int)crow);
         linear(cxn, (int)crow, CH, cl.fc1, ch, CC.ffn, ACT_QUICK_GELU);
-        linear(ch, (int)crow, CC.ffn, cl.fc2, cx, CH, 0, 1);
+        if (l + 1 < CC.layers) {
+            ln.w = clip_.layers[l + 1].ln1.w; ln.b = clip_.layers[l + 1].ln1.b;
+            linear(ch, (int)crow, CC.ffn, cl.fc2, cx, CH, 0, 1, nullptr, &ln, (int)crow);
+        } else {
+            linear(ch, (int)crow, CC.ffn, cl.fc2, cx, CH, 0, 1);
+        }
     }
     float* pre = wsf("p_pre", (size_t)n * Sq * (CH + c1));
     float* post = wsf(out, (size_t)n * Sq * cfg_.proj_out);
@@ -1154,8 +1186,9 @@
     }
     (void)Lmax;
     (void)KVH;
-    linear(CTX, T, H, d.o, X, H, 0, 1);
-    launch_rmsnorm(X, H, XN, H, T, H, d.post_norm.w, L.rms_eps, st);
+    NormAfter pn;
+    pn.kind = NORM_RMS; pn.w = d.post_norm.w; pn.eps = L.rms_eps; pn.y = XN; pn.ldy = H;
+    linear(CTX, T, H, d.o, X, H, 0, 1, nullptr, &pn, T);
     if (!d.moe) {
         const int I = L.inter;
         float* G = wsf("d_g", (size_t)T * 2 * I);
diff --git a/deepseek-ocr.rs_amd/csrc/engine/engine.hpp b/deepseek-ocr.rs_amd/csrc/engine/engine.hpp
--- a/deepseek-ocr.rs_amd/csrc/engine/engine.hpp
+++ b/deepseek-ocr.rs_amd/csrc/engine/engine.hpp
@@ -375,7 +375,7 @@
     }
     void* pinned(const std::string& name, size_t bytes);
     void linear(const float* x, int M, int ldx, const Lin& l, float* y, int ldy, int act = 0, int accumulate = 0,
-                const int* c_rows = nullptr);
+                const int* c_rows = nullptr, const NormAfter* norm = nullptr, int norm_rows = 0);
     float* sam_pos(int g);
     std::pair<float*, float*> sam_rel(SamBlock& b, int g);
     float* clip_pos(int tokens);
diff --git a/deepseek-ocr.rs_amd/csrc/kernels/gemm_bf16.hip b/deepseek-ocr.rs_amd/csrc/kernels/gemm_bf16.hip
--- a/deepseek-ocr.rs_amd/csrc/kernels/gemm_bf16.hip
+++ b/deepseek-ocr.rs_amd/csrc/kernels/gemm_bf16.hip
@@ -5,6 +5,7 @@
 
 #include "dev_common.hpp"
 #include "kernels.hpp"
+#include "norm_row.hpp"
 
 namespace dsocr {
 
@@ -221,7 +222,122 @@
     }
 }
 
+template <bool VEC, int NCH>
+__global__ __launch_bounds__(64) void splitk_reduce_norm_kernel(GemmBf16Args g) {
+    const int lane = threadIdx.x, row = blockIdx.x;
+    const long mn = (long)g.M * g.N;
+    const long orow = g.c_rows ? (long)g.c_rows[row] : (long)row;
+    if (orow < 0) return;
+    float4 x[NCH];
+#pragma unroll
+    for (int k = 0; k < NCH; ++k) {
+        const int col = lane * 4 + k * 256;
+        if (col >= g.N) continue;
+        const long i = (long)row * g.N + col;
+        float bv[4] = {0.f, 0.f, 0.f, 0.f};
+        if (g.bias)
+#pragma unroll
+            for (int e = 0; e < 4; ++e) bv[e] = g.bias[col + e];
+        float4 v = make_float4(0.f, 0.f, 0.f, 0.f);
+        for (int sp0 = 0; sp0 < g.splits; sp0 += 8) {
+            float4 p[8];
+#pragma unroll
+            for (int j = 0; j < 8; ++j)
+                if (sp0 + j < g.splits) {
+                    const float* pp = g.part + (sp0 + j) * mn + i;
+                    if (VEC) p[j] = *reinterpret_cast<const float4*>(pp);
+                    else p[j] = make_float4(pp[0], pp[1], pp[2], pp[3]);
+                }
+#pragma unroll
+            for (int j = 0; j < 8; ++j)
+                if (sp0 + j < g.splits) { v.x += p[j].x; v.y += p[j].y; v.z += p[j].z; v.w += p[j].w; }
+        }
+        float r[4] = {v.x, v.y, v.z, v.w};
+#pragma unroll
+        for (int e = 0; e < 4; ++e) {
+            float t = apply_act(r[e] + bv[e], g.act);
+            float* cp = g.C + orow * g.ldc + col + e;
+            if (g.accumulate) t += *cp;
+            *cp = t;
+            r[e] = t;
+        }
+        x[k] = make_float4(r[0], r[1], r[2], r[3]);
+    }
+    const NormAfter& n = g.norm;
+    const long nrow = n.rows ? (long)n.rows[orow] : orow;
+    if (nrow < 0) return;
+    float* yr = n.y + nrow * n.ldy;
+    const int cols = g.N;
+    if (n.kind == NORM_LAYER) {
+        float s = 0.f;
+#pragma unroll
+        for (int k = 0; k < NCH; ++k)
+            if (lane * 4 + k * 256 < cols) s += ln_sum4(x[k]);
+        const float mean = wave_sum(s) / (float)cols;
+        float q = 0.f;
+#pragma unroll
+        for (int k = 0; k < NCH; ++k)
+            if (lane * 4 + k * 256 < cols) q += ln_sq4(x[k], mean);
+        const float denom = norm_denom(wave_sum(q), cols, n.eps);
+#pragma unroll
+        for (int k = 0; k < NCH; ++k) {
+            const int c = lane * 4 + k * 256;
+            if (c >= cols) continue;
+            float4 wv = *reinterpret_cast<const float4*>(n.w + c);
+            float4 bv = *reinterpret_cast<const float4*>(n.b + c);
+            *reinterpret_cast<float4*>(yr + c) = ln_out4(x[k], mean, denom, wv, bv);
+        }
+    } else {
+        float q = 0.f;
+#pragma unroll
+        for (int k = 0; k < NCH; ++k)
+            if (lane * 4 + k * 256 < cols) q += rms_sq4(x[k]);
+        const float denom = norm_denom(wave_sum(q), cols, n.eps);
+#pragma unroll
+        for (int k = 0; k < NCH; ++k) {
+            const int c = lane * 4 + k * 256;
+            if (c >= cols) continue;
+            float4 wv = *reinterpret_cast<const float4*>(n.w + c);
+            *reinterpret_cast<float4*>(yr + c) = rms_out4(x[k], denom, wv);
+        }
+    }
+}
+
+constexpr int RN_MAX_CH = 8;
+
+int splitk_reduce_width(const GemmBf16Args& g) {
+    const bool aligned = g.N % 4 == 0 && (reinterpret_cast<uintptr_t>(g.part) & 15) == 0;
+    return aligned && (g.norm.kind || g.M <= 65535) ? 4 : 1;
+}
+
+bool gemm_f32a_norm_ok(const GemmBf16Args& g) {
+    const NormAfter& n = g.norm;
+    if (n.kind != NORM_LAYER && n.kind != NORM_RMS) return false;
+    if (g.splits <= 1 || !g.part || g.out_bf16 || g.N % 4 || g.N > 256 * RN_MAX_CH) return false;
+    if (!n.w || !n.y || n.ldy % 4 || (reinterpret_cast<uintptr_t>(n.y) & 15) || (reinterpret_cast<uintptr_t>(n.w) & 15))
+        return false;
+    if (n.kind == NORM_LAYER && (!n.b || (reinterpret_cast<uintptr_t>(n.b) & 15))) return false;
+    if (n.kind == NORM_RMS && n.rows) return false;
+    return true;
+}
+
+template <bool VEC>
+static void launch_splitk_reduce_norm(const GemmBf16Args& g, hipStream_t s) {
+    const int nch = (g.N + 255) / 256;
+    const dim3 grid((unsigned)g.M), block(64);
+    if (nch <= 1) hipLaunchKernelGGL((splitk_reduce_norm_kernel<VEC, 1>), grid, block, 0, s, g);
+    else if (nch <= 3) hipLaunchKernelGGL((splitk_reduce_norm_kernel<VEC, 3>), grid, block, 0, s, g);
+    else if (nch <= 4) hipLaunchKernelGGL((splitk_reduce_norm_kernel<VEC, 4>), grid, block, 0, s, g);
+    else if (nch <= 5) hipLaunchKernelGGL((splitk_reduce_norm_kernel<VEC, 5>), grid, block, 0, s, g);
+    else hipLaunchKernelGGL((splitk_reduce_norm_kernel<VEC, RN_MAX_CH>), grid, block, 0, s, g);
+}
+
 static void launch_splitk_reduce(const GemmBf16Args& g, hipStream_t s) {
+    if (g.norm.kind) {
+        if (splitk_reduce_width(g) == 4) launch_splitk_reduce_norm<true>(g, s);
+        else launch_splitk_reduce_norm<false>(g, s);
+        return;
+    }
     if (g.N % 4 == 0 && g.M <= 65535 && (reinterpret_cast<uintptr_t>(g.part) & 15) == 0) {
         hipLaunchKernelGGL(splitk_reduce4_kernel, dim3((unsigned)((g.N / 4 + 255) / 256), (unsigned)g.M), dim3(256), 0, s, g);
         return;
@@ -523,6 +639,7 @@
     if (g.K % TB_K || g.lda % 8 || g.ldw % 8 || (reinterpret_cast<uintptr_t>(g.A) & 15) ||
         (reinterpret_cast<uintptr_t>(g.W) & 15))
         throw std::runtime_error("EINVAL: gemm_bf16 needs K % 64 == 0 and 16-byte aligned rows");
+    if (g.norm.kind) throw std::runtime_error("EINVAL: gemm_bf16 takes no row norm (gemm_f32a's split-K reduce does)");
     if (g.splits < 1 || !g.part) g.splits = 1;
     g.group_m = gemm_group_m(g.group_m);
     const long pp_tiles = (long)((g.M + PP_M - 1) / PP_M) * ((g.N + PP_N - 1) / PP_N);
@@ -751,6 +868,8 @@
     if (g.M <= 0 || g.N <= 0) return;
     if (!gemm_f32a_ok(g)) throw std::runtime_error("EINVAL: gemm_f32a needs K % 32 == 0 and 16-byte aligned rows");
     if (g.splits < 1 || !g.part) g.splits = 1;
+    if (g.norm.kind && !gemm_f32a_norm_ok(g))
+        throw std::runtime_error("EINVAL: gemm_f32a row norm needs splits > 1, N % 4 == 0, N <= 2048 and 16-byte aligned rows");
     g.group_m = gemm_group_m(g.group_m);
     const int tiles = ((g.M + FX_M - 1) / FX_M) * ((g.N + FX_N - 1) / FX_N);
     if (g.w_f16) hipLaunchKernelGGL((gemm_f32a_nt_kernel<true>), dim3(tiles * g.splits), dim3(256), 0, s, g);
diff --git a/deepseek-ocr.rs_amd/csrc/kernels/kernels.hpp b/deepseek-ocr.rs_amd/csrc/kernels/kernels.hpp
--- a/deepseek-ocr.rs_amd/csrc/kernels/kernels.hpp
+++ b/deepseek-ocr.rs_amd/csrc/kernels/kernels.hpp
@@ -23,6 +23,16 @@
 };
 ProfEvents& prof_events();
 enum Act : int { ACT_NONE = 0, ACT_GELU_ERF = 1, ACT_QUICK_GELU = 2, ACT_SILU = 3 };
+
+enum NormKind : int { NORM_NONE = 0, NORM_LAYER = 1, NORM_RMS = 2 };
+struct NormAfter {
+    int kind = NORM_NONE;
+    const float* w = nullptr;
+    const float* b = nullptr;
+    float eps = 0.f;
+    float* y = nullptr; long ldy = 0;
+    const int* rows = nullptr;
+};
 
 struct GemmBf16Args {
     int M = 0, N = 0, K = 0;
@@ -33,6 +43,7 @@
     const int* c_rows = nullptr;
     int act = 0, accumulate = 0;
     int splits = 1; float* part = nullptr;
+    NormAfter norm;
     int out_bf16 = 0;
     int w_f16 = 0;
     int variant = 0;
@@ -47,6 +58,8 @@
 int gemm_bf16_splits(int M, int N, int K);
 bool gemm_f32a_ok(const GemmBf16Args& g);
 int gemm_f32a_splits(int M, int N, int K);
+bool gemm_f32a_norm_ok(const GemmBf16Args& g);
+int splitk_reduce_width(const GemmBf16Args& g);
 void launch_gemm_f32a(const GemmBf16Args& g, hipStream_t s);
 
 struct GemmArgs {
diff --git a/deepseek-ocr.rs_amd/csrc/kernels/norm.hip b/deepseek-ocr.rs_amd/csrc/kernels/norm.hip
--- a/deepseek-ocr.rs_amd/csrc/kernels/norm.hip
+++ b/deepseek-ocr.rs_amd/csrc/kernels/norm.hip
@@ -1,5 +1,6 @@
 #include "dev_common.hpp"
 #include "kernels.hpp"
+#include "norm_row.hpp"
 
 namespace dsocr {
 
@@ -14,28 +15,19 @@
     float* yr = y + orow * ldy;
     float s = 0.f;
     for (int c = lane * 4; c < cols; c += 256) {
-        float4 v = *reinterpret_cast<const float4*>(xr + c);
-        s += (v.x + v.y) + (v.z + v.w);
+        s += ln_sum4(*reinterpret_cast<const float4*>(xr + c));
     }
     const float mean = wave_sum(s) / (float)cols;
     float q = 0.f;
     for (int c = lane * 4; c < cols; c += 256) {
-        float4 v = *reinterpret_cast<const float4*>(xr + c);
-        float a0 = v.x - mean, a1 = v.y - mean, a2 = v.z - mean, a3 = v.w - mean;
-        q += (a0 * a0 + a1 * a1) + (a2 * a2 + a3 * a3);
+        q += ln_sq4(*reinterpret_cast<const float4*>(xr + c), mean);
     }
-    const float var = wave_sum(q) / (float)cols;
-    const float denom = sqrtf(var + eps);
+    const float denom = norm_denom(wave_sum(q), cols, eps);
     for (int c = lane * 4; c < cols; c += 256) {
         float4 v = *reinterpret_cast<const float4*>(xr + c);
         float4 wv = *reinterpret_cast<const float4*>(w + c);
         float4 bv = *reinterpret_cast<const float4*>(b + c);
-        float4 o;
-        o.x = (v.x - mean) / denom * wv.x + bv.x;
-        o.y = (v.y - mean) / denom * wv.y + bv.y;
-        o.z = (v.z - mean) / denom * wv.z + bv.z;
-        o.w = (v.w - mean) / denom * wv.w + bv.w;
-        *reinterpret_cast<float4*>(yr + c) = o;
+        *reinterpret_cast<float4*>(yr + c) = ln_out4(v, mean, denom, wv, bv);
     }
 }
 
@@ -55,19 +47,13 @@
     float* yr = y + (long)r * ldy;
     float q = 0.f;
     for (int c = lane * 4; c < cols; c += 256) {
-        float4 v = *reinterpret_cast<const float4*>(xr + c);
-        q += (v.x * v.x + v.y * v.y) + (v.z * v.z + v.w * v.w);
+        q += rms_sq4(*reinterpret_cast<const float4*>(xr + c));
     }
-    const float denom = sqrtf(wave_sum(q) / (float)cols + eps);
+    const float denom = norm_denom(wave_sum(q), cols, eps);
     for (int c = lane * 4; c < cols; c += 256) {
         float4 v = *reinterpret_cast<const float4*>(xr + c);
         float4 wv = *reinterpret_cast<const float4*>(w + c);
-        float4 o;
-        o.x = (v.x / denom) * wv.x;
-        o.y = (v.y / denom) * wv.y;
-        o.z = (v.z / denom) * wv.z;
-        o.w = (v.w / denom) * wv.w;
-        *reinterpret_cast<float4*>(yr + c) = o;
+        *reinterpret_cast<float4*>(yr + c) = rms_out4(v, denom, wv);
     }
 }
 
diff --git a/deepseek-ocr.rs_amd/csrc/kernels/norm_row.hpp b/deepseek-ocr.rs_amd/csrc/kernels/norm_row.hpp
--- /dev/null
+++ b/deepseek-ocr.rs_amd/csrc/kernels/norm_row.hpp
@@ -0,0 +1,47 @@
+#pragma once
+#include <hip/hip_runtime.h>
+
+namespace dsocr {
+
+__device__ __forceinline__ float ln_sum4(float4 v) {
+#pragma clang fp contract(off)
+    return (v.x + v.y) + (v.z + v.w);
+}
+
+__device__ __forceinline__ float ln_sq4(float4 v, float mean) {
+#pragma clang fp contract(off)
+    const float a0 = v.x - mean, a1 = v.y - mean, a2 = v.z - mean, a3 = v.w - mean;
+    return __builtin_fmaf(a0, a0, a1 * a1) + __builtin_fmaf(a2, a2, a3 * a3);
+}
+
+__device__ __forceinline__ float4 ln_out4(float4 v, float mean, float denom, float4 w, float4 b) {
+#pragma clang fp contract(off)
+    float4 o;
+    o.x = __builtin_fmaf((v.x - mean) / denom, w.x, b.x);
+    o.y = __builtin_fmaf((v.y - mean) / denom, w.y, b.y);
+    o.z = __builtin_fmaf((v.z - mean) / denom, w.z, b.z);
+    o.w = __builtin_fmaf((v.w - mean) / denom, w.w, b.w);
+    return o;
+}
+
+__device__ __forceinline__ float rms_sq4(float4 v) {
+#pragma clang fp contract(off)
+    return __builtin_fmaf(v.y, v.y, v.x * v.x) + __builtin_fmaf(v.z, v.z, v.w * v.w);
+}
+
+__device__ __forceinline__ float4 rms_out4(float4 v, float denom, float4 w) {
+#pragma clang fp contract(off)
+    float4 o;
+    o.x = (v.x / denom) * w.x;
+    o.y = (v.y / denom) * w.y;
+    o.z = (v.z / denom) * w.z;
+    o.w = (v.w / denom) * w.w;
+    return o;
+}
+
+__device__ __forceinline__ float norm_denom(float sq_sum, int cols, float eps) {
+#pragma clang fp contract(off)
+    return sqrtf(sq_sum / (float)cols + eps);
+}
+
+}
diff --git a/deepseek-ocr.rs_amd/dsocr/_lib.py b/deepseek-ocr.rs_amd/dsocr/_lib.py
--- a/deepseek-ocr.rs_amd/dsocr/_lib.py
+++ b/deepseek-ocr.rs_amd/dsocr/_lib.py
@@ -125,6 +125,15 @@
                 [(n, C.c_void_p) for n in ("out_tok", "ban_out", "ctx_out", "ctx_len_out", "out_ids", "out_len", "done",
                                            "kv_pos", "kv_len", "x_next", "blk_cnt", "blk_t", "cand", "cand_hi", "xn_out", "xn_gemv",
                                            "q", "scale", "bound", "qnorm", "qfrag")])
+
+
+class GemmNormArgsC(C.Structure):
+    _fields_ = [("M", C.c_int), ("N", C.c_int), ("K", C.c_int), ("A", C.c_void_p), ("W", C.c_void_p), ("wdtype", C.c_int),
+                ("bias", C.c_void_p), ("c_fused", C.c_void_p), ("c_ref", C.c_void_p), ("ldc", C.c_int),
+                ("c_rows_out", C.c_int), ("c_rows", C.c_void_p), ("act", C.c_int), ("accumulate", C.c_int),
+                ("splits", C.c_int), ("part_skew", C.c_int), ("norm_kind", C.c_int), ("norm_w", C.c_void_p),
+                ("norm_b", C.c_void_p), ("eps", C.c_float), ("y_fused", C.c_void_p), ("y_ref", C.c_void_p),
+                ("ldy", C.c_int), ("norm_rows", C.c_void_p), ("variant", C.c_int), ("reduce_width", C.POINTER(C.c_int))]
 
 
 SESSION_PER_REQUEST = 1
@@ -187,6 +196,7 @@
     "dsocr_k_ngram_window",
     "dsocr_guided_check", "dsocr_generate_guided", "dsocr_session_stage_guided", "dsocr_session_guided_state",
     "dsocr_k_guided_mask", "dsocr_k_guided_advance",
+    "dsocr_k_gemm_f32a_norm",
 ]
 
 VARIANT_OCR1, VARIANT_OCR2 = 0, 1
@@ -262,6 +272,7 @@
     L.dsocr_resize_catmull_rom.argtypes = [vp, u32, u32, vp, u32, u32]
     L.dsocr_k_gemm.argtypes = [i32, i32, i32, vp, vp, i32, vp, vp, i32, i32]
     L.dsocr_k_gemm_f32a.argtypes = [i32, i32, i32, vp, vp, i32, vp, vp, i32, i32, i32]
+    L.dsocr_k_gemm_f32a_norm.argtypes = [C.POINTER(GemmNormArgsC)]
     L.dsocr_k_gemm_grouped.argtypes = [i32, i32, i32, vp, i32, vp, vp, i32, C.c_longlong, vp, C.c_longlong, vp, i32, vp, i32,
                                        i32, vp, i32, i32, i32]
     L.dsocr_k_gemv.argtypes = [i32, i32, i32, vp, vp, f32, vp, i32, vp, vp, i32, i32]
diff --git a/include/dsocr.h b/include/dsocr.h
--- a/include/dsocr.h
+++ b/include/dsocr.h
@@ -322,6 +322,29 @@
                           int act, int accumulate);
 dsocr_status dsocr_k_gemm_f32a(int M, int N, int K, const float* A, const void* W, int wdtype, const float* bias,
                                float* C, int act, int accumulate, int splits);
+typedef struct dsocr_gemm_norm_args {
+    int M, N, K;
+    const float* A;
+    const void* W;
+    int wdtype;
+    const float* bias;
+    float* c_fused;
+    float* c_ref;
+    int ldc, c_rows_out;
+    const int* c_rows;
+    int act, accumulate, splits, part_skew;
+    int norm_kind;
+    const float* norm_w;
+    const float* norm_b;
+    float eps;
+    float* y_fused;
+    float* y_ref;
+    int ldy;
+    const int* norm_rows;
+    int variant;
+    int* reduce_width;
+} dsocr_gemm_norm_args;
+dsocr_status dsocr_k_gemm_f32a_norm(const dsocr_gemm_norm_args* a);
 dsocr_status dsocr_k_gemm_grouped(int M, int N, int K, const float* A, int lda, const int* a_rows, const void* W,
                                   int wdtype, long long w_group_stride, const float* bias, long long bias_group_stride,
                                   float* C, int ldc, const int* c_rows, int act, int accumulate, const int* group_off,
```

Result: no change. 4.159 pages/s, median of 2 (+0.8%).
